# wuwushrek/sde4mbrl_px4

Hardware: AMD Instinct MI355X
Metric: MPC solves/sec, Iris H=50 P=128, arithmetic f32x3/fast (p50 solve latency in p50_solve_latency_ms: arithmetic f32/fast; same-arithmetic pairs in by_arithmetic; every arithmetic against float64 in vs_float64) (higher is better)
Workload: dtype f32 (state, accumulation and every operand f32; the two 32x32 MLP contractions per step evaluated as three-limb bf16 splits of both f32 operands on v_mfma_f32_32x32x16_bf16: error against float64 not larger than the f32 fma chain's (tests/test_mfma16_model_cpu.py), bit-identical to the CPU oracle)

## Files before the change

include/sdempc.h:

```cpp
#ifndef SDEMPC_H
#define SDEMPC_H

#include <stddef.h>
#include <stdint.h>

#ifdef __cplusplus
extern "C" {
#endif

#define SDEMPC_ABI_VERSION 3

#define SDEMPC_NX 13
#define SDEMPC_NNOISE 6
#define SDEMPC_MAX_MOTORS 8
#define SDEMPC_HID 32
#define SDEMPC_BLOB_MAGIC 0x31454453
#define SDEMPC_BLOB_HEADER_INTS 16
#define SDEMPC_BLOB_FLOATS 2120

#define SDEMPC_OK 0
#define SDEMPC_EINVAL (-1)
#define SDEMPC_EBLOB (-2)
#define SDEMPC_EDEVICE (-3)
#define SDEMPC_ENOMEM (-4)
#define SDEMPC_ECAPACITY (-5)

typedef struct sdempc_cfg {
    int32_t struct_size;
    int32_t horizon;
    int32_t num_particles;
    int32_t num_motors;
    const float* time_steps;
    float discount;
    float uref[SDEMPC_MAX_MOTORS];
    float uerr;
    float perr[3], verr[3], qerr[3], werr[3];
    float res_mult;
    float u_slew_coeff;
    int32_t has_slew_constr;
    float u_slew_lo[SDEMPC_MAX_MOTORS], u_slew_hi[SDEMPC_MAX_MOTORS];
    float u_slew_constr_coeff;
    float u_lo[SDEMPC_MAX_MOTORS], u_hi[SDEMPC_MAX_MOTORS];
    int32_t max_iter;
    int32_t max_no_improvement_iter;
    int32_t use_moment_scale;
    float moment_scale;
    float beta_init;
    float atol, rtol;
    float stepsize;
    float ls_init_stepsize, ls_max_stepsize, ls_coef, ls_decrease_factor, ls_increase_factor;
    int32_t ls_reset_option;
    int32_t ls_maxls;
    int32_t mlp_dtype;
    int32_t math_mode;
    int32_t num_state_constr;
    int32_t state_id[SDEMPC_NX];
    float state_w[SDEMPC_NX], state_lo[SDEMPC_NX], state_hi[SDEMPC_NX];
} sdempc_cfg;

typedef struct sdempc_info {
    float avg_linesearch;
    float stepsize;
    float num_steps;
    float grad_sqr;
    float avg_stepsize;
    float init_cost;
    float opt_cost;
    float num_ls_trials;
} sdempc_info;

typedef struct sdempc_handle sdempc_handle;

int sdempc_create(const sdempc_cfg* cfg, const void* model_blob, size_t blob_bytes,
                  int32_t max_batch, sdempc_handle** out);
void sdempc_destroy(sdempc_handle* h);
const char* sdempc_last_error(const sdempc_handle* h);
int sdempc_abi_version(void);
#define SDEMPC_BUILD_ALL_VARIANTS 1
int sdempc_build_flags(void);

int sdempc_set_device(sdempc_handle* h, int32_t device);

int sdempc_device_ready(const sdempc_handle* h);

#define SDEMPC_OPT_LANE 1
#define SDEMPC_OPT_COOP 2
#define SDEMPC_OPT_SPEC 3
#define SDEMPC_OPT_PK 4
#define SDEMPC_OPT_USTG 5
#define SDEMPC_OPT_COOP_LAUNCH 6
#define SDEMPC_OPT_COOP_FENCE 7
#define SDEMPC_OPT_COOP_SPIN_US 8
#define SDEMPC_OPT_DEVICE_CUS 9
#define SDEMPC_OPT_DUO 10
#define SDEMPC_OPT_HEX 11
#define SDEMPC_OPT_TEST_ABSENT_WG 12
#define SDEMPC_OPT_TEST_WS_FILL 13
#define SDEMPC_OPT_TEST_LOOP_CHUNK_BYTES 14
int sdempc_set_option(sdempc_handle* h, int32_t key, int32_t value);
int sdempc_get_option(const sdempc_handle* h, int32_t key, int32_t* value);

int sdempc_reset(sdempc_handle* h, const float* x, const float* xdes, float* yk, sdempc_info* info);

int sdempc_rollout_batch(sdempc_handle* h, int32_t B, const float* x0, const float* u,
                         const float* xref, const float* noise,
                         float* cost , float* traj ,
                         float* xmean );
int sdempc_grad_batch(sdempc_handle* h, int32_t B, const float* x0, const float* u,
                      const float* xref, const float* noise,
                      float* cost , float* grad );
int sdempc_solve_batch(sdempc_handle* h, int32_t B, const float* x0, const float* xref,
                       const float* noise, const float* u_init ,
                       const float* stepsize_in ,
                       float* uopt , float* xevol ,
                       sdempc_info* info );

size_t sdempc_noise_dev_floats(const sdempc_handle* h, int32_t B);
size_t sdempc_traj_dev_floats(const sdempc_handle* h, int32_t B);
int sdempc_noise_to_device_layout(const sdempc_handle* h, int32_t B, const float* noise_host, float* out_host);
int sdempc_noise_to_device_layout_dev(sdempc_handle* h, int32_t B, const void* noise_canonical_dev,
                                      void* noise_out_dev, void* stream);
int sdempc_traj_to_canonical_dev(sdempc_handle* h, int32_t B, void* traj_out_dev, void* stream);
int sdempc_solve_batch_dev(sdempc_handle* h, int32_t B, const void* x0_dev, const void* xref_dev,
                           const void* noise_dev, const void* u_init_dev, const void* stepsize_dev,
                           void* uopt_dev, void* xevol_dev, void* info_dev ,
                           void* stream);
int sdempc_rollout_batch_dev(sdempc_handle* h, int32_t B, const void* x0_dev, const void* u_dev,
                             const void* xref_dev, const void* noise_dev, void* cost_dev,
                             void* xmean_dev , int32_t store_traj, void* stream);
int sdempc_grad_batch_dev(sdempc_handle* h, int32_t B, const void* x0_dev, const void* u_dev,
                          const void* xref_dev, const void* noise_dev, void* cost_dev,
                          void* grad_dev, void* stream);

int sdempc_noise_from_keys_dev(sdempc_handle* h, int32_t B, const uint32_t* keys, void* noise_out_dev , void* stream);
int sdempc_noise_from_keys(sdempc_handle* h, int32_t B, const uint32_t* keys, float* noise );
int sdempc_solve_batch_keys(sdempc_handle* h, int32_t B, const float* x0, const float* xref, const uint32_t* keys,
                            const float* u_init , const float* stepsize_in ,
                            float* uopt , float* xevol , sdempc_info* info );

int sdempc_closed_loop_batch(sdempc_handle* h, int32_t B, int32_t T, const float* x0,
                             const float* xref, int32_t xref_ticks, int32_t xref_batch,
                             const uint32_t* keys, const float* u_init , const float* stepsize_in ,
                             float* xs , float* us , sdempc_info* info ,
                             float* u_next , float* stepsize_next ,
                             uint32_t* keys_next );

#define SDEMPC_PLANT_MAX_SUBSTEPS 64
typedef struct sdempc_plant_cfg {
    int32_t struct_size;
    int32_t num_plants;
    int32_t substeps;
    float dt;
    int32_t mlp_dtype;
    int32_t math_mode;
} sdempc_plant_cfg;
int sdempc_closed_loop_batch_plant(sdempc_handle* h, const sdempc_plant_cfg* pc,
                                   const void* const* plant_blobs , const size_t* plant_blob_bytes ,
                                   const int32_t* plant_of ,
                                   int32_t B, int32_t T, const float* x0,
                                   const float* xref, int32_t xref_ticks, int32_t xref_batch,
                                   const uint32_t* keys, const float* u_init , const float* stepsize_in ,
                                   float* xs , float* us , sdempc_info* info ,
                                   float* u_next , float* stepsize_next ,
                                   uint32_t* keys_next );

typedef struct sdempc_timing_cfg {
    int32_t struct_size;
    int32_t solve_period;
    int32_t solve_delay;
    float lag_alpha;
} sdempc_timing_cfg;
int sdempc_closed_loop_batch_timed(sdempc_handle* h, const sdempc_timing_cfg* timing, const sdempc_plant_cfg* pc,
                                   const void* const* plant_blobs , const size_t* plant_blob_bytes ,
                                   const int32_t* plant_of , int32_t B, int32_t T, const float* x0,
                                   const float* xref, int32_t xref_solves, int32_t xref_batch,
                                   const uint32_t* keys, const float* u_init , const float* stepsize_in ,
                                   const float* u_act_in ,
                                   float* xs , float* us , sdempc_info* info ,
                                   float* u_next , float* stepsize_next ,
                                   uint32_t* keys_next , float* u_act_next );

typedef struct sdempc_scenario_cfg {
    int32_t struct_size;
    const float* dist;
    int32_t dist_ticks;
    int32_t dist_batch;
    int32_t plant_ticks;
} sdempc_scenario_cfg;
int sdempc_closed_loop_batch_scenario(sdempc_handle* h, const sdempc_scenario_cfg* scenario, const sdempc_timing_cfg* timing, const sdempc_plant_cfg* pc,
                                      const void* const* plant_blobs , const size_t* plant_blob_bytes ,
                                      const int32_t* plant_of , int32_t B, int32_t T, const float* x0,
                                      const float* xref, int32_t xref_solves, int32_t xref_batch,
                                      const uint32_t* keys, const float* u_init , const float* stepsize_in ,
                                      const float* u_act_in ,
                                      float* xs , float* us , sdempc_info* info ,
                                      float* u_next , float* stepsize_next ,
                                      uint32_t* keys_next , float* u_act_next );

typedef struct sdempc_rate_cfg {
    int32_t struct_size;
    float kp[3];
    float ki_dt[3];
    float integ_limit[3];
    float mixer[SDEMPC_MAX_MOTORS][3];
    float motor_weight;
    float inv_m;
} sdempc_rate_cfg;
int sdempc_closed_loop_batch_rate(sdempc_handle* h, const sdempc_rate_cfg* rate, const sdempc_scenario_cfg* scenario ,
                                  const sdempc_timing_cfg* timing, const sdempc_plant_cfg* pc,
                                  const void* const* plant_blobs , const size_t* plant_blob_bytes ,
                                  const int32_t* plant_of , int32_t B, int32_t T, const float* x0,
                                  const float* xref, int32_t xref_solves, int32_t xref_batch,
                                  const uint32_t* keys, const float* u_init , const float* stepsize_in ,
                                  const float* u_act_in ,
                                  float* xs , float* us , sdempc_info* info ,
                                  float* u_next , float* stepsize_next ,
                                  uint32_t* keys_next , float* u_act_next ,
                                  const float* rate_integ_in , const float* rate_tail_in ,
                                  float* ws , float* rate_integ_next , float* rate_tail_next );

int sdempc_solve_status(sdempc_handle* h);
int32_t sdempc_layout_fallbacks(const sdempc_handle* h);

int sdempc_work_counters(sdempc_handle* h, uint64_t out[4], int32_t reset);

int sdempc_last_kernel_name(const sdempc_handle* h, char* buf, size_t n);

float sdempc_last_kernel_ms(const sdempc_handle* h);

#ifdef __cplusplus
}
#endif
#endif
```

sde4mbrl_px4_amd/_abi.py:

```python
import ctypes as C
import os

NX = 13
NNOISE = 6
MAX_MOTORS = 8
HID = 32
BLOB_MAGIC = 0x31454453
BLOB_HEADER_INTS = 16
BLOB_FLOATS = 2120

_F8 = C.c_float * MAX_MOTORS
_F3 = C.c_float * 3


class SdempcCfg(C.Structure):
    _fields_ = [
        ("struct_size", C.c_int32),
        ("horizon", C.c_int32),
        ("num_particles", C.c_int32),
        ("num_motors", C.c_int32),
        ("time_steps", C.POINTER(C.c_float)),
        ("discount", C.c_float),
        ("uref", _F8),
        ("uerr", C.c_float),
        ("perr", _F3), ("verr", _F3), ("qerr", _F3), ("werr", _F3),
        ("res_mult", C.c_float),
        ("u_slew_coeff", C.c_float),
        ("has_slew_constr", C.c_int32),
        ("u_slew_lo", _F8), ("u_slew_hi", _F8),
        ("u_slew_constr_coeff", C.c_float),
        ("u_lo", _F8), ("u_hi", _F8),
        ("max_iter", C.c_int32),
        ("max_no_improvement_iter", C.c_int32),
        ("use_moment_scale", C.c_int32),
        ("moment_scale", C.c_float),
        ("beta_init", C.c_float),
        ("atol", C.c_float), ("rtol", C.c_float),
        ("stepsize", C.c_float),
        ("ls_init_stepsize", C.c_float), ("ls_max_stepsize", C.c_float), ("ls_coef", C.c_float),
        ("ls_decrease_factor", C.c_float), ("ls_increase_factor", C.c_float),
        ("ls_reset_option", C.c_int32),
        ("ls_maxls", C.c_int32),
        ("mlp_dtype", C.c_int32),
        ("math_mode", C.c_int32),
        ("num_state_constr", C.c_int32),
        ("state_id", C.c_int32 * NX),
        ("state_w", C.c_float * NX), ("state_lo", C.c_float * NX), ("state_hi", C.c_float * NX),
    ]


class SdempcInfo(C.Structure):
    _fields_ = [(n, C.c_float) for n in (
        "avg_linesearch", "stepsize", "num_steps", "grad_sqr", "avg_stepsize", "init_cost", "opt_cost",
        "num_ls_trials")]


class SdempcPlantCfg(C.Structure):
    _fields_ = [("struct_size", C.c_int32), ("num_plants", C.c_int32), ("substeps", C.c_int32), ("dt", C.c_float),
                ("mlp_dtype", C.c_int32), ("math_mode", C.c_int32)]


class SdempcTimingCfg(C.Structure):
    _fields_ = [("struct_size", C.c_int32), ("solve_period", C.c_int32), ("solve_delay", C.c_int32), ("lag_alpha", C.c_float)]


class SdempcScenarioCfg(C.Structure):
    _fields_ = [("struct_size", C.c_int32), ("dist", C.POINTER(C.c_float)), ("dist_ticks", C.c_int32), ("dist_batch", C.c_int32),
                ("plant_ticks", C.c_int32)]


class SdempcRateCfg(C.Structure):
    _fields_ = [("struct_size", C.c_int32), ("kp", _F3), ("ki_dt", _F3), ("integ_limit", _F3), ("mixer", (C.c_float * 3) * MAX_MOTORS),
                ("motor_weight", C.c_float), ("inv_m", C.c_float)]


PLANT_MAX_SUBSTEPS = 64

INFO_FIELDS = [f[0] for f in SdempcInfo._fields_]

OPTIONS = {"lane": 1, "coop": 2, "spec": 3, "pk": 4, "ustg": 5, "coop_launch": 6, "coop_fence": 7, "coop_spin_us": 8, "device_cus": 9, "duo": 10, "hex": 11, "test_absent_wg": 12, "test_ws_fill": 13,
           "test_loop_chunk_bytes": 14}

ABI_VERSION = 3

_LIB = None


def lib_path():
    override = os.environ.get("SDEMPC_LIB")
    if override:
        return os.path.abspath(override)
    return os.path.join(os.path.dirname(os.path.abspath(__file__)), "csrc", "libsdempc.so")


def load_library():
    global _LIB
    if _LIB is not None:
        return _LIB
    path = lib_path()
    if not os.path.exists(path):
        raise RuntimeError(
            f"{path} is missing: build the HIP extension first (python -c 'import __graft_entry__ as g; g.build()' "
            "or make -C sde4mbrl_px4_amd/csrc). sde4mbrl_px4_amd has no CPU fallback.")
    lib = C.CDLL(path)
    vp, i32, fp = C.c_void_p, C.c_int32, C.POINTER(C.c_float)
    lib.sdempc_create.argtypes = [C.POINTER(SdempcCfg), vp, C.c_size_t, i32, C.POINTER(vp)]
    lib.sdempc_create.restype = C.c_int
    lib.sdempc_destroy.argtypes = [vp]
    lib.sdempc_destroy.restype = None
    lib.sdempc_last_error.argtypes = [vp]
    lib.sdempc_last_error.restype = C.c_char_p
    lib.sdempc_abi_version.restype = C.c_int
    got = lib.sdempc_abi_version()
    if got != ABI_VERSION:
        raise RuntimeError(f"{path} reports ABI version {got}, this package's struct layouts are version {ABI_VERSION} "
                           "(include/sdempc.h: SDEMPC_ABI_VERSION): rebuild the library (make -C sde4mbrl_px4_amd/csrc)")
    lib.sdempc_build_flags.restype = C.c_int
    lib.sdempc_set_device.argtypes = [vp, i32]
    lib.sdempc_device_ready.argtypes = [vp]
    lib.sdempc_device_ready.restype = C.c_int
    lib.sdempc_set_option.argtypes = [vp, i32, i32]
    lib.sdempc_set_option.restype = C.c_int
    lib.sdempc_get_option.argtypes = [vp, i32, C.POINTER(i32)]
    lib.sdempc_get_option.restype = C.c_int
    lib.sdempc_reset.argtypes = [vp, fp, fp, fp, C.POINTER(SdempcInfo)]
    lib.sdempc_rollout_batch.argtypes = [vp, i32, fp, fp, fp, fp, fp, fp, fp]
    lib.sdempc_grad_batch.argtypes = [vp, i32, fp, fp, fp, fp, fp, fp]
    lib.sdempc_solve_batch.argtypes = [vp, i32, fp, fp, fp, fp, fp, fp, fp, C.POINTER(SdempcInfo)]
    lib.sdempc_noise_dev_floats.argtypes = [vp, i32]
    lib.sdempc_noise_dev_floats.restype = C.c_size_t
    lib.sdempc_traj_dev_floats.argtypes = [vp, i32]
    lib.sdempc_traj_dev_floats.restype = C.c_size_t
    lib.sdempc_noise_to_device_layout.argtypes = [vp, i32, fp, fp]
    lib.sdempc_noise_to_device_layout_dev.argtypes = [vp, i32, vp, vp, vp]
    lib.sdempc_traj_to_canonical_dev.argtypes = [vp, i32, vp, vp]
    lib.sdempc_solve_batch_dev.argtypes = [vp, i32] + [vp] * 9
    lib.sdempc_rollout_batch_dev.argtypes = [vp, i32, vp, vp, vp, vp, vp, vp, i32, vp]
    lib.sdempc_grad_batch_dev.argtypes = [vp, i32, vp, vp, vp, vp, vp, vp, vp]
    u32p = C.POINTER(C.c_uint32)
    lib.sdempc_noise_from_keys_dev.argtypes = [vp, i32, u32p, vp, vp]
    lib.sdempc_noise_from_keys.argtypes = [vp, i32, u32p, fp]
    lib.sdempc_solve_batch_keys.argtypes = [vp, i32, fp, fp, u32p, fp, fp, fp, fp, C.POINTER(SdempcInfo)]
    lib.sdempc_closed_loop_batch.argtypes = [vp, i32, i32, fp, fp, i32, i32, u32p, fp, fp, fp, fp, C.POINTER(SdempcInfo), fp, fp, u32p]
    lib.sdempc_closed_loop_batch_plant.argtypes = [vp, C.POINTER(SdempcPlantCfg), C.POINTER(vp), C.POINTER(C.c_size_t), C.POINTER(i32)] + \
        lib.sdempc_closed_loop_batch.argtypes[1:]
    lib.sdempc_solve_status.argtypes = [vp]
    lib.sdempc_solve_status.restype = C.c_int
    lib.sdempc_layout_fallbacks.argtypes = [vp]
    lib.sdempc_layout_fallbacks.restype = C.c_int32
    lib.sdempc_work_counters.argtypes = [vp, C.POINTER(C.c_uint64), i32]
    lib.sdempc_work_counters.restype = C.c_int
    lib.sdempc_last_kernel_name.argtypes = [vp, C.c_char_p, C.c_size_t]
    lib.sdempc_last_kernel_name.restype = C.c_int
    lib.sdempc_last_kernel_ms.argtypes = [vp]
    lib.sdempc_last_kernel_ms.restype = C.c_float
    for name in ("sdempc_set_device", "sdempc_reset", "sdempc_rollout_batch", "sdempc_grad_batch", "sdempc_solve_batch",
                 "sdempc_noise_to_device_layout", "sdempc_solve_batch_dev", "sdempc_rollout_batch_dev",
                 "sdempc_grad_batch_dev", "sdempc_noise_to_device_layout_dev", "sdempc_traj_to_canonical_dev",
                 "sdempc_noise_from_keys_dev", "sdempc_noise_from_keys", "sdempc_solve_batch_keys", "sdempc_closed_loop_batch",
                 "sdempc_closed_loop_batch_plant"):
        getattr(lib, name).restype = C.c_int
    _LIB = lib
    return lib


def timed_entry(lib):
    try:
        fn = lib.sdempc_closed_loop_batch_timed
    except AttributeError:
        raise RuntimeError(f"{lib_path()} has no sdempc_closed_loop_batch_timed (SPEC.md §11b): rebuild the library (make -C sde4mbrl_px4_amd/csrc)") from None
    if fn.argtypes is None:
        a = list(lib.sdempc_closed_loop_batch_plant.argtypes)
        fp = C.POINTER(C.c_float)
        fn.argtypes = [a[0], C.POINTER(SdempcTimingCfg)] + a[1:14] + [fp] + a[14:] + [fp]
        fn.restype = C.c_int
    return fn


def scenario_entry(lib):
    try:
        fn = lib.sdempc_closed_loop_batch_scenario
    except AttributeError:
        raise RuntimeError(f"{lib_path()} has no sdempc_closed_loop_batch_scenario (SPEC.md §11c): rebuild the library (make -C sde4mbrl_px4_amd/csrc)") from None
    if fn.argtypes is None:
        a = list(timed_entry(lib).argtypes)
        fn.argtypes = [a[0], C.POINTER(SdempcScenarioCfg)] + a[1:]
        fn.restype = C.c_int
    return fn


def rate_entry(lib):
    try:
        fn = lib.sdempc_closed_loop_batch_rate
    except AttributeError:
        raise RuntimeError(f"{lib_path()} has no sdempc_closed_loop_batch_rate (SPEC.md §11d): rebuild the library (make -C sde4mbrl_px4_amd/csrc)") from None
    if fn.argtypes is None:
        a = list(scenario_entry(lib).argtypes)
        fp = C.POINTER(C.c_float)
        fn.argtypes = [a[0], C.POINTER(SdempcRateCfg)] + a[1:] + [fp] * 5
        fn.restype = C.c_int
    return fn


EXPORTED_SYMBOLS = [
    "sdempc_create", "sdempc_destroy", "sdempc_last_error", "sdempc_abi_version", "sdempc_build_flags", "sdempc_set_device", "sdempc_device_ready", "sdempc_set_option", "sdempc_get_option", "sdempc_reset",
    "sdempc_rollout_batch", "sdempc_grad_batch", "sdempc_solve_batch", "sdempc_noise_dev_floats",
    "sdempc_traj_dev_floats", "sdempc_noise_to_device_layout", "sdempc_solve_batch_dev", "sdempc_rollout_batch_dev",
    "sdempc_grad_batch_dev", "sdempc_last_kernel_ms", "sdempc_last_kernel_name", "sdempc_work_counters", "sdempc_solve_status", "sdempc_layout_fallbacks", "sdempc_noise_to_device_layout_dev", "sdempc_traj_to_canonical_dev",
    "sdempc_noise_from_keys_dev", "sdempc_noise_from_keys", "sdempc_solve_batch_keys", "sdempc_closed_loop_batch",
    "sdempc_closed_loop_batch_plant", "sdempc_closed_loop_batch_timed", "sdempc_closed_loop_batch_scenario",
    "sdempc_closed_loop_batch_rate",
]
```

sde4mbrl_px4_amd/csrc/sdempc_api.cpp:

```cpp
#include <hip/hip_runtime.h>
#include <math.h>
#include <stdint.h>
#include <stdio.h>
#include <stdlib.h>
#include <string.h>

#include <cxxabi.h>

#include <memory>
#include <new>
#include <stdexcept>
#include <string>
#include <vector>

#include "../../include/sdempc.h"
#include "sdempc_kernels.h"

using namespace sdempc;
static_assert(blob::FLOATS == SDEMPC_BLOB_FLOATS, "blob layout: sdempc_kernels.h and include/sdempc.h");

namespace {
std::string g_create_error;

float f16_rtz_host(float x) {
// ... 174 lines not shown
            (h)->err = b__;                                                             \
            return SDEMPC_EDEVICE;                                                      \
        }                                                                               \
    } while (0)

int env_int(const char* name, int dflt, int lo, int hi) {
    const char* e = getenv(name);
    if (!e || !*e) return dflt;
    char* end = nullptr;
    const long v = strtol(e, &end, 10);
    if (end == e || v < lo || v > hi) return dflt;
    return (int)v;
}
void default_options(sdempc_handle* h) {
    LaunchOpts& o = h->base.opt;
    o.cus = 256;
    o.lane = env_int("SDEMPC_LANE", 1, 0, 1);
    o.coop = env_int("SDEMPC_COOP", 1, 0, 1);
    o.spec = env_int("SDEMPC_SPEC", 1, 0, 1);
    o.pk = env_int("SDEMPC_PK", -1, -1, 1);
    o.ustg = env_int("SDEMPC_USTG", -1, -1, 1);
    o.duo = env_int("SDEMPC_DUO", -1, -1, 1);
    o.coop_launch = env_int("SDEMPC_COOP_LAUNCH", 0, 0, 1);
    o.coop_fence = env_int("SDEMPC_COOP_FENCE", 0, 0, 1);
    o.hex = env_int("SDEMPC_HEX", 1, 0, 1);
    o.absent_wg = -1;
    h->spin_us = env_int("SDEMPC_COOP_SPIN_US", -1, -1, 10 * 1000 * 1000);
}
unsigned coop_spin_ticks(const sdempc_handle* h) {
    if (h->spin_us >= 0) return (unsigned)((uint64_t)h->spin_us * 100u > 0xFFFFFFFFull ? 0xFFFFFFFFu : (unsigned)h->spin_us * 100u);
    float ms = h->coop_ms_last > 0.0f ? 5.0f * h->coop_ms_last : 100.0f;
    if (ms < 2.0f) ms = 2.0f;
    if (ms > 100.0f) ms = 100.0f;
    return (unsigned)(ms * 1e5f);
}

int null_stream_done(sdempc_handle* h) {
    HIPCHK(h, hipStreamSynchronize(nullptr));
    return 0;
}
int dev_alloc(sdempc_handle* h, DevBuf& b, size_t bytes, bool fill = false) {
    if (bytes == 0) bytes = 16;
    HIPCHK(h, hipMalloc(&b.p, bytes));
    b.bytes = bytes;
    if (fill && h->ws_fill >= 0) {
        HIPCHK(h, hipMemset(b.p, h->ws_fill, bytes));
        return null_stream_done(h);
    }
    return 0;
}
void dev_free(DevBuf& b) {
    if (b.p) (void)hipFree(b.p);
    b.p = nullptr;
    b.bytes = 0;
}

size_t noise_floats(const sdempc_handle* h, int B) { return (size_t)B * h->G * h->H * SDEMPC_NNOISE * 32; }
size_t traj_floats(const sdempc_handle* h, int B) { return (size_t)B * h->G * (h->H + 1) * SDEMPC_NX * 32; }

int ensure_device_impl(sdempc_handle* h) {
    if (h->dev_ready) {
        HIPCHK(h, hipSetDevice(h->device));
        return 0;
    }
    int n = 0;
    hipError_t e = hipGetDeviceCount(&n);
    if (e != hipSuccess || n <= 0) return fail(h, SDEMPC_EDEVICE, "no HIP device available (%s); sdempc has no CPU fallback", hipGetErrorString(e));
    if (h->device >= n) return fail(h, SDEMPC_EDEVICE, "device ordinal out of range%s");
    HIPCHK(h, hipSetDevice(h->device));
    {
        int cus = 0;
        HIPCHK(h, hipDeviceGetAttribute(&cus, hipDeviceAttributeMultiprocessorCount, h->device));
        if (cus > 0) h->base.opt.cus = cus;
    }
    HIPCHK(h, hipStreamCreateWithFlags(&h->stream, hipStreamNonBlocking));
    HIPCHK(h, hipEventCreate(&h->ev0));
    HIPCHK(h, hipEventCreate(&h->ev1));
    const int H = h->H, m = h->m, B = h->max_batch;
    int rc;
    if ((rc = dev_alloc(h, h->d_dt, sizeof(float) * H))) return rc;
    if ((rc = dev_alloc(h, h->d_sdt, sizeof(float) * H * SDEMPC_NNOISE))) return rc;
    if ((rc = dev_alloc(h, h->d_disc, sizeof(float) * (H + 1)))) return rc;
    if ((rc = dev_alloc(h, h->d_beta, sizeof(float) * h->h_beta.size()))) return rc;
    if ((rc = dev_alloc(h, h->d_wts, sizeof(float) * h->blob_f.size()))) return rc;
    HIPCHK(h, hipMemcpy(h->d_dt.p, h->time_steps.data(), sizeof(float) * H, hipMemcpyHostToDevice));
    HIPCHK(h, hipMemcpy(h->d_sdt.p, h->h_sdt.data(), sizeof(float) * H * SDEMPC_NNOISE, hipMemcpyHostToDevice));
    HIPCHK(h, hipMemcpy(h->d_disc.p, h->h_disc.data(), sizeof(float) * (H + 1), hipMemcpyHostToDevice));
    HIPCHK(h, hipMemcpy(h->d_beta.p, h->h_beta.data(), sizeof(float) * h->h_beta.size(), hipMemcpyHostToDevice));
    HIPCHK(h, hipMemcpy(h->d_wts.p, h->blob_f.data(), sizeof(float) * h->blob_f.size(), hipMemcpyHostToDevice));
    if (h->cfg.num_state_constr > 0) {
        CostK::StateBound tab[SDEMPC_NX];
        for (int k = 0; k < h->cfg.num_state_constr; ++k)
            tab[k] = CostK::StateBound{h->cfg.state_id[k], h->cfg.state_w[k], h->cfg.state_lo[k], h->cfg.state_hi[k]};
        if ((rc = dev_alloc(h, h->d_sctab, sizeof(CostK::StateBound) * h->cfg.num_state_constr))) return rc;
        HIPCHK(h, hipMemcpy(h->d_sctab.p, tab, sizeof(CostK::StateBound) * h->cfg.num_state_constr, hipMemcpyHostToDevice));
        h->base.C.sc_n = h->cfg.num_state_constr;
        h->base.C.sc_tab = (const CostK::StateBound*)h->d_sctab.p;
    }
    if ((rc = dev_alloc(h, h->d_x0, sizeof(float) * B * SDEMPC_NX, true))) return rc;
    if ((rc = dev_alloc(h, h->d_u, sizeof(float) * B * H * m, true))) return rc;
    if ((rc = dev_alloc(h, h->d_xref, sizeof(float) * B * (H + 1) * SDEMPC_NX, true))) return rc;
    if ((rc = dev_alloc(h, h->d_noise, sizeof(float) * noise_floats(h, B), true))) return rc;
    if ((rc = dev_alloc(h, h->d_step, sizeof(float) * B, true))) return rc;
    if ((rc = dev_alloc(h, h->d_cost, sizeof(float) * B, true))) return rc;
    if ((rc = dev_alloc(h, h->d_grad, sizeof(float) * B * H * m, true))) return rc;
    if ((rc = dev_alloc(h, h->d_xmean, sizeof(float) * B * (H + 1) * SDEMPC_NX, true))) return rc;
    if ((rc = dev_alloc(h, h->d_uopt, sizeof(float) * B * H * m, true))) return rc;
    if ((rc = dev_alloc(h, h->d_info, sizeof(float) * B * 8, true))) return rc;
    if ((rc = dev_alloc(h, h->d_work, sizeof(unsigned long long) * 5))) return rc;
    HIPCHK(h, hipMemset(h->d_work.p, 0, h->d_work.bytes));
    if ((rc = null_stream_done(h))) return rc;
    h->base.work = (unsigned long long*)h->d_work.p;
    h->base.ticket_host = &h->ticket_total;
    h->ticket_total = 0;
    h->base.dt = (const float*)h->d_dt.p;
    h->base.sdt = (const float*)h->d_sdt.p;
    h->base.disc = (const float*)h->d_disc.p;
    h->base.beta = (const float*)h->d_beta.p;
    h->base.wts = (const float*)h->d_wts.p;
    h->dev_ready = true;
    return 0;
}

int ensure_workspace(sdempc_handle* h, int rows) {
    if (rows <= h->ws_rows) return 0;
    HIPCHK(h, hipStreamSynchronize(h->stream));
    for (DevBuf* b : {&h->d_traj, &h->d_act, &h->d_part, &h->d_ustg}) dev_free(*b);
    h->ws_rows = 0; h->base.ws_rows = 0; h->traj_batch = 0;
    h->base.traj = h->base.act = h->base.part = h->base.ustg = nullptr;
    const int H = h->H;
    int rc;
    if ((rc = dev_alloc(h, h->d_traj, sizeof(float) * traj_floats(h, rows), true))) return rc;
    if (h->ws_fill < 0) {
        HIPCHK(h, hipMemset(h->d_traj.p, 0, h->d_traj.bytes));
        if ((rc = null_stream_done(h))) return rc;
    }
    if ((rc = dev_alloc(h, h->d_act, sizeof(float) * (size_t)rows * h->G * H * ACT_STRIDE, true))) return rc;
    if ((rc = dev_alloc(h, h->d_part, sizeof(float) * (size_t)rows * h->G * part_stride(H), true))) return rc;
    if ((rc = dev_alloc(h, h->d_ustg, sizeof(float) * (size_t)rows * H * 36, true))) return rc;
    h->base.traj = (float*)h->d_traj.p;
    h->base.act = (float*)h->d_act.p;
    h->base.part = (float*)h->d_part.p;
    h->base.ustg = (float*)h->d_ustg.p;
    h->ws_rows = rows;
    h->base.ws_rows = rows;
    return 0;
}

void release_device(sdempc_handle* h);

int ensure_device(sdempc_handle* h) {
    const bool was_ready = h->dev_ready;
    const int rc = ensure_device_impl(h);
    if (rc != 0 && !was_ready) { const std::string keep = h->err; release_device(h); h->err = keep; }
    return rc;
}

int check_batch(sdempc_handle* h, int B) {
    if (!h) return SDEMPC_EINVAL;
    if (B < 1) return fail(h, SDEMPC_EINVAL, "batch must be >= 1%s");
    if (B > h->max_batch) return fail(h, SDEMPC_ECAPACITY, "batch exceeds max_batch given to sdempc_create%s");
    return 0;
}

void noise_to_dev_layout(const sdempc_handle* h, int B, const float* in, float* out) {
    const int P = h->P, H = h->H, G = h->G;
    memset(out, 0, sizeof(float) * noise_floats(h, B));
    for (int b = 0; b < B; ++b)
        for (int p = 0; p < P; ++p) {
            const int g = p / 32, l = p % 32;
            for (int t = 0; t < H; ++t)
                for (int i = 0; i < SDEMPC_NNOISE; ++i)
                    out[((((size_t)b * G + g) * H + t) * SDEMPC_NNOISE + i) * 32 + l] = in[(((size_t)b * P + p) * H + t) * SDEMPC_NNOISE + i];
        }
}

int stage_common(sdempc_handle* h, int B, const float* x0, const float* u, const float* xref, const float* noise) {
    const int H = h->H, m = h->m;
    int rc;
    if (!h->d_noise_canon.p && (rc = dev_alloc(h, h->d_noise_canon, sizeof(float) * (size_t)h->max_batch * h->P * H * SDEMPC_NNOISE, true))) return rc;
    HIPCHK(h, hipMemcpyAsync(h->d_x0.p, x0, sizeof(float) * B * SDEMPC_NX, hipMemcpyHostToDevice, h->stream));
    HIPCHK(h, hipMemcpyAsync(h->d_u.p, u, sizeof(float) * B * H * m, hipMemcpyHostToDevice, h->stream));
    HIPCHK(h, hipMemcpyAsync(h->d_xref.p, xref, sizeof(float) * B * (H + 1) * SDEMPC_NX, hipMemcpyHostToDevice, h->stream));
    HIPCHK(h, hipMemcpyAsync(h->d_noise_canon.p, noise, sizeof(float) * (size_t)B * h->P * H * SDEMPC_NNOISE, hipMemcpyHostToDevice, h->stream));
    HIPCHK(h, launch_relayout(true, (const float*)h->d_noise_canon.p, (float*)h->d_noise.p, B, h->P, h->G, H * SDEMPC_NNOISE, h->stream));
    return 0;
}

int noise_from_keys(sdempc_handle* h, int B, const uint32_t* keys, float* out_dev, hipStream_t st) {
    int rc;
    if (!h->d_keys.p && (rc = dev_alloc(h, h->d_keys, sizeof(uint32_t) * 2 * (size_t)h->max_batch))) return rc;
    HIPCHK(h, hipMemcpyAsync(h->d_keys.p, keys, sizeof(uint32_t) * 2 * (size_t)B, hipMemcpyHostToDevice, st));
    HIPCHK(h, launch_noise_from_keys((const uint32_t*)h->d_keys.p, out_dev, B, h->P, h->G, h->H, st));
    return 0;
}

int coop_timed_out(sdempc_handle* h, bool* timed_out) {
    *timed_out = false;
    if (h->last_coop_B <= 0) return 0;
    std::vector<unsigned> f(COOP_BAR_WORDS * (size_t)h->last_coop_B);
    HIPCHK(h, hipMemcpy(f.data(), h->d_coop_bar.p, sizeof(unsigned) * f.size(), hipMemcpyDeviceToHost));
    for (int b = 0; b < h->last_coop_B; ++b)
        if (f[COOP_BAR_WORDS * b + 1] != 0u) *timed_out = true;
    if (*timed_out) {
        h->coop_off = true;
        h->layout_fallbacks += 1;
        h->last_coop_B = 0;
    } else if (h->timed) {
        float ms = 0.0f;
        if (hipEventElapsedTime(&ms, h->ev0, h->ev1) == hipSuccess && ms > 0.0f) h->coop_ms_last = ms;
    }
    return 0;
}

int tickets_consistent(sdempc_handle* h) {
    if (!h->last_ticketed || !h->dev_ready) return 0;
    h->last_ticketed = false;
    unsigned word = 0;
    HIPCHK(h, hipMemcpy(&word, (const char*)h->d_work.p + 4 * sizeof(unsigned long long), sizeof word, hipMemcpyDeviceToHost));
    if (word == h->ticket_total) return 0;
    char msg[256];
    snprintf(msg, sizeof msg, "ticketed launch: the device's ticket word reads %u where the host expects %u (aborted kernel, overlapping launches of one "
                              "handle, or a replayed graph); instances of that launch may be unsolved", word, h->ticket_total);
    h->ticket_total = word;
    return fail(h, SDEMPC_EDEVICE, "%s", msg);
}

template <class F>
int timed_launch(sdempc_handle* h, hipStream_t st, F&& f) {
    HIPCHK(h, hipEventRecord(h->ev0, st));
    hipError_t e = f();
    if (e != hipSuccess) return fail(h, SDEMPC_EDEVICE, "kernel launch failed: %s", hipGetErrorString(e));
    HIPCHK(h, hipEventRecord(h->ev1, st));
    h->timed = true;
    h->last_fn = last_launched_kernel();
    return 0;
}


int solve_staged(sdempc_handle* h, int32_t B, float* uopt, float* xevol, sdempc_info* info);
struct LoopIo {
    int B, T, xref_ticks, xref_batch;
    const float *x0, *xref;
    const uint32_t* keys;
    const float *u_init, *stepsize_in;
    float *xs, *us;
    sdempc_info* info;
    float *u_next, *stepsize_next;
    uint32_t* keys_next;
};
struct PlantRun {
    KArgs k;
    LoopPlant Q;
    float* xi;
    float dt;
};
struct TimedRun {
    int S, D;
    float alpha;
    const float* u_act_in;
    float* u_act_next;
};
struct ScenarioRun {
    const float* dist;
    int Td, Bd;
    const int32_t* plant_of;
    int Tp;
};
struct RateRun {
    const sdempc_rate_cfg* cfg;
    float inv_m;
    const float *integ_in, *tail_in;
    float *ws, *integ_next, *tail_next;
};
inline int loop_solves(int T, int S) { return (int)(((long long)T + S - 1) / S); }
enum LoopLayer { LOOP_PLAIN, LOOP_PLANT, LOOP_TIMED, LOOP_SCENARIO, LOOP_RATE };
struct LoopCall {
    LoopLayer layer;
    LoopIo io;
    const sdempc_plant_cfg* pc;
    const void* const* plant_blobs;
    const size_t* plant_blob_bytes;
    const int32_t* plant_of;
    const sdempc_timing_cfg* tc;
    const float* u_act_in;
    float* u_act_next;
    const sdempc_scenario_cfg* sc;
    const sdempc_rate_cfg* rc;
    const float *rate_integ_in, *rate_tail_in;
    float *ws, *rate_integ_next, *rate_tail_next;
};
int closed_loop_call(sdempc_handle* h, const LoopCall& c);
int check_loop_args(sdempc_handle* h, const LoopIo& io, int solves);
int check_plant_args(sdempc_handle* h, const sdempc_plant_cfg* pc, const void* const* plant_blobs, const size_t* plant_blob_bytes, const int32_t* plant_of, int B, int sched_rows);
int closed_loop_attempts(sdempc_handle* h, const LoopIo& io, const PlantRun* plant, const TimedRun* timed, const ScenarioRun* scen, const RateRun* rate);
int closed_loop_run(sdempc_handle* h, const LoopIo& io, const PlantRun* plant, const TimedRun* timed, const ScenarioRun* scen, const RateRun* rate, bool* again);
int stage_plants(sdempc_handle* h, const sdempc_plant_cfg& pc, const void* const* blobs, const int32_t* plant_of, int B, PlantRun* out, int xi_ticks = 1);
}

extern "C" {

int sdempc_abi_version(void) { return SDEMPC_ABI_VERSION; }
int sdempc_build_flags(void) { return SDEMPC_ALL_VARIANTS ? SDEMPC_BUILD_ALL_VARIANTS : 0; }

const char* sdempc_last_error(const sdempc_handle* h) { return h ? h->err.c_str() : g_create_error.c_str(); }

int sdempc_create(const sdempc_cfg* cfg, const void* model_blob, size_t blob_bytes, int32_t max_batch, sdempc_handle** out) {
    return guarded(nullptr, [&]() -> int {
    if (!out) return fail(nullptr, SDEMPC_EINVAL, "out is NULL%s");
    *out = nullptr;
    if (!cfg || cfg->struct_size != (int32_t)sizeof(sdempc_cfg)) return fail(nullptr, SDEMPC_EINVAL, "cfg NULL or struct_size mismatch%s");
    if (int rc = check_blob(nullptr, model_blob, blob_bytes)) return rc;
    const int32_t* hd = (const int32_t*)model_blob;
    const int m = hd[2];
    if (m < 1 || m > SDEMPC_MAX_MOTORS || m != cfg->num_motors) return fail(nullptr, SDEMPC_EINVAL, "num_motors of cfg and model blob differ or out of range%s");
    if (cfg->horizon < 1 || cfg->horizon > 4096 || cfg->num_particles < 1 || !cfg->time_steps || max_batch < 1)
        return fail(nullptr, SDEMPC_EINVAL, "horizon/num_particles/time_steps/max_batch invalid%s");
    if (cfg->max_iter < 0 || cfg->ls_maxls < 0 || cfg->max_no_improvement_iter < 1) return fail(nullptr, SDEMPC_EINVAL, "apg parameters invalid%s");
    if (cfg->num_state_constr < 0 || cfg->num_state_constr > SDEMPC_NX) return fail(nullptr, SDEMPC_EINVAL, "num_state_constr out of range%s");
    for (int k = 0; k < cfg->num_state_constr; ++k)
        if (cfg->state_id[k] < 0 || cfg->state_id[k] >= SDEMPC_NX || (k > 0 && cfg->state_id[k] <= cfg->state_id[k - 1]))
            return fail(nullptr, SDEMPC_EINVAL, "state_id must be strictly ascending indices into the 13-state%s");
    for (int t = 0; t < cfg->horizon; ++t)
        if (!(cfg->time_steps[t] > 0.0f)) return fail(nullptr, SDEMPC_EINVAL, "time_steps must be positive%s");
    if (smem_bytes(cfg->horizon, m, team_ipb((cfg->num_particles + 31) / 32, cfg->horizon, m)) > 160 * 1024) return fail(nullptr, SDEMPC_EINVAL, "horizon too large for one workgroup's LDS (160 KiB)%s");
    if (cfg->max_iter > 10 * 1000 * 1000) return fail(nullptr, SDEMPC_EINVAL, "max_iter beyond 10^7%s");
    std::unique_ptr<sdempc_handle> hp(new (std::nothrow) sdempc_handle());
    sdempc_handle* h = hp.get();
    if (!h) return fail(nullptr, SDEMPC_ENOMEM, "out of memory%s");
    h->cfg = *cfg;
    h->H = cfg->horizon; h->P = cfg->num_particles; h->m = m; h->G = (h->P + 31) / 32; h->max_batch = max_batch;
    h->time_steps.assign(cfg->time_steps, cfg->time_steps + h->H);
    h->cfg.time_steps = h->time_steps.data();
    const float* f = (const float*)(hd + SDEMPC_BLOB_HEADER_INTS);
    if (cfg->mlp_dtype < 0 || cfg->mlp_dtype > 2) return fail(nullptr, SDEMPC_EINVAL, "mlp_dtype must be 0 (f32), 1 (f16) or 2 (f32x3)%s");
    if (cfg->math_mode != 0 && cfg->math_mode != 1) return fail(nullptr, SDEMPC_EINVAL, "math_mode must be 0 (exact) or 1 (fast)%s");
    PreparedModel pm;
    prepare_model(f, cfg->mlp_dtype, cfg->math_mode, h->time_steps.data(), h->H, pm);
    h->blob_f = std::move(pm.blob_f);
    h->h_sdt = std::move(pm.sdt);
    h->h_disc.resize(h->H + 1);
    float d = 1.0f / (float)h->H;
    for (int t = 0; t <= h->H; ++t) { h->h_disc[t] = d; d = d * cfg->discount; }
    h->h_beta.resize(cfg->max_iter + 2);
    for (int i = 0; i < cfg->max_iter + 2; ++i) {
        float b = (i == 0) ? cfg->beta_init : (float)(i + 1) / (float)(i + 4);
        if (i > 0 && cfg->use_moment_scale) b = cfg->moment_scale * b;
        h->h_beta[i] = b;
    }
    KArgs& a = h->base;
    memset(&a, 0, sizeof a);
    a.H = h->H; a.P = h->P; a.m = m; a.G = h->G;
    a.invP = 1.0f / (float)h->P;
    a.f16 = cfg->mlp_dtype;
    a.fast = cfg->math_mode == 1;
    a.M = pm.M;
    for (int i = 0; i < 3; ++i) { a.C.perr[i] = cfg->perr[i]; a.C.verr[i] = cfg->verr[i]; a.C.qerr[i] = cfg->qerr[i]; a.C.werr[i] = cfg->werr[i]; }
    a.C.res_mult = cfg->res_mult; a.C.uerr = cfg->uerr; a.C.slew = cfg->u_slew_coeff; a.C.slew_cc = cfg->u_slew_constr_coeff;
    a.C.has_sc = cfg->has_slew_constr;
    for (int j = 0; j < 8; ++j) {
        a.C.slew_lo[j] = cfg->u_slew_lo[j]; a.C.slew_hi[j] = cfg->u_slew_hi[j]; a.C.uref[j] = cfg->uref[j];
        a.C.ulo[j] = cfg->u_lo[j]; a.C.uhi[j] = cfg->u_hi[j];
    }
    a.C.sc_n = 0; a.C.sc_tab = nullptr;
    a.A.max_iter = cfg->max_iter; a.A.max_noimp = cfg->max_no_improvement_iter; a.A.maxls = cfg->ls_maxls;
    a.A.reset_inc = cfg->ls_reset_option == 1;
    a.A.atol = cfg->atol; a.A.rtol = cfg->rtol; a.A.stepsize = cfg->stepsize; a.A.smax = cfg->ls_max_stepsize;
    a.A.coef = cfg->ls_coef; a.A.dec = cfg->ls_decrease_factor; a.A.inc = cfg->ls_increase_factor;
    default_options(h);
    *out = hp.release();
    return SDEMPC_OK;
    });
}

void sdempc_destroy(sdempc_handle* h) {
    if (!h) return;
    release_device(h);
    delete h;
}

}

namespace {
void release_device(sdempc_handle* h) {
    if (h->dev_ready || h->stream || h->d_dt.p) {
        (void)hipSetDevice(h->device);
        for (DevBuf* b : {&h->d_sctab, &h->d_ustg, &h->d_part, &h->d_act, &h->d_dt, &h->d_sdt, &h->d_disc, &h->d_beta, &h->d_wts, &h->d_traj, &h->d_x0, &h->d_u, &h->d_xref, &h->d_noise, &h->d_noise_canon, &h->d_traj_canon, &h->d_keys, &h->d_loop, &h->d_loop_chunk, &h->d_plant, &h->d_rate, &h->d_work, &h->d_coop_bar, &h->d_coop_pp, &h->d_coop_ck,
                          &h->d_step, &h->d_cost, &h->d_grad, &h->d_xmean, &h->d_uopt, &h->d_info})
            dev_free(*b);
        if (h->ev0) (void)hipEventDestroy(h->ev0);
        if (h->ev1) (void)hipEventDestroy(h->ev1);
        if (h->stream) (void)hipStreamDestroy(h->stream);
        h->ev0 = h->ev1 = nullptr; h->stream = nullptr; h->coop_cap = 0; h->ws_rows = 0;
    }
    h->dev_ready = false; h->timed = false;
}
}

extern "C" {

int sdempc_set_device(sdempc_handle* h, int32_t device) {
    return guarded(h, [&]() -> int {
    if (!h) return SDEMPC_EINVAL;
    if (h->dev_ready) return fail(h, SDEMPC_EINVAL, "sdempc_set_device must precede the first device call%s");
    if (device < 0) return fail(h, SDEMPC_EINVAL, "negative device ordinal%s");
    h->device = device;
    return SDEMPC_OK;
    });
}

int sdempc_device_ready(const sdempc_handle* h) { return h && h->dev_ready ? 1 : 0; }

int sdempc_set_option(sdempc_handle* h, int32_t key, int32_t value) {
    return guarded(h, [&]() -> int {
    if (!h) return SDEMPC_EINVAL;
    LaunchOpts& o = h->base.opt;
    auto flag = [&](int& dst) { if (value != 0 && value != 1) return fail(h, SDEMPC_EINVAL, "option value must be 0 or 1%s"); dst = value; return (int)SDEMPC_OK; };
    auto tri = [&](int& dst) { if (value < -1 || value > 1) return fail(h, SDEMPC_EINVAL, "option value must be -1 (auto), 0 or 1%s"); dst = value; return (int)SDEMPC_OK; };
    switch (key) {
        case SDEMPC_OPT_LANE: return flag(o.lane);
        case SDEMPC_OPT_COOP: { int rc = flag(o.coop); if (rc == SDEMPC_OK && value == 1) h->coop_off = false; return rc; }
        case SDEMPC_OPT_SPEC: return flag(o.spec);
        case SDEMPC_OPT_PK:
            if (value == 1 && !SDEMPC_ALL_VARIANTS) return fail(h, SDEMPC_EINVAL, "this build carries no packed-tanh instantiations (make EXTRA=-DSDEMPC_ALL_VARIANTS=1)%s");
            return tri(o.pk);
        case SDEMPC_OPT_USTG: return tri(o.ustg);
        case SDEMPC_OPT_DUO: return tri(o.duo);
        case SDEMPC_OPT_COOP_LAUNCH: return flag(o.coop_launch);
        case SDEMPC_OPT_COOP_FENCE: return flag(o.coop_fence);
        case SDEMPC_OPT_HEX: return flag(o.hex);
        case SDEMPC_OPT_TEST_ABSENT_WG:
            if (value < -1) return fail(h, SDEMPC_EINVAL, "absent workgroup must be -1 (none) or a workgroup index%s");
            o.absent_wg = value;
            return SDEMPC_OK;
        case SDEMPC_OPT_TEST_WS_FILL:
            if (value < -1 || value > 255) return fail(h, SDEMPC_EINVAL, "workspace fill must be -1 (none) or a byte value 0..255%s");
            h->ws_fill = value;
            return SDEMPC_OK;
        case SDEMPC_OPT_COOP_SPIN_US:
            if (value < -1) return fail(h, SDEMPC_EINVAL, "spin budget must be -1 (derived) or >= 0 microseconds%s");
            h->spin_us = value;
            return SDEMPC_OK;
        case SDEMPC_OPT_TEST_LOOP_CHUNK_BYTES:
            if (value < -1) return fail(h, SDEMPC_EINVAL, "loop chunk bytes must be -1 (built-in) or >= 0%s");
            h->loop_chunk_bytes = value;
            return SDEMPC_OK;
        default: return fail(h, SDEMPC_EINVAL, "unknown option key%s");
    }
    });
}

int sdempc_get_option(const sdempc_handle* h, int32_t key, int32_t* value) {
    return guarded(h, [&]() -> int {
    if (!h || !value) return SDEMPC_EINVAL;
    const LaunchOpts& o = h->base.opt;
    switch (key) {
        case SDEMPC_OPT_LANE: *value = o.lane; break;
        case SDEMPC_OPT_COOP: *value = o.coop && !h->coop_off; break;
        case SDEMPC_OPT_SPEC: *value = o.spec; break;
        case SDEMPC_OPT_PK: *value = o.pk; break;
        case SDEMPC_OPT_USTG: *value = o.ustg; break;
        case SDEMPC_OPT_DUO: *value = o.duo; break;
        case SDEMPC_OPT_COOP_LAUNCH: *value = o.coop_launch; break;
        case SDEMPC_OPT_COOP_FENCE: *value = o.coop_fence; break;
        case SDEMPC_OPT_HEX: *value = o.hex; break;
        case SDEMPC_OPT_TEST_ABSENT_WG: *value = o.absent_wg; break;
        case SDEMPC_OPT_TEST_WS_FILL: *value = h->ws_fill; break;
        case SDEMPC_OPT_TEST_LOOP_CHUNK_BYTES: *value = h->loop_chunk_bytes; break;
        case SDEMPC_OPT_COOP_SPIN_US: *value = h->spin_us >= 0 ? h->spin_us : (int32_t)(coop_spin_ticks(h) / 100u); break;
        case SDEMPC_OPT_DEVICE_CUS: *value = o.cus; break;
        default: return SDEMPC_EINVAL;
    }
    return SDEMPC_OK;
    });
}

int sdempc_reset(sdempc_handle* h, const float* x, const float* xdes, float* yk, sdempc_info* info) {
    return guarded(h, [&]() -> int {
    if (!h || !yk || !info) return SDEMPC_EINVAL;
    (void)x; (void)xdes;
    for (int t = 0; t < h->H; ++t)
        for (int j = 0; j < h->m; ++j) yk[t * h->m + j] = h->cfg.uref[j];
    memset(info, 0, sizeof *info);
    info->stepsize = h->cfg.ls_maxls > 0 ? h->cfg.ls_init_stepsize : h->cfg.stepsize;
    return SDEMPC_OK;
    });
}

size_t sdempc_noise_dev_floats(const sdempc_handle* h, int32_t B) { return h ? noise_floats(h, B) : 0; }
size_t sdempc_traj_dev_floats(const sdempc_handle* h, int32_t B) { return h ? traj_floats(h, B) : 0; }

int sdempc_noise_to_device_layout(const sdempc_handle* h, int32_t B, const float* noise_host, float* out_host) {
    return guarded(h, [&]() -> int {
    if (!h || !noise_host || !out_host || B < 1) return SDEMPC_EINVAL;
    noise_to_dev_layout(h, B, noise_host, out_host);
    return SDEMPC_OK;
    });
}

int sdempc_noise_to_device_layout_dev(sdempc_handle* h, int32_t B, const void* noise_canonical_dev, void* noise_out_dev, void* stream) {
    return guarded(h, [&]() -> int {
    int rc = check_batch(h, B);
    if (rc) return rc;
    if (!noise_canonical_dev || !noise_out_dev) return fail(h, SDEMPC_EINVAL, "NULL device pointer%s");
    if ((rc = ensure_device(h))) return rc;
    hipStream_t st = stream ? (hipStream_t)stream : h->stream;
    HIPCHK(h, launch_relayout(true, (const float*)noise_canonical_dev, (float*)noise_out_dev, B, h->P, h->G, h->H * SDEMPC_NNOISE, st));
    return SDEMPC_OK;
    });
}

int sdempc_traj_to_canonical_dev(sdempc_handle* h, int32_t B, void* traj_out_dev, void* stream) {
    return guarded(h, [&]() -> int {
    int rc = check_batch(h, B);
    if (rc) return rc;
    if (!traj_out_dev) return fail(h, SDEMPC_EINVAL, "NULL device pointer%s");
    if ((rc = ensure_device(h))) return rc;
    if (B > h->traj_batch)
        return fail(h, SDEMPC_EINVAL, h->traj_batch ? "the trajectory workspace holds fewer instances than asked for (last rollout with store_traj was smaller)%s"
                                                     : "the trajectory workspace holds no rollout: run a rollout with store_traj first (a gradient evaluation, a solve or a "
                                                       "workspace reallocation since then has overwritten it)%s");
    hipStream_t st = stream ? (hipStream_t)stream : h->stream;
    HIPCHK(h, launch_relayout(false, (const float*)h->d_traj.p, (float*)traj_out_dev, B, h->P, h->G, (h->H + 1) * SDEMPC_NX, st));
    return SDEMPC_OK;
    });
}

int sdempc_rollout_batch_dev(sdempc_handle* h, int32_t B, const void* x0_dev, const void* u_dev, const void* xref_dev, const void* noise_dev,
                             void* cost_dev, void* xmean_dev, int32_t store_traj, void* stream) {
    return guarded(h, [&]() -> int {
    int rc = check_batch(h, B);
    if (rc) return rc;
    if (!x0_dev || !u_dev || !xref_dev || !noise_dev || !cost_dev) return fail(h, SDEMPC_EINVAL, "NULL device pointer%s");
    if ((rc = ensure_device(h))) return rc;
    if ((rc = ensure_workspace(h, B))) return rc;
    KArgs a = h->base;
    a.x0 = (const float*)x0_dev; a.u = (const float*)u_dev; a.xref = (const float*)xref_dev; a.noise = (const float*)noise_dev;
    a.cost = (float*)cost_dev; a.xmean = (float*)xmean_dev; a.store_traj = store_traj;
    hipStream_t st = stream ? (hipStream_t)stream : h->stream;
    h->traj_batch = 0;
    rc = timed_launch(h, st, [&] { return launch_rollout(a, B, st); });
    if (rc == SDEMPC_OK && store_traj) h->traj_batch = B;
    return rc;
    });
}

int sdempc_grad_batch_dev(sdempc_handle* h, int32_t B, const void* x0_dev, const void* u_dev, const void* xref_dev, const void* noise_dev,
                          void* cost_dev, void* grad_dev, void* stream) {
    return guarded(h, [&]() -> int {
    int rc = check_batch(h, B);
    if (rc) return rc;
    if (!x0_dev || !u_dev || !xref_dev || !noise_dev || !cost_dev || !grad_dev) return fail(h, SDEMPC_EINVAL, "NULL device pointer%s");
    if ((rc = ensure_device(h))) return rc;
    if ((rc = ensure_workspace(h, B))) return rc;
    KArgs a = h->base;
    a.x0 = (const float*)x0_dev; a.u = (const float*)u_dev; a.xref = (const float*)xref_dev; a.noise = (const float*)noise_dev;
    a.cost = (float*)cost_dev; a.grad = (float*)grad_dev;
    hipStream_t st = stream ? (hipStream_t)stream : h->stream;
    h->traj_batch = 0;
    return timed_launch(h, st, [&] { return launch_grad(a, B, st); });
    });
}

int sdempc_solve_batch_dev(sdempc_handle* h, int32_t B, const void* x0_dev, const void* xref_dev, const void* noise_dev, const void* u_init_dev,
                           const void* stepsize_dev, void* uopt_dev, void* xevol_dev, void* info_dev, void* stream) {
    return guarded(h, [&]() -> int {
    int rc = check_batch(h, B);
    if (rc) return rc;
    if (!x0_dev || !xref_dev || !noise_dev || !u_init_dev || !stepsize_dev || !uopt_dev || !xevol_dev || !info_dev)
        return fail(h, SDEMPC_EINVAL, "NULL device pointer%s");
    if ((rc = ensure_device(h))) return rc;
    {
        KArgs probe = h->base; probe.B = B;
        if ((rc = ensure_workspace(h, solve_workspace_rows(probe, B)))) return rc;
    }
    h->traj_batch = 0;
    KArgs a = h->base;
    a.x0 = (const float*)x0_dev; a.u = (const float*)u_init_dev; a.xref = (const float*)xref_dev; a.noise = (const float*)noise_dev;
    a.stepsize_in = (const float*)stepsize_dev; a.uopt = (float*)uopt_dev; a.xmean = (float*)xevol_dev; a.info = (float*)info_dev;
    hipStream_t st = stream ? (hipStream_t)stream : h->stream;
    const bool coop_ok = !a.f16 && !h->coop_off && a.C.sc_n == 0;
    const int smax = coop_ok ? spec_max_instances(h->P, h->H, h->m, a.opt) : 0;
    int cmax = coop_ok ? coop_max_instances(h->P, h->H, h->m, a.opt) : 0;
    if (smax > cmax) cmax = smax;
    if (B <= cmax) {
        if (!h->d_coop_bar.p) {
            const int cap = cmax < h->max_batch ? cmax : h->max_batch;
            if ((rc = dev_alloc(h, h->d_coop_bar, sizeof(unsigned) * COOP_BAR_WORDS * (size_t)cap))) return rc;
            if ((rc = dev_alloc(h, h->d_coop_pp, sizeof(float) * coop_pp_floats(h->H, h->G) * cap, true))) return rc;
            if ((rc = dev_alloc(h, h->d_coop_ck, sizeof(float) * coop_ck_floats(h->H, h->P) * cap, true))) return rc;
            h->coop_cap = cap;
        }
        if (B <= h->coop_cap) {
            HIPCHK(h, hipMemsetAsync(h->d_coop_bar.p, 0, sizeof(unsigned) * COOP_BAR_WORDS * (size_t)B, st));
            a.coop_bar = (unsigned*)h->d_coop_bar.p; a.coop_pp = (float*)h->d_coop_pp.p; a.coop_ck = (float*)h->d_coop_ck.p;
            a.coop_spin = coop_spin_ticks(h);
            h->last_coop_B = B; h->last_ticketed = false;
            if (B <= smax) {
                HIPCHK(h, hipMemsetAsync(h->d_coop_pp.p, 0, sizeof(float) * coop_pp_floats(h->H, h->G) * (size_t)B, st));
                return timed_launch(h, st, [&] { return launch_solve_spec(a, B, st); });
            }
            if (B <= coop_max_instances(h->P, h->H, h->m, a.opt)) return timed_launch(h, st, [&] { return launch_solve_coop(a, B, st); });
            h->last_coop_B = 0;
        }
    }
    h->last_coop_B = 0;
// ... 585 lines not shown
```

sde4mbrl_px4_amd/csrc/sdempc_duo.inc.h:

```cpp

DI void half_split(float v, float& a_both, float& b_both) {
    unsigned a = __builtin_bit_cast(unsigned, v), b;
    asm("v_mov_b32 %0, %1" : "=v"(b) : "v"(a));
    auto r = __builtin_amdgcn_permlane32_swap(a, b, false, false);
    const unsigned r0 = r[0], r1 = r[1];
    a_both = __builtin_bit_cast(float, r0); b_both = __builtin_bit_cast(float, r1);
}
DI float half_join_sum(float pa, float pb) {
    auto r = __builtin_amdgcn_permlane32_swap(__builtin_bit_cast(unsigned, pa), __builtin_bit_cast(unsigned, pb), false, false);
    const unsigned r0 = r[0], r1 = r[1];
    return __builtin_bit_cast(float, r0) + __builtin_bit_cast(float, r1);
}

template <class Team>
DI int duo_workspace_slot() { return __builtin_amdgcn_readfirstlane((int)(blockIdx.x * Team::IPB) + Team::team()); }

struct DuoPair {
    int g;
    bool hasB;
    bool own;
};
DI DuoPair duo_pair(int gp, int G, int h) {
    DuoPair p;
    p.hasB = (2 * gp + 1) < G;
    p.own = (h == 0) || p.hasB;
    p.g = 2 * gp + ((h && p.hasB) ? 1 : 0);
    return p;
}

DI void duo_reform_rotation(const float* x, float* Rm) {
    float xq[NX];
#pragma unroll
    for (int i = 0; i < NX; ++i) xq[i] = x[i];
#pragma unroll
    for (int i = 6; i < 10; ++i) asm volatile("" : "+v"(xq[i]));
    rot_from_q(xq, Rm);
}

constexpr int PRIO_SLICE_LOG2 = 16;
DI void duo_rotate_priority() {
    const unsigned slot = __builtin_amdgcn_s_getreg(63492) & 15u;
    const unsigned r = ((unsigned)(__builtin_amdgcn_s_memrealtime() >> PRIO_SLICE_LOG2) + slot) % 3u;
    if (r == 0) __builtin_amdgcn_s_setprio(0);
    else if (r == 1) __builtin_amdgcn_s_setprio(1);
    else __builtin_amdgcn_s_setprio(2);
}

DI void duo_noise_request(const float* nzb, unsigned nzo, int t, const float* stage) {
    const float* rows = nzb + (size_t)t * (NN * 32);
    const unsigned m0 = (unsigned)__builtin_amdgcn_readfirstlane((int)(unsigned)(size_t)(const __attribute__((address_space(3))) float*)stage);
    unsigned m0_keep;
    asm volatile(
        "s_mov_b32 %0, m0\n\t"
        "s_mov_b32 m0, %3\n\ts_nop 0\n\tglobal_load_lds_dword %1, %2\n\t"
        "s_add_u32 m0, m0, 0x80\n\ts_nop 0\n\tglobal_load_lds_dword %1, %2 offset:128\n\t"
        "s_add_u32 m0, m0, 0x80\n\ts_nop 0\n\tglobal_load_lds_dword %1, %2 offset:256\n\t"
        "s_add_u32 m0, m0, 0x80\n\ts_nop 0\n\tglobal_load_lds_dword %1, %2 offset:384\n\t"
        "s_add_u32 m0, m0, 0x80\n\ts_nop 0\n\tglobal_load_lds_dword %1, %2 offset:512\n\t"
        "s_add_u32 m0, m0, 0x80\n\ts_nop 0\n\tglobal_load_lds_dword %1, %2 offset:640\n\t"
        "s_mov_b32 m0, %0"
        : "=&s"(m0_keep) : "v"(nzo * 4u), "s"(rows), "s"(m0) : "memory", "scc");
}
template <int PENDING>
DI void duo_noise_take(const float* stage, int lane, float* xi) {
    asm volatile("s_waitcnt vmcnt(%0)" ::"n"(PENDING) : "memory");
#pragma unroll
    for (int i = 0; i < NN; ++i) xi[i] = stage[i * 64 + lane];
}

template <int F16, bool CKPT, bool NZS>
DI void duo_step_fwd(const KArgs& a, const Smem& sm, const WaveW& ww, int t, int h, int lane, bool hasB, const float* x, const float* xi_reg, float* xn,
                     StepAux& A, float* acA, float* acB) {
    const float* ust = sm.ust + t * UST;
    float z[NN], zA[NN], zB[NN];
    fwd_head(x, A.Rm, z);
#pragma unroll
    for (int k = 0; k < NN; ++k) half_split(z[k], zA[k], zB[k]);
    SCHED_PHASE();
    float PA[7], PB[7];
    fwd_mlp_partials<F16, false, CKPT ? 4 : 7>(a, sm, ww, ust, h, lane, zA, A, PA);
    if constexpr (CKPT) {
#pragma unroll
        for (int q = 0; q < 4; ++q)
            *reinterpret_cast<float4*>(acA + (q * 64 + lane) * 4) = make_float4(A.h2[4 * q], A.h2[4 * q + 1], A.h2[4 * q + 2], A.h2[4 * q + 3]);
    }
    SCHED_PHASE();
    if (hasB) {
        fwd_mlp_partials<F16, false, CKPT ? 4 : 7>(a, sm, ww, ust, h, lane, zB, A, PB);
        if constexpr (CKPT) {
#pragma unroll
            for (int q = 0; q < 4; ++q)
                *reinterpret_cast<float4*>(acB + (q * 64 + lane) * 4) = make_float4(A.h2[4 * q], A.h2[4 * q + 1], A.h2[4 * q + 2], A.h2[4 * q + 3]);
        }
    } else {
#pragma unroll
        for (int i = 0; i < 7; ++i) PB[i] = PA[i];
    }
    SCHED_PHASE();
    float o[6];
#pragma unroll
    for (int i = 0; i < 6; ++i) o[i] = half_join_sum(PA[i], PB[i]) + a.M.b3[i];
    const float eta = sigmoid_spec(half_join_sum(PA[6], PB[6]) + a.M.b3n);
    SCHED_PHASE();
    if constexpr (CKPT) duo_reform_rotation(x, A.Rm);
    float xi[NN];
    if constexpr (NZS) duo_noise_take<CKPT ? 4 : 0>(sm.nzs, lane, xi);
    else {
#pragma unroll
        for (int i = 0; i < NN; ++i) xi[i] = xi_reg[i];
    }
    fwd_tail(a, sm, ust, t, x, xi, A.Rm, o, eta, xn, A);
}

template <class Team, int F16, bool NZS>
DI float duo_rollout(const KArgs& a, const Smem& sm, const WaveW& ww, const float* u, int b, int tid, bool store_traj, float* xmean_out) {
    b = opaque_s(b); tid = opaque_v(tid);
    const int H = a.H, G = a.G, P = a.P;
    const int lane = tid & 63, j = lane & 31, h = lane >> 5;
    const int wave = __builtin_amdgcn_readfirstlane(tid >> 6);
    const bool want_mean = xmean_out != nullptr;
    CLK_BEGIN(t_roll);
    Team::sync();
    block_prepass<Team>(a, sm, u, tid);
    const int PS = part_stride(H);
    const int ws = duo_workspace_slot<Team>();
    float* prows = a.part + (size_t)ws * G * PS;
    float cu = block_ucost<Team>(a, sm, u, tid);
    Team::sync();
    const int NPAIR = (G + 1) >> 1;
    for (int gp = wave; gp < NPAIR; gp += Team::NWAVES) {
        const DuoPair pr = duo_pair(gp, G, h);
        const bool valid = pr.own && (pr.g * 32 + j) < P;
        const unsigned gofs = (unsigned)(pr.g - 2 * gp);
        const float* nzb = a.noise + ((size_t)(b * G + 2 * gp) * H) * NN * 32;
        float* tjb = a.traj + ((size_t)(ws * G + 2 * gp) * (H + 1)) * NX * 32;
        const unsigned nzo = gofs * (unsigned)(H * NN * 32) + (unsigned)j;
        const unsigned tjo = gofs * (unsigned)((H + 1) * NX * 32) + (unsigned)j;
        float* xm = prows + (size_t)pr.g * PS;
        float x[NX], xn[NX], xi[NN];
#pragma unroll
        for (int i = 0; i < NX; ++i) x[i] = a.x0[b * NX + i];
        if constexpr (NZS) {
            duo_noise_request(nzb, nzo, 0, sm.nzs);
#pragma unroll
            for (int i = 0; i < NX; ++i) asm volatile("" : "+v"(x[i]));
        } else {
#pragma unroll
            for (int i = 0; i < NN; ++i) xi[i] = nzb[nzo + (unsigned)(i * 32)];
        }
        if (store_traj && pr.own) {
#pragma unroll
            for (int i = 0; i < NX; ++i) tjb[tjo + (unsigned)(i * 32)] = x[i];
        }
        if (want_mean) {
#pragma unroll
            for (int i = 0; i < NX; ++i) { float s = group_bfly32(valid ? x[i] : 0.0f); if (j == 0 && pr.own) xm[i] = s; }
        }
        float J = 0.0f;
        StepAux A;
        CLK_BEGIN(t_loop);
        for (int t = 0; t < H; ++t) {
            duo_rotate_priority();
            float xin[NN];
            if constexpr (!NZS) {
                if (t + 1 < H) {
#pragma unroll
                    for (int i = 0; i < NN; ++i) xin[i] = nzb[nzo + (unsigned)(((t + 1) * NN + i) * 32)];
                }
            }
            duo_step_fwd<F16, false, NZS>(a, sm, ww, t, h, lane, pr.hasB, x, xi, xn, A, nullptr, nullptr);
            if constexpr (NZS) { if (t + 1 < H) duo_noise_request(nzb, nzo, t + 1, sm.nzs); }
            float l = stage_cost<false>(a, xn, sm.xref + (t + 1) * NX, nullptr);
            l = FMA(a.C.res_mult * A.eta, A.eta, l);
            J = FMA(sm.disc[t], l, J);
#pragma unroll
            for (int i = 0; i < NX; ++i) x[i] = xn[i];
            if constexpr (!NZS) {
                if (t + 1 < H) {
#pragma unroll
                    for (int i = 0; i < NN; ++i) xi[i] = xin[i];
                }
            }
            if (store_traj && pr.own) {
#pragma unroll
                for (int i = 0; i < NX; ++i) tjb[tjo + (unsigned)(((t + 1) * NX + i) * 32)] = x[i];
            }
            if (want_mean) {
#pragma unroll
                for (int i = 0; i < NX; ++i) { float s = group_bfly32(valid ? x[i] : 0.0f); if (j == 0 && pr.own) xm[(t + 1) * NX + i] = s; }
            }
        }
        CLK_END(2, t_loop);
        const float T = group_bfly32(valid ? J : 0.0f);
        if (j == 0 && pr.own) xm[PS - 1] = T;
    }
    Team::sync();
    const float tot = group_ordered_sum(prows, G, PS, PS - 1);
    if (want_mean) {
        for (int i = tid; i < (H + 1) * NX; i += Team::NT) xmean_out[i] = group_ordered_sum(prows, G, PS, i) * a.invP;
    }
    CLK_END(1, t_roll);
    return FMA(tot, a.invP, cu);
}

template <class Team, int M, int F16, bool NZS>
DI float duo_cost_grad(const KArgs& a, const Smem& sm, const WaveW& ww, const float* y, float* gout, int b, int tid) {
    b = opaque_s(b); tid = opaque_v(tid);
    const int H = a.H, G = a.G, P = a.P;
    constexpr int nq = M + 4;
    const int lane = tid & 63, j = lane & 31, h = lane >> 5;
    const int wave = __builtin_amdgcn_readfirstlane(tid >> 6);
    CLK_BEGIN(t_grad);
    Team::sync();
    block_prepass<Team>(a, sm, y, tid);
    const int PS = part_stride(H);
    const int ws = duo_workspace_slot<Team>();
    float* prows = a.part + (size_t)ws * G * PS;
    float cu = block_ucost<Team>(a, sm, y, tid);
    Team::sync();
    const int NPAIR = (G + 1) >> 1;
    for (int gp = wave; gp < NPAIR; gp += Team::NWAVES) {
        const DuoPair pr = duo_pair(gp, G, h);
        const bool valid = pr.own && (pr.g * 32 + j) < P;
        const int gA = 2 * gp, gB = pr.hasB ? 2 * gp + 1 : gA;
        const unsigned gofs = (unsigned)(pr.g - gA);
        const float* nzb = a.noise + ((size_t)(b * G + gA) * H) * NN * 32;
        float* tjb = a.traj + ((size_t)(ws * G + gA) * (H + 1)) * NX * 32;
        const unsigned nzo = gofs * (unsigned)(H * NN * 32) + (unsigned)j;
        const unsigned tjo = gofs * (unsigned)((H + 1) * NX * 32) + (unsigned)j;
        float* acA = a.act + ((size_t)(ws * G + gA) * H) * ACT_STRIDE;
        float* acB = a.act + ((size_t)(ws * G + gB) * H) * ACT_STRIDE;
        const unsigned aso = gofs * (unsigned)(H * ACT_STRIDE) + 1024u + (unsigned)j * 8u;
        float* Sq = prows + (size_t)pr.g * PS;
        float x[NX], xn[NX], xi[NN];
        StepAux A;
        CLK_BEGIN(t_fwd);
#pragma unroll
        for (int i = 0; i < NX; ++i) x[i] = a.x0[b * NX + i];
        if (pr.own) {
#pragma unroll
            for (int i = 0; i < NX; ++i) tjb[tjo + (unsigned)(i * 32)] = x[i];
        }
        if constexpr (NZS) {
            duo_noise_request(nzb, nzo, 0, sm.nzs);
#pragma unroll
            for (int i = 0; i < NX; ++i) asm volatile("" : "+v"(x[i]));
        } else {
#pragma unroll
            for (int i = 0; i < NN; ++i) xi[i] = nzb[nzo + (unsigned)(i * 32)];
        }
        float J = 0.0f;
        for (int t = 0; t < H; ++t) {
            duo_rotate_priority();
            float xin[NN];
            if constexpr (!NZS) {
                if (t + 1 < H) {
#pragma unroll
                    for (int i = 0; i < NN; ++i) xin[i] = nzb[nzo + (unsigned)(((t + 1) * NN + i) * 32)];
                }
            }
            duo_step_fwd<F16, true, NZS>(a, sm, ww, t, h, lane, pr.hasB, x, xi, xn, A, acA + (size_t)t * ACT_STRIDE, acB + (size_t)t * ACT_STRIDE);
            if constexpr (NZS) { if (t + 1 < H) duo_noise_request(nzb, nzo, t + 1, sm.nzs); }
            if (pr.own) {
                const unsigned so = aso + (unsigned)(t * ACT_STRIDE);
                *reinterpret_cast<float4*>(acA + so) = make_float4(A.eta, A.Fb[0], A.Fb[1], A.Fb[2]);
                acA[so + 4] = A.rn;
            }
            float l = stage_cost<false>(a, xn, sm.xref + (t + 1) * NX, nullptr);
            l = FMA(a.C.res_mult * A.eta, A.eta, l);
            J = FMA(sm.disc[t], l, J);
#pragma unroll
            for (int i = 0; i < NX; ++i) x[i] = xn[i];
            if constexpr (!NZS) {
                if (t + 1 < H) {
#pragma unroll
                    for (int i = 0; i < NN; ++i) xi[i] = xin[i];
                }
            }
            if (pr.own) {
#pragma unroll
                for (int i = 0; i < NX; ++i) tjb[tjo + (unsigned)(((t + 1) * NX + i) * 32)] = x[i];
            }
        }
        { const float T = group_bfly32(valid ? J : 0.0f); if (j == 0 && pr.own) Sq[PS - 1] = T; }
        CLK_END(4, t_fwd);
        CLK_BEGIN(t_adj);
        float lam[NX], xt[NX];
#pragma unroll
        for (int i = 0; i < NX; ++i) lam[i] = 0.0f;
        __builtin_amdgcn_fence(__ATOMIC_SEQ_CST, "workgroup");
        for (int t = H - 1; t >= 0; --t) {
            duo_rotate_priority();
            const float* apA = acA + (size_t)t * ACT_STRIDE;
            const float* apB = acB + (size_t)t * ACT_STRIDE;
            float4 hA[4], hB[4];
#pragma unroll
            for (int q = 0; q < 4; ++q) hA[q] = *reinterpret_cast<const float4*>(apA + (q * 64 + lane) * 4);
            float touched = 0.0f;
            {
                if (pr.hasB) {
                    const float* tp = apB + (lane & 31) * 32;
                    asm volatile("global_load_dword %0, %1, off" : "=v"(touched) : "v"(tp) : "memory");
                }
            }
            const unsigned so = aso + (unsigned)(t * ACT_STRIDE);
            const float4 ns4 = *reinterpret_cast<const float4*>(acA + so);
            const float nrn = acA[so + 4];
            {
#pragma unroll
                for (int i = 0; i < NX; ++i) xt[i] = tjb[tjo + (unsigned)((t * NX + i) * 32)];
#pragma unroll
                for (int i = 0; i < NN; ++i) xi[i] = nzb[nzo + (unsigned)((t * NN + i) * 32)];
            }
            const float dsc = sm.disc[t];
            {
                float gx[NX];
                stage_cost<true>(a, x, sm.xref + (t + 1) * NX, gx);
#pragma unroll
                for (int i = 0; i < NX; ++i) lam[i] = FMA(dsc, gx[i], lam[i]);
            }
            SCHED_PHASE();
            const float* ust = sm.ust + t * UST;
            float z[NN], zA[NN], zB[NN];
            fwd_head(xt, A.Rm, z);
#pragma unroll
            for (int k = 0; k < NN; ++k) half_split(z[k], zA[k], zB[k]);
            A.eta = ns4.x; A.Fb[0] = ns4.y; A.Fb[1] = ns4.z; A.Fb[2] = ns4.w; A.rn = nrn;
#pragma unroll
            for (int i = 0; i < 3; ++i) A.Jom[i] = a.M.J[i] * xt[10 + i];
#pragma unroll
            for (int i = 0; i < 4; ++i) A.qn[i] = x[6 + i];
            const float ebc = dsc * ((2.0f * a.C.res_mult) * A.eta);
            VjpTmp T;
            float gq[12], lamn[NX];
            vjp_head<M>(a, sm, t, xt, xi, A, lam, ebc, T, gq);
            float eA, eB, obA[6], obB[6];
            float adj_inv = 1.0f;
            ObLimbs OA, OB;
            if constexpr (FAST && F16 != 0) {
                const AdjScale S = adj_scale(a, T.ebraw, T.ob);
                adj_inv = S.inv;
                half_split(T.ebraw * S.s2, eA, eB);
                float obs[6];
#pragma unroll
                for (int i = 0; i < 6; ++i) obs[i] = T.ob[i] * S.s2;
                const ObLimbs O = ob_limbs(obs);
#pragma unroll
                for (int i = 0; i < 3; ++i) {
                    float la, lb;
                    half_split(__builtin_bit_cast(float, O.r1[i]), la, lb); OA.r1[i] = __builtin_bit_cast(unsigned, la); OB.r1[i] = __builtin_bit_cast(unsigned, lb);
                    half_split(__builtin_bit_cast(float, O.r2[i]), la, lb); OA.r2[i] = __builtin_bit_cast(unsigned, la); OB.r2[i] = __builtin_bit_cast(unsigned, lb);
                }
            } else {
            half_split(T.ebraw, eA, eB);
#pragma unroll
            for (int i = 0; i < 6; ++i) half_split(T.ob[i], obA[i], obB[i]);
            }
            SCHED_PHASE();
            float zb[NN];
            if constexpr (FAST && F16 != 0) {
                constexpr int NR = AdjRegs<M>::N;
                float rA[NR], rB[NR];
                if constexpr (NZS) {
#pragma unroll
                    for (int k = 0; k < NN; ++k) sm.nzs[k * 64 + lane] = zB[k];
                }
                adj_mlp_pass_mp<NR, false, F16>(sm, ww, ust, h, lane, zA, hA, eA, OA, rA, []() {});
                SCHED_PHASE();
                if constexpr (NZS) {
#pragma unroll
                    for (int k = 0; k < NN; ++k) zB[k] = sm.nzs[k * 64 + lane];
                }
                if (pr.hasB) adj_mlp_pass_mp<NR, true, F16>(sm, ww, ust, h, lane, zB, hB, eB, OB, rB, [&]() {
#pragma unroll
                    for (int q = 0; q < 4; ++q) hB[q] = *reinterpret_cast<const float4*>(apB + (q * 64 + lane) * 4);
                });
                else {
#pragma unroll
                    for (int r = 0; r < NR; ++r) asm volatile("v_mov_b32 %0, %1" : "=v"(rB[r]) : "v"(rA[r]));
                }
                SCHED_PHASE();
                float lo[8], hi[8];
#pragma unroll
                for (int r = 0; r < NR; ++r) {
                    auto sw = __builtin_amdgcn_permlane32_swap(__builtin_bit_cast(unsigned, rA[r]), __builtin_bit_cast(unsigned, rB[r]), false, false);
                    const unsigned s0 = sw[0], s1 = sw[1];
                    lo[r] = __builtin_bit_cast(float, s0); hi[r] = __builtin_bit_cast(float, s1);
                }
#pragma unroll
                for (int k = 0; k < NN; ++k) zb[k] = (adj_row_upper(k) ? hi[adj_row_reg(k)] : lo[adj_row_reg(k)]) * adj_inv;
#pragma unroll
                for (int jj = 0; jj < M; ++jj) gq[jj] = (adj_row_upper(NN + jj) ? hi[adj_row_reg(NN + jj)] : lo[adj_row_reg(NN + jj)]) * adj_inv;
            } else {
            float PzA[NN], PuA[M], PzB[NN], PuB[M];
            adj_mlp_pass<M, F16>(sm, ww, ust, h, lane, zA, hA, eA, obA, PzA, PuA);
            SCHED_PHASE();
            if (pr.hasB) {
#pragma unroll
                for (int q = 0; q < 4; ++q) hB[q] = *reinterpret_cast<const float4*>(apB + (q * 64 + lane) * 4);
                SCHED_PHASE();
                adj_mlp_pass<M, F16>(sm, ww, ust, h, lane, zB, hB, eB, obB, PzB, PuB);
            } else {
#pragma unroll
                for (int k = 0; k < NN; ++k) PzB[k] = PzA[k];
#pragma unroll
                for (int jj = 0; jj < M; ++jj) PuB[jj] = PuA[jj];
            }
            SCHED_PHASE();
#pragma unroll
            for (int k = 0; k < NN; ++k) zb[k] = half_join_sum(PzA[k], PzB[k]);
#pragma unroll
            for (int jj = 0; jj < M; ++jj) gq[jj] = half_join_sum(PuA[jj], PuB[jj]);
            }
            asm volatile("" :: "v"(touched));
            duo_reform_rotation(xt, A.Rm);
            vjp_tail(sm, t, xt, A, lam, T, zb, lamn);
#pragma unroll
            for (int i = 0; i < NX; ++i) { lam[i] = lamn[i]; x[i] = xt[i]; }
#pragma unroll
            for (int k = 0; k < nq; ++k) {
                const float s = group_bfly32(valid ? gq[k] : 0.0f);
                if (j == 0 && pr.own) Sq[t * 12 + k] = s;
            }
        }
        CLK_END(5, t_adj);
    }
    Team::sync();
    const float tot = group_ordered_sum(prows, G, PS, PS - 1);
    assemble_gradient<Team, M>(a, sm, y, gout, tid, [&](int q) { return group_ordered_sum(prows, G, PS, q); });
    Team::sync();
    CLK_END(3, t_grad);
    return FMA(tot, a.invP, cu);
}
```

sde4mbrl_px4_amd/csrc/sdempc_kernels.h:

```cpp
#pragma once
#include <hip/hip_runtime.h>
#include <stddef.h>
#include <stdint.h>

#ifndef SDEMPC_ALL_VARIANTS
#define SDEMPC_ALL_VARIANTS 0
#endif

namespace sdempc {

namespace blob {
constexpr int SF = 40;
constexpr int SIGMA = 48;
constexpr int W1Z = 56, B1 = W1Z + 64 * 6, W1U = B1 + 64, W2 = W1U + 32 * 8, B2 = W2 + 32 * 32, W3 = B2 + 32, B3 = W3 + 8 * 32, W3N = B3 + 8, B3N = W3N + 32;
constexpr int FLOATS = B3N + 8;
static_assert(FLOATS == 2120, "include/sdempc.h: SDEMPC_BLOB_FLOATS");
}

struct ModelK {
    float inv_mass, grav, J[3], iJ[3], ct2, ct1, ct0, cm2, cm1;
    float rx[8], ry[8], dir[8];
    float sF[3], sT[3];
    float b3[6], b3n;
    float adj_s0, adj_i0;
};
struct CostK {
    float perr[3], verr[3], qerr[3], werr[3];
    float res_mult, uerr, slew, slew_cc;
    int has_sc;
    float slew_lo[8], slew_hi[8], uref[8], ulo[8], uhi[8];
    int sc_n;
    struct StateBound { int id; float w, lo, hi; };
    const StateBound* sc_tab;
};
struct ApgK {
    int max_iter, max_noimp, maxls, reset_inc;
    float atol, rtol, stepsize, smax, coef, dec, inc;
};
struct LaunchOpts {
    int cus;
    int lane;
    int coop;
    int spec;
    int pk;
    int ustg;
    int coop_launch;
    int duo;
    int coop_fence;
    int absent_wg;
    int hex;
};
constexpr int COOP_BAR_WORDS = 4;
struct KArgs {
    int H, P, m, G;
    int B;
    float invP;
    ModelK M;
    CostK C;
    ApgK A;
    const float* dt;
    const float* sdt;
    const float* disc;
    const float* beta;
    const float* wts;
    const float* x0;
    const float* u;
    const float* xref;
    const float* noise;
    const float* stepsize_in;
    float* traj;
    float* act;
    float* part;
    float* cost;
    float* grad;
    float* xmean;
    float* uopt;
    float* info;
    int store_traj;
    int ws_rows;
    int f16;
    int coop_nwg;
    int coop_ngrp;
    unsigned* coop_bar;
    float* ustg;
    unsigned coop_spin;
    float* coop_pp;
    float* coop_ck;
    unsigned long long* work;
    int tickets;
    unsigned ticket_base;
    unsigned* ticket_host;
    int fast;
    LaunchOpts opt;
};

__host__ __device__ inline int part_stride(int H) { const int a = H * 12, b = (H + 1) * 13; return ((a > b ? a : b) + 1 + 3) & ~3; }
constexpr int ACT_STRIDE = 1280;
size_t smem_bytes(int H, int m, int ipb);
void note_kernel(const void* host_fn);
const void* last_launched_kernel();
int coop_nwg(int P);
int coop_max_instances(int P, int H, int m, const LaunchOpts& o);
size_t coop_pp_floats(int H, int G);
size_t coop_ck_floats(int H, int P);
hipError_t launch_solve_coop(const KArgs& a, int B, hipStream_t st);
int spec_max_instances(int P, int H, int m, const LaunchOpts& o);
hipError_t launch_solve_spec(const KArgs& a, int B, hipStream_t st);
int team_ipb(int G, int H, int m);
hipError_t launch_rollout(const KArgs& a, int B, hipStream_t st);
hipError_t launch_grad(const KArgs& a, int B, hipStream_t st);
hipError_t launch_solve(const KArgs& a, int B, hipStream_t st);
int solve_workspace_rows(const KArgs& a, int B);
struct LoopAdvance {
    const float* uopt;
    const float* info;
    const float* xi;
    const unsigned* coop_bar;
    float* x;
    float* u;
    float* step;
    float* xs;
    float* us;
    unsigned* gave_up;
    int B, H;
};
struct LoopPlant {
    const ModelK* models;
    const float* wts;
    const float* sdt;
    const int* plant_of;
    int wts_stride;
    int substeps;
};
struct LoopPeriod {
    float* act;
    float alpha;
    int ticks;
    int xi_ticks;
    int shift;
    int arrive;
};
struct LoopScenario {
    const float* dist;
    int dist_tick_stride;
    int dist_ep_stride;
    const int* plant;
    int plant_tick_stride;
    float dtp;
};
struct LoopRate {
    float kp[3], ki_dt[3], glim[3];
    float M[8][3];
    float lo[8], hi[8];
    float inv_m;
    float w;
    const float* xevol;
    float* wt;
    float* g;
    float* ws;
};
hipError_t launch_loop(const KArgs& a, const LoopAdvance& L, const LoopPlant* Q, const LoopPeriod* R, const LoopScenario* C, const LoopRate* W, hipStream_t st);
hipError_t launch_loop_keys(uint32_t* keys_dev, uint32_t* sub_dev, float* xi_dev, int B, hipStream_t st, int substeps = 1);
hipError_t launch_loop_keys_period(uint32_t* keys_dev, uint32_t* sub_dev, float* xi_dev, int B, int ticks, int xi_ticks, int substeps, hipStream_t st);
hipError_t launch_broadcast_rows(const float* row_dev, float* rows_dev, int n, int B, hipStream_t st);
hipError_t launch_relayout(bool to_dev, const float* in, float* out, int B, int P, int G, int C, hipStream_t st);
hipError_t launch_noise_from_keys(const uint32_t* keys_dev, float* out, int B, int P, int G, int H, hipStream_t st);

}
```

sde4mbrl_px4_amd/csrc/sdempc_kernels.hip:

```cpp
#include <hip/hip_runtime.h>
#include <stdint.h>
#include <stdlib.h>
#include <type_traits>
#include "sdempc_kernels.h"

#ifndef SDEMPC_FAST
#define SDEMPC_FAST 0
#endif
#ifndef SDEMPC_TU
#define SDEMPC_TU 0
#endif
#ifndef SDEMPC_VAR_PHASE_CLK
#define SDEMPC_VAR_PHASE_CLK 0
#endif

namespace sdempc {
#if SDEMPC_FAST
namespace fastm {
#else
namespace exact {
#endif
constexpr bool FAST = SDEMPC_FAST != 0;

typedef float f32x16 __attribute__((ext_vector_type(16)));
typedef _Float16 half8 __attribute__((ext_vector_type(8)));
typedef __bf16 bf16x8 __attribute__((ext_vector_type(8)));
typedef unsigned u32x4 __attribute__((ext_vector_type(4)));
#define FMA(a, b, c) __builtin_fmaf((a), (b), (c))
#define DI __device__ __forceinline__
#define SCHED_PHASE() __builtin_amdgcn_sched_barrier(0)

constexpr int NX = 13, NN = 6, HID = 32;

struct TeamBlock {
    static constexpr int NT = 256, NWAVES = 4, IPB = 1, BNT = 256;
    DI static int tid() { return threadIdx.x; }
    DI static int team() { return 0; }
    DI static void sync() { __syncthreads(); }
};
struct TeamBlock8 {
    static constexpr int NT = 512, NWAVES = 8, IPB = 1, BNT = 512;
    DI static int tid() { return threadIdx.x; }
    DI static int team() { return 0; }
    DI static void sync() { __syncthreads(); }
};
struct TeamBlock2 {
    static constexpr int NT = 128, NWAVES = 2, IPB = 1, BNT = 128;
    DI static int tid() { return threadIdx.x; }
    DI static int team() { return 0; }
    DI static void sync() { __syncthreads(); }
};
__shared__ unsigned sdempc_pair_bar[8];
#if SDEMPC_VAR_PHASE_CLK
__shared__ unsigned long long sdempc_clk[8][8];
DI unsigned long long clk_now() { return __builtin_amdgcn_s_memrealtime(); }
DI void clk_add(int slot, unsigned long long t0) { if ((threadIdx.x & 63) == 0) sdempc_clk[threadIdx.x >> 6][slot] += clk_now() - t0; }
#define CLK_BEGIN(v) const unsigned long long v = clk_now()
#define CLK_END(slot, v) clk_add(slot, v)
#else
#define CLK_BEGIN(v) ((void)0)
#define CLK_END(slot, v) ((void)0)
#endif
template <int IPB_>
struct TeamPairT {
    static constexpr int NT = 128, NWAVES = 2, IPB = IPB_, BNT = 128 * IPB_;
    DI static int tid() { return threadIdx.x & 127; }
    DI static int team() { return __builtin_amdgcn_readfirstlane(threadIdx.x >> 7); }
    DI static void sync() {
        CLK_BEGIN(tb);
        __builtin_amdgcn_fence(__ATOMIC_RELEASE, "workgroup");
        unsigned* c = sdempc_pair_bar + team();
        unsigned v = 0;
        if ((threadIdx.x & 63) == 0) v = __hip_atomic_fetch_add(c, 1u, __ATOMIC_RELAXED, __HIP_MEMORY_SCOPE_WORKGROUP);
        v = (unsigned)__builtin_amdgcn_readfirstlane((int)v);
        const unsigned target = (v | 1u) + 1u;
        while ((int)(__hip_atomic_load(c, __ATOMIC_RELAXED, __HIP_MEMORY_SCOPE_WORKGROUP) - target) < 0) __builtin_amdgcn_s_sleep(1);
        __builtin_amdgcn_fence(__ATOMIC_ACQUIRE, "workgroup");
        CLK_END(6, tb);
    }
};
using TeamPair = TeamPairT<2>;
using TeamHex = TeamPairT<6>;
struct TeamWave {
    static constexpr int NT = 64, NWAVES = 1, IPB = 4, BNT = 256;
    DI static int tid() { return threadIdx.x & 63; }
    DI static int team() { return __builtin_amdgcn_readfirstlane(threadIdx.x >> 6); }
    DI static void sync() { __builtin_amdgcn_fence(__ATOMIC_SEQ_CST, "workgroup"); __builtin_amdgcn_wave_barrier(); }
};

#include "sdempc_math.inc.h"

struct Smem {
    float *W3, *w3n, *b1n, *b2, *b1d, *W1zT, *W1uT;
    float *A2, *A2T;
    float *A2h;
    float *A2x, *A2xT;
    float *ust;
    float *xref;
    float *dt, *sdt, *disc;
    float *red;
    float *tot;
    float *rec, *nzl, *cend;
    float *v[6];
    float *nzs;
};
constexpr int NZ_STAGE = 6 * 64;
constexpr int ZROWS_D = 15, ZROWS_N = 7;
constexpr int A3T_ROWS = 33;
struct AdjOff { int xt, azd, azn, a3t; };
__host__ __device__ constexpr AdjOff adj_off(int f16) { return f16 == 2 ? AdjOff{1536, 1024, 2560, 2784} : AdjOff{0, 1024, 1536, 1760}; }
static_assert(adj_off(2).azd + 2 * 2 * 2 * ZROWS_D * 4 <= 1536 && adj_off(2).azn + 2 * 2 * 2 * ZROWS_N * 4 <= adj_off(2).a3t && adj_off(2).a3t + 2 * A3T_ROWS * 4 <= 3072, "f32x3: adjoint images must fit the slack of the limb region");
static_assert(adj_off(1).azd + 2 * 2 * 2 * ZROWS_D * 4 <= adj_off(1).azn && adj_off(1).azn + 2 * 2 * 2 * ZROWS_N * 4 <= adj_off(1).a3t && adj_off(1).a3t + 2 * A3T_ROWS * 4 <= 2048, "f16: adjoint images must stay below the fp16 forward image");
constexpr int UST = 36;
constexpr int REC = 64, NZL = 8;
constexpr int COOP_ROW = 172;
constexpr int SPEC_SLOTS = 9;
__host__ __device__ inline size_t coop_gtot_offset(int H, int Ppad) { return (size_t)2 * 2 * SPEC_SLOTS * part_stride(H) * Ppad; }
__host__ __device__ inline size_t coop_pp_stride(int H, int Ppad) { return coop_gtot_offset(H, Ppad) + 4 * (size_t)part_stride(H); }

DI Smem carve(float* base, int H, int m, int team, bool coop = false, bool ust_lds = true) {
    Smem s;
    float* p = base;
    s.W3 = p; p += 6 * HID;
    s.w3n = p; p += HID;
    s.b1n = p; p += HID;
    s.b2 = p; p += HID;
    s.b1d = p; p += HID;
    s.W1zT = p; p += NN * 2 * HID;
    s.W1uT = p; p += m * HID;
    s.A2 = p; p += HID * HID;
    s.A2T = p; p += HID * HID;
    s.A2h = p; p += 512 + 512;
    s.A2x = s.A2; s.A2xT = s.A2 + 3 * 2 * 64 * 4;
    s.dt = p; p += (H + 3) & ~3;
    s.sdt = p; p += (H * NN + 3) & ~3;
    s.disc = p; p += (H + 1 + 3) & ~3;
    const int nv = (H * m + 3) & ~3;
    const int per_team = (ust_lds ? H * UST : 0) + (((H + 1) * NX + 3) & ~3) + 16 + 6 * nv;
    p += team * per_team;
    s.ust = p; if (ust_lds) p += H * UST;
    s.xref = p; p += ((H + 1) * NX + 3) & ~3;
    s.red = p; p += 16;
    for (int i = 0; i < 6; ++i) { s.v[i] = p; p += nv; }
    s.tot = p;
    s.rec = s.tot + ((H * 12 + 3) & ~3); s.nzl = s.rec + H * REC; s.cend = s.nzl + 4 * H * NZL;
    s.nzs = nullptr;
    (void)coop;
    return s;
}
__host__ __device__ inline size_t smem_floats(int H, int m, int ipb, bool coop = false, bool ust_lds = true) {
    size_t shared = 6 * HID + 4 * HID + NN * 2 * HID + (size_t)m * HID + 2 * HID * HID + 1024 + ((H + 3) & ~3) + ((H * NN + 3) & ~3) + ((H + 1 + 3) & ~3);
    size_t per_team = (ust_lds ? (size_t)H * UST : 0) + (((H + 1) * NX + 3) & ~3) + 16 + 6 * (size_t)((H * m + 3) & ~3);
    return shared + ipb * per_team + (coop ? (size_t)((H * 12 + 3) & ~3) + (size_t)H * REC + (size_t)4 * H * NZL : 0);
}
inline size_t smem_bytes(int H, int m, int ipb, bool coop = false, bool ust_lds = true, int nz_waves = 0) {
    return (smem_floats(H, m, ipb, coop, ust_lds) + (size_t)nz_waves * NZ_STAGE) * sizeof(float);
}

constexpr int OFF_SF = blob::SF;
constexpr int OFF_W1Z = blob::W1Z, OFF_B1 = blob::B1, OFF_W1U = blob::W1U, OFF_W2 = blob::W2, OFF_B2 = blob::B2,
              OFF_W3 = blob::W3, OFF_B3 = blob::B3, OFF_W3N = blob::W3N, OFF_B3N = blob::B3N;

constexpr int BLOB_FLOATS = OFF_B3N + 8;
static_assert(BLOB_FLOATS == 2120, "blob layout (include/sdempc.h: SDEMPC_BLOB_FLOATS)");
constexpr int VJP_BASE = FAST ? BLOB_FLOATS : 0;
DI float fwd_w1(float w) { return FAST ? TANH_PRESCALE * w : w; }
DI float vjp_w3(float w) { return FAST ? -2.0f * w : w; }

struct WaveW {
    float w1d[3], w1n[3];
    half8 h1d, h1n;
};

DI int opaque_s(int v) { asm volatile("" : "+s"(v)); return v; }
DI int opaque_v(int v) { asm volatile("" : "+v"(v)); return v; }
DI int rowmap(int r, int h) { return (r & 3) + 8 * (r >> 2) + 4 * h; }

DI void load_adj_images(const KArgs& a, const Smem& sm, const float* w, int tid, int BNT, const AdjOff O, bool with_xt) {
    if (with_xt) {
        unsigned short* axt = reinterpret_cast<unsigned short*>(sm.A2 + O.xt);
        for (int i = tid; i < 2 * 64 * 8; i += BNT) {
            const int e = i & 7, l = (i >> 3) & 63, hf = i >> 9, jj = l & 31, hh = l >> 5, un = rowmap(8 * hf + e, hh);
            const float wv = w[VJP_BASE + OFF_W2 + un * HID + jj];
            const _Float16 h1 = (_Float16)wv;
            const _Float16 h2 = (_Float16)(wv - (float)h1);
            axt[(0 * 2 + hf) * 512 + l * 8 + e] = __builtin_bit_cast(unsigned short, h1);
            axt[(1 * 2 + hf) * 512 + l * 8 + e] = __builtin_bit_cast(unsigned short, h2);
        }
    }
    unsigned short* zd = reinterpret_cast<unsigned short*>(sm.A2 + O.azd);
    unsigned short* zn = reinterpret_cast<unsigned short*>(sm.A2 + O.azn);
    for (int i = tid; i < 2 * 2 * (ZROWS_D + ZROWS_N) * 8; i += BNT) {
        const int e = i & 7, rw = (i >> 3) % (ZROWS_D + ZROWS_N), hh = ((i >> 3) / (ZROWS_D + ZROWS_N)) & 1, hf = ((i >> 3) / (ZROWS_D + ZROWS_N)) >> 1;
        const int un = rowmap(8 * hf + e, hh);
        const bool dr = rw < ZROWS_D;
        const int row = dr ? rw : rw - ZROWS_D;
        float wz = 0.0f;
        if (dr) wz = row < NN ? w[VJP_BASE + OFF_W1Z + un * NN + row] : (row < NN + a.m ? w[VJP_BASE + OFF_W1U + un * 8 + (row - NN)] : 0.0f);
        else if (row < NN) wz = w[VJP_BASE + OFF_W1Z + (HID + un) * NN + row];
        const _Float16 h1 = (_Float16)wz;
        const _Float16 h2 = (_Float16)(wz - (float)h1);
        unsigned short* dst = dr ? zd : zn;
        const int R = dr ? ZROWS_D : ZROWS_N;
        dst[(((0 * 2 + hf) * 2 + hh) * R + row) * 8 + e] = __builtin_bit_cast(unsigned short, h1);
        dst[(((1 * 2 + hf) * 2 + hh) * R + row) * 8 + e] = __builtin_bit_cast(unsigned short, h2);
    }
    unsigned short* a3 = reinterpret_cast<unsigned short*>(sm.A2 + O.a3t);
    for (int i = tid; i < A3T_ROWS * 8; i += BNT) {
        const int e = i & 7, row = i >> 3;
        const float w3v = (row < HID && e < 6) ? w[OFF_W3 + e * HID + row] : 0.0f;
        const _Float16 h1 = (_Float16)w3v;
        const _Float16 h2 = (_Float16)(w3v - (float)h1);
        a3[(0 * A3T_ROWS + row) * 8 + e] = __builtin_bit_cast(unsigned short, h1);
        a3[(1 * A3T_ROWS + row) * 8 + e] = __builtin_bit_cast(unsigned short, h2);
    }
}

DI void load_weights(const KArgs& a, const Smem& sm, WaveW& ww, int tid, int BNT) {
    const float* w = a.wts;
    const int lane = tid & 63, j = lane & 31, h = lane >> 5;
    for (int i = tid; i < 6 * HID; i += BNT) sm.W3[i] = w[OFF_W3 + i];
    for (int i = tid; i < HID; i += BNT) {
        sm.w3n[i] = w[OFF_W3N + i];
        sm.b1d[i] = w[OFF_B1 + i];
        sm.b1n[i] = w[OFF_B1 + HID + i];
        sm.b2[i] = w[OFF_B2 + i];
    }
    for (int i = tid; i < NN * 2 * HID; i += BNT) { int k = i / (2 * HID), r = i % (2 * HID); sm.W1zT[i] = w[VJP_BASE + OFF_W1Z + r * NN + k]; }
    for (int i = tid; i < a.m * HID; i += BNT) { int j = i / HID, r = i % HID; sm.W1uT[i] = w[VJP_BASE + OFF_W1U + r * 8 + j]; }
    for (int i = tid; i < a.H; i += BNT) sm.dt[i] = a.dt[i];
    for (int i = tid; i < a.H * NN; i += BNT) sm.sdt[i] = a.sdt[i];
    for (int i = tid; i <= a.H; i += BNT) sm.disc[i] = a.disc[i];
#pragma unroll
    for (int s = 0; s < 3; ++s) { ww.w1d[s] = w[OFF_W1Z + j * NN + 2 * s + h]; ww.w1n[s] = w[OFF_W1Z + (HID + j) * NN + 2 * s + h]; }
    if (a.f16 == 2) {
        unsigned short* ax = reinterpret_cast<unsigned short*>(sm.A2x);
        unsigned short* axt = reinterpret_cast<unsigned short*>(sm.A2xT);
        for (int i = tid; i < 2 * 64 * 8; i += BNT) {
            const int e = i & 7, l = (i >> 3) & 63, hf = i >> 9, jj = l & 31, hh = l >> 5, un = rowmap(8 * hf + e, hh);
            float wv[2] = {w[OFF_W2 + jj * HID + un], w[VJP_BASE + OFF_W2 + un * HID + jj]};
            if constexpr (FAST) {
#pragma unroll
                for (int tr = 0; tr < 2; ++tr) {
                    unsigned short* dst = tr ? axt : ax;
                    const _Float16 h1 = (_Float16)wv[tr];
                    const _Float16 h2 = (_Float16)(wv[tr] - (float)h1);
                    dst[(0 * 2 + hf) * 512 + l * 8 + e] = __builtin_bit_cast(unsigned short, h1);
                    dst[(1 * 2 + hf) * 512 + l * 8 + e] = __builtin_bit_cast(unsigned short, h2);
                }
            }
#pragma unroll
            for (int tr = FAST ? 2 : 0; tr < 2; ++tr) {
                unsigned short* dst = tr ? axt : ax;
                float rem = wv[tr];
#pragma unroll
                for (int lb = 0; lb < 3; ++lb) {
                    const unsigned hi = __float_as_uint(rem) & 0xFFFF0000u;
                    dst[(lb * 2 + hf) * 512 + l * 8 + e] = (unsigned short)(hi >> 16);
                    rem = rem - __uint_as_float(hi);
                }
            }
        }
        if constexpr (FAST) load_adj_images(a, sm, w, tid, BNT, adj_off(2), false);
    } else if (FAST && a.f16 == 1) {
        load_adj_images(a, sm, w, tid, BNT, adj_off(1), true);
    } else
    for (int i = tid; i < HID * HID; i += BNT) {
        int c = i & 3, l = (i >> 2) & 63, q = i >> 8, jj = l & 31, hh = l >> 5, r = 4 * q + c;
        sm.A2[i] = w[OFF_W2 + jj * HID + rowmap(r, hh)];
        sm.A2T[i] = w[VJP_BASE + OFF_W2 + rowmap(r, hh) * HID + jj];
    }
    if (a.f16 == 1) {
        _Float16* ah = reinterpret_cast<_Float16*>(sm.A2h);
        for (int i = tid; i < 2 * 64 * 8; i += BNT) {
            int e = i & 7, l = (i >> 3) & 63, hf = i >> 9, jj = l & 31, hh = l >> 5;
            ah[i] = (_Float16)w[OFF_W2 + jj * HID + rowmap(8 * hf + e, hh)];
        }
#pragma unroll
        for (int e = 0; e < 8; ++e) {
            ww.h1d[e] = (e < NN && h == 0) ? (_Float16)w[OFF_W1Z + j * NN + e] : (_Float16)0.0f;
            ww.h1n[e] = (e < NN && h == 0) ? (_Float16)w[OFF_W1Z + (HID + j) * NN + e] : (_Float16)0.0f;
        }
    }
}

template <int CTRL>
DI float dpp_f(float v) {
    return __builtin_bit_cast(float, __builtin_amdgcn_update_dpp(0, __builtin_bit_cast(int, v), CTRL, 0xF, 0xF, false));
}
DI float xor32_sum(float v) {
    unsigned a = __builtin_bit_cast(unsigned, v), b;
    asm("v_mov_b32 %0, %1" : "=v"(b) : "v"(a));
    auto r = __builtin_amdgcn_permlane32_swap(a, b, false, false);
    const unsigned r0 = r[0], r1 = r[1];
    return __builtin_bit_cast(float, r0) + __builtin_bit_cast(float, r1);
}
DI float xor16_sum(float v) {
    unsigned a = __builtin_bit_cast(unsigned, v), b;
    asm("v_mov_b32 %0, %1" : "=v"(b) : "v"(a));
    auto r = __builtin_amdgcn_permlane16_swap(a, b, false, false);
    const unsigned r0 = r[0], r1 = r[1];
    return __builtin_bit_cast(float, r0) + __builtin_bit_cast(float, r1);
}
DI float group_bfly32(float v) {
    v = xor16_sum(v);
    v = v + dpp_f<0x128>(v);
    v = v + dpp_f<0x124>(v);
    v = v + dpp_f<0x4E>(v);
    v = v + dpp_f<0xB1>(v);
    return v;
}
DI float wave_bfly64(float v) { return group_bfly32(xor32_sum(v)); }
template <class Team, class F>
DI float team_reduce256(const Smem& sm, int N, int tid, F&& elem) {
    if constexpr (Team::NT != 256 && Team::NT != 64) Team::sync();
    if constexpr (Team::NT >= 256) {
        float acc = 0.0f;
        if (tid < 256)
            for (int e = tid; e < N; e += 256) acc = elem(e, acc);
        acc = wave_bfly64(acc);
        Team::sync();
        if ((tid & 63) == 0 && tid < 256) sm.red[tid >> 6] = acc;
        Team::sync();
        return ((sm.red[0] + sm.red[1]) + sm.red[2]) + sm.red[3];
    } else {
        const int ln = tid & 63;
        float w[4];
#pragma unroll
        for (int vw = 0; vw < 4; ++vw) {
            float acc = 0.0f;
            for (int e = vw * 64 + ln; e < N; e += 256) acc = elem(e, acc);
            w[vw] = wave_bfly64(acc);
        }
        return ((w[0] + w[1]) + w[2]) + w[3];
    }
}
template <class Team>
DI float block_dot(const Smem& sm, const float* x, const float* y, int N, int tid) {
    return team_reduce256<Team>(sm, N, tid, [&](int e, float acc) { return FMA(x[e], y ? y[e] : 1.0f, acc); });
}

DI float slew_dw(const KArgs& a, const float* u, int t, int j, int m, float& cterm) {
    float ds = u[t * m + j] - u[(t - 1) * m + j];
    float c = (a.C.slew * ds) * ds;
    float d = (2.0f * a.C.slew) * ds;
    if (a.C.has_sc) {
        float hi = ds - a.C.slew_hi[j]; hi = hi < 0.0f ? 0.0f : hi;
        float lo = a.C.slew_lo[j] - ds; lo = lo < 0.0f ? 0.0f : lo;
        c = FMA(a.C.slew_cc * hi, hi, c);
        c = FMA(a.C.slew_cc * lo, lo, c);
        d = FMA(2.0f * a.C.slew_cc, hi - lo, d);
    }
    cterm = c;
    return d;
}
DI float ucost_elem(const KArgs& a, const Smem& sm, const float* u, int e, int m) {
    int t = e / m, j = e - t * m;
    float du = u[e] - a.C.uref[j];
    float c = (a.C.uerr * du) * du;
    if (t >= 1) {
        float ds = u[e] - u[e - m];
        c = FMA(a.C.slew * ds, ds, c);
        if (a.C.has_sc) {
            float hi = ds - a.C.slew_hi[j]; hi = hi < 0.0f ? 0.0f : hi;
            float lo = a.C.slew_lo[j] - ds; lo = lo < 0.0f ? 0.0f : lo;
            c = FMA(a.C.slew_cc * hi, hi, c);
            c = FMA(a.C.slew_cc * lo, lo, c);
        }
    }
    return sm.disc[t] * c;
}
template <class Team>
DI float block_ucost(const KArgs& a, const Smem& sm, const float* u, int tid) {
    return team_reduce256<Team>(sm, a.H * a.m, tid, [&](int e, float acc) { return FMA(ucost_elem(a, sm, u, e, a.m), 1.0f, acc); });
}

template <class Team>
DI void block_prepass(const KArgs& a, const Smem& sm, const float* u, int tid) {
    const int H = a.H, m = a.m;
    for (int e = tid; e < H * HID; e += Team::NT) {
        int t = e >> 5, r = e & 31;
        float c = sm.b1d[r];
        for (int j = 0; j < m; ++j) c = FMA(fwd_w1(sm.W1uT[j * HID + r]), u[t * m + j], c);
        sm.ust[t * UST + r] = c;
    }
    for (int t = tid; t < H; t += Team::NT) {
        float Tz = 0.0f, t0 = 0.0f, t1 = 0.0f, t2 = 0.0f;
        for (int j = 0; j < m; ++j) {
            float uj = u[t * m + j];
            float T = FMA(FMA(a.M.ct2, uj, a.M.ct1), uj, a.M.ct0);
            float Mq = a.M.dir[j] * (FMA(a.M.cm2, uj, a.M.cm1) * uj);
            Tz = Tz + T;
            t0 = FMA(a.M.ry[j], T, t0);
            t1 = FMA(-a.M.rx[j], T, t1);
            t2 = t2 + Mq;
        }
        sm.ust[t * UST + 32] = Tz; sm.ust[t * UST + 33] = t0; sm.ust[t * UST + 34] = t1; sm.ust[t * UST + 35] = t2;
    }
}

#include "sdempc_step.inc.h"

DI float group_ordered_sum(const float* rows, int G, int PS, int i) {
    float S0 = 0.0f, S1 = 0.0f, S2 = 0.0f, S3 = 0.0f;
    for (int g = 0; g < G; g += 4) {
        S0 = S0 + rows[(size_t)g * PS + i];
        if (g + 1 < G) S1 = S1 + rows[(size_t)(g + 1) * PS + i];
        if (g + 2 < G) S2 = S2 + rows[(size_t)(g + 2) * PS + i];
        if (g + 3 < G) S3 = S3 + rows[(size_t)(g + 3) * PS + i];
    }
    return ((S0 + S1) + S2) + S3;
}

#include "sdempc_lane.inc.h"

#include "sdempc_lane2.inc.h"

#include "sdempc_coop.inc.h"

#include "sdempc_duo.inc.h"

template <class Team, int F16, bool PK = false>
DI float block_rollout(const KArgs& a, const Smem& sm, const WaveW& ww, const float* u, int b, int tid, bool store_traj, float* xmean_out) {
    b = opaque_s(b); tid = opaque_v(tid);
    const int H = a.H, G = a.G, P = a.P;
    const int lane = tid & 63, j = lane & 31, h = lane >> 5, wave = tid >> 6;
    const bool want_mean = xmean_out != nullptr;
    Team::sync();
    block_prepass<Team>(a, sm, u, tid);
    const int PS = part_stride(H);
    float* prows = a.part + (size_t)b * G * PS;
    float cu = block_ucost<Team>(a, sm, u, tid);
    float x0r[NX];
#pragma unroll
    for (int i = 0; i < NX; ++i) x0r[i] = a.x0[b * NX + i];
    for (int g = wave; g < G; g += Team::NWAVES) {
        const bool valid = (g * 32 + j) < P;
        const float* nz = a.noise + ((size_t)(b * G + g) * H) * NN * 32 + j;
        float* tj = a.traj + ((size_t)(b * G + g) * (H + 1)) * NX * 32 + j;
        float* xm = prows + (size_t)g * PS;
        float x[NX], xn[NX], xi[NN];
#pragma unroll
        for (int i = 0; i < NX; ++i) x[i] = x0r[i];
#pragma unroll
        for (int i = 0; i < NN; ++i) xi[i] = nz[i * 32];
        if (store_traj) {
#pragma unroll
            for (int c = 0; c < 7; ++c) { if (c + 7 * h < NX) tj[(c + 7 * h) * 32] = h ? x[(c + 7) % NX] : x[c]; }
        }
        if (want_mean) {
#pragma unroll
            for (int i = 0; i < NX; ++i) { float s = group_bfly32(valid ? x[i] : 0.0f); if (lane == 0) xm[i] = s; }
        }
        float J = 0.0f;
        StepAux A;
        for (int t = 0; t < H; ++t) {
            float xin[NN];
            if (t + 1 < H) {
#pragma unroll
                for (int i = 0; i < NN; ++i) xin[i] = nz[((t + 1) * NN + i) * 32];
            }
            step_fwd<F16, PK>(a, sm, ww, t, h, lane, x, xi, xn, A);
            float l = stage_cost<false>(a, xn, sm.xref + (t + 1) * NX, nullptr);
            l = FMA(a.C.res_mult * A.eta, A.eta, l);
            J = FMA(sm.disc[t], l, J);
#pragma unroll
            for (int i = 0; i < NX; ++i) x[i] = xn[i];
            if (t + 1 < H) {
#pragma unroll
                for (int i = 0; i < NN; ++i) xi[i] = xin[i];
            }
            if (store_traj) {
                float* tp = tj + (size_t)(t + 1) * NX * 32;
#pragma unroll
                for (int c = 0; c < 7; ++c) { if (c + 7 * h < NX) tp[(c + 7 * h) * 32] = h ? x[(c + 7) % NX] : x[c]; }
            }
            if (want_mean) {
#pragma unroll
                for (int i = 0; i < NX; ++i) { float s = group_bfly32(valid ? x[i] : 0.0f); if (lane == 0) xm[(t + 1) * NX + i] = s; }
            }
        }
        float T = group_bfly32(valid ? J : 0.0f);
        if (lane == 0) xm[PS - 1] = T;
    }
    Team::sync();
    const float tot = group_ordered_sum(prows, G, PS, PS - 1);
    if (want_mean) {
        for (int i = tid; i < (H + 1) * NX; i += Team::NT) xmean_out[i] = group_ordered_sum(prows, G, PS, i) * a.invP;
    }
    return FMA(tot, a.invP, cu);
}

template <class Team, int M, int F16, bool PK = false, bool PREF = true>
DI float block_cost_grad(const KArgs& a, const Smem& sm, const WaveW& ww, const float* y, float* gout, int b, int tid) {
    b = opaque_s(b); tid = opaque_v(tid);
    const int H = a.H, G = a.G, P = a.P, m = a.m;
    constexpr int nq = M + 4;
    const int lane = tid & 63, j = lane & 31, h = lane >> 5, wave = tid >> 6;
    Team::sync();
    block_prepass<Team>(a, sm, y, tid);
    const int PS = part_stride(H);
    float* prows = a.part + (size_t)b * G * PS;
    float cu = block_ucost<Team>(a, sm, y, tid);
    float x0r[NX];
#pragma unroll
    for (int i = 0; i < NX; ++i) x0r[i] = a.x0[b * NX + i];
    for (int g = wave; g < G; g += Team::NWAVES) {
        const bool valid = (g * 32 + j) < P;
        const float* nz = a.noise + ((size_t)(b * G + g) * H) * NN * 32 + j;
        float* tj = a.traj + ((size_t)(b * G + g) * (H + 1)) * NX * 32 + j;
        float* ac = a.act + ((size_t)(b * G + g) * H) * ACT_STRIDE;
        float* Sq = prows + (size_t)g * PS;
        float x[NX], xn[NX], xi[NN];
        StepAux A;
#pragma unroll
        for (int i = 0; i < NX; ++i) x[i] = x0r[i];
#pragma unroll
        for (int i = 0; i < NN; ++i) xi[i] = nz[i * 32];
#pragma unroll
        for (int c = 0; c < 7; ++c) { if (c + 7 * h < NX) tj[(c + 7 * h) * 32] = h ? x[(c + 7) % NX] : x[c]; }
        float J = 0.0f;
        for (int t = 0; t < H; ++t) {
            float xin[NN];
            if (t + 1 < H) {
#pragma unroll
                for (int i = 0; i < NN; ++i) xin[i] = nz[((t + 1) * NN + i) * 32];
            }
            step_fwd<F16, PK>(a, sm, ww, t, h, lane, x, xi, xn, A);
            {
                float* ap = ac + (size_t)t * ACT_STRIDE;
#pragma unroll
                for (int q = 0; q < 4; ++q)
                    *reinterpret_cast<float4*>(ap + (q * 64 + lane) * 4) = make_float4(A.h2[4 * q], A.h2[4 * q + 1], A.h2[4 * q + 2], A.h2[4 * q + 3]);
                if (h == 0) {
                    *reinterpret_cast<float4*>(ap + 1024 + j * 8) = make_float4(A.eta, A.Fb[0], A.Fb[1], A.Fb[2]);
                    ap[1024 + j * 8 + 4] = A.rn;
                }
            }
            float l = stage_cost<false>(a, xn, sm.xref + (t + 1) * NX, nullptr);
            l = FMA(a.C.res_mult * A.eta, A.eta, l);
            J = FMA(sm.disc[t], l, J);
#pragma unroll
            for (int i = 0; i < NX; ++i) x[i] = xn[i];
            if (t + 1 < H) {
#pragma unroll
                for (int i = 0; i < NN; ++i) xi[i] = xin[i];
            }
            float* tp = tj + (size_t)(t + 1) * NX * 32;
#pragma unroll
            for (int c = 0; c < 7; ++c) { if (c + 7 * h < NX) tp[(c + 7 * h) * 32] = h ? x[(c + 7) % NX] : x[c]; }
        }
        { const float T = group_bfly32(valid ? J : 0.0f); if (lane == 0) Sq[PS - 1] = T; }
        float lam[NX], xt[NX];
#pragma unroll
        for (int i = 0; i < NX; ++i) lam[i] = 0.0f;
        __builtin_amdgcn_fence(__ATOMIC_SEQ_CST, "workgroup");
        float4 nh[4], ns4;
        float nrn, nxt[NX], nxi[NN];
        auto issue_loads = [&](int t) {
            const float* ap = ac + (size_t)t * ACT_STRIDE;
#pragma unroll
            for (int q = 0; q < 4; ++q) nh[q] = *reinterpret_cast<const float4*>(ap + (q * 64 + lane) * 4);
            ns4 = *reinterpret_cast<const float4*>(ap + 1024 + j * 8);
            nrn = ap[1024 + j * 8 + 4];
            const float* tp = tj + (size_t)t * NX * 32;
#pragma unroll
            for (int i = 0; i < NX; ++i) nxt[i] = tp[i * 32];
#pragma unroll
            for (int i = 0; i < NN; ++i) nxi[i] = nz[(t * NN + i) * 32];
        };
        if constexpr (PREF) issue_loads(H - 1);
        for (int t = H - 1; t >= 0; --t) {
            if constexpr (!PREF) issue_loads(t);
            f32x16 h2l;
#pragma unroll
            for (int q = 0; q < 4; ++q) { h2l[4 * q] = nh[q].x; h2l[4 * q + 1] = nh[q].y; h2l[4 * q + 2] = nh[q].z; h2l[4 * q + 3] = nh[q].w; }
            const float eta_l = ns4.x, fb0 = ns4.y, fb1 = ns4.z, fb2 = ns4.w, rn_l = nrn;
#pragma unroll
            for (int i = 0; i < NX; ++i) xt[i] = nxt[i];
#pragma unroll
            for (int i = 0; i < NN; ++i) xi[i] = nxi[i];
            if constexpr (PREF) { if (t > 0) issue_loads(t - 1); }
            const float dsc = sm.disc[t];
            {
                float gx[NX];
                stage_cost<true>(a, x, sm.xref + (t + 1) * NX, gx);
#pragma unroll
                for (int i = 0; i < NX; ++i) lam[i] = FMA(dsc, gx[i], lam[i]);
            }
            SCHED_PHASE();
            float lamn[NX], gq[12];
            step_fwd<F16, PK>(a, sm, ww, t, h, lane, xt, xi, xn, A);
            A.h2 = h2l; A.eta = eta_l; A.Fb[0] = fb0; A.Fb[1] = fb1; A.Fb[2] = fb2; A.rn = rn_l;
#pragma unroll
            for (int i = 0; i < 3; ++i) A.Jom[i] = a.M.J[i] * xt[10 + i];
#pragma unroll
            for (int i = 0; i < 4; ++i) A.qn[i] = x[6 + i];
            float ebc = dsc * ((2.0f * a.C.res_mult) * A.eta);
            step_vjp<M, (F16 == 2 || (FAST && F16 == 1)) ? F16 : 0>(a, sm, ww, t, h, lane, xt, xi, A, lam, ebc, lamn, gq);
#pragma unroll
            for (int i = 0; i < NX; ++i) { lam[i] = lamn[i]; x[i] = xt[i]; }
            {
                constexpr int half = (nq + 1) / 2;
#pragma unroll
                for (int k = 0; k < half; ++k) {
                    const float lo = gq[k], hi = (k + half < nq) ? gq[k + half] : 0.0f;
                    float s = group_bfly32(valid ? (h ? hi : lo) : 0.0f);
                    if (j == 0 && (h == 0 || k + half < nq)) {
                        Sq[t * 12 + k + h * half] = s;
                    }
                }
            }
        }
    }
    Team::sync();
    const float tot = group_ordered_sum(prows, G, PS, PS - 1);
    const int N = H * m;
    for (int e = tid; e < N; e += Team::NT) {
        int t = e / m, jj = e - t * m;
        float S[5];
        int idx[5] = {jj, M, M + 1, M + 2, M + 3};
#pragma unroll
        for (int k = 0; k < 5; ++k) {
            S[k] = group_ordered_sum(prows, G, PS, t * 12 + idx[k]);
        }
        float uj = y[e];
        float dT = FMA(2.0f * a.M.ct2, uj, a.M.ct1);
        float dM = a.M.dir[jj] * FMA(2.0f * a.M.cm2, uj, a.M.cm1);
        float acc = S[0];
        acc = FMA(S[1], dT, acc);
        acc = FMA(S[2], a.M.ry[jj] * dT, acc);
        acc = FMA(S[3], -(a.M.rx[jj] * dT), acc);
        acc = FMA(S[4], dM, acc);
        float du = uj - a.C.uref[jj];
        float dw = 0.0f, ctmp;
        if (t >= 1) dw = slew_dw(a, y, t, jj, m, ctmp);
        float gcu = sm.disc[t] * FMA(2.0f * a.C.uerr, du, dw);
        if (t + 1 < H) { float dwn = slew_dw(a, y, t + 1, jj, m, ctmp); gcu = FMA(-sm.disc[t + 1], dwn, gcu); }
        gout[e] = FMA(acc, a.invP, gcu);
    }
    Team::sync();
    return FMA(tot, a.invP, cu);
}

template <class Team, int F16, bool PK, int MODE>
DI float team_rollout(const KArgs& a, const Smem& sm, const WaveW& ww, const LaneW& LW, CoopCtx& CC, const float* u, int b, int tid, bool store_traj, float* xmean_out) {
    if constexpr (MODE >= 3) return duo_rollout<Team, F16, MODE == 3>(a, sm, ww, u, b, tid, store_traj, xmean_out);
    else if constexpr (MODE == 2) return coop_rollout<Team>(a, sm, LW, CC, u, b, tid, xmean_out);
    else if constexpr (MODE == 1) return lane_rollout<Team>(a, sm, LW, u, b, tid, store_traj, xmean_out);
    else return block_rollout<Team, F16, PK>(a, sm, ww, u, b, tid, store_traj, xmean_out);
}
template <class Team, int M, int F16, bool PK, bool PREF, int MODE>
DI float team_cost_grad(const KArgs& a, const Smem& sm, const WaveW& ww, const LaneW& LW, CoopCtx& CC, const float* y, float* gout, int b, int tid) {
    if constexpr (MODE >= 3) return duo_cost_grad<Team, M, F16, MODE == 3>(a, sm, ww, y, gout, b, tid);
    else if constexpr (MODE == 2) return coop_cost_grad<Team, M>(a, sm, LW, CC, y, gout, b, tid);
    else if constexpr (MODE == 1) return lane_cost_grad<Team, M>(a, sm, LW, y, gout, b, tid);
    else return block_cost_grad<Team, M, F16, PK, PREF>(a, sm, ww, y, gout, b, tid);
}

template <class Team>
DI void load_common(const KArgs& a, const Smem& sm, int b, int tid) {
    for (int i = tid; i < (a.H + 1) * NX; i += Team::NT) sm.xref[i] = a.xref[(size_t)b * (a.H + 1) * NX + i];
}

#define SDEMPC_KERNEL_PROLOGUE(USTG_)                                                \
    extern __shared__ __attribute__((aligned(16))) float smem[];                     \
    LaneW LW;                                                                        \
    CoopCtx CC;                                                                      \
    const int tid = Team::tid();                                                     \
    int b_;                                                                          \
    if constexpr (MODE == 2) {                                                       \
        b_ = blockIdx.x / a.coop_nwg;                                                \
        CC.nwg = a.coop_nwg; CC.wgi = blockIdx.x - b_ * a.coop_nwg; CC.Ppad = a.G * 32; CC.epoch = 0u; CC.spin_limit = a.coop_spin; CC.fence = a.opt.coop_fence; \
        CC.bar = a.coop_bar + COOP_BAR_WORDS * b_;                                              \
        CC.pp = a.coop_pp + (size_t)b_ * coop_pp_stride(a.H, CC.Ppad);               \
        CC.gtot = reinterpret_cast<unsigned long long*>(CC.pp + coop_gtot_offset(a.H, CC.Ppad)); \
        CC.ck = a.coop_ck + (size_t)b_ * a.P * (a.H + 1) * COOP_ROW;                 \
    } else {                                                                         \
        b_ = blockIdx.x * Team::IPB + Team::team();                                  \
    }                                                                                \
    const int b = __builtin_amdgcn_readfirstlane(b_);                                \
    Smem sm = carve(smem, a.H, a.m, Team::team(), MODE == 2, !(USTG_));              \
    if constexpr (USTG_) sm.ust = a.ustg + (size_t)b * a.H * UST;                    \
    WaveW ww;                                                                        \
    load_weights(a, sm, ww, threadIdx.x, Team::BNT);                                 \
    __syncthreads();                                                                 \
    if (b >= a.B) return;  \
    if constexpr (MODE == 2) { if ((int)blockIdx.x == a.opt.absent_wg) return; }  \
    if constexpr (MODE == 1) load_lane_weights(a, LW, threadIdx.x & 63);              \
    load_common<Team>(a, sm, b, tid);                                                \
    if constexpr (MODE == 2) {                                                       \
        __syncthreads(); lane2_stage<Team>(a, sm, b, CC.wgi, tid);                   \
        if (CC.wgi == 0)    \
            for (int i = tid; i < 2 * part_stride(a.H); i += Team::NT) __hip_atomic_store(CC.gtot + i, 0ull, __ATOMIC_RELAXED, __HIP_MEMORY_SCOPE_AGENT); \
    }

template <class Team, int F16, int MODE = 0>
__global__ void __launch_bounds__(Team::BNT, (MODE ? 2 : 3)) sdempc_rollout_kernel(KArgs a) {
    SDEMPC_KERNEL_PROLOGUE(false);
    const int N = a.H * a.m;
    for (int e = tid; e < N; e += Team::NT) sm.v[5][e] = a.u[(size_t)b * N + e];
    float c = team_rollout<Team, F16, false, MODE>(a, sm, ww, LW, CC, sm.v[5], b, tid, a.store_traj != 0, a.xmean ? a.xmean + (size_t)b * (a.H + 1) * NX : nullptr);
    if (tid == 0) a.cost[b] = c;
}

template <class Team, int M, int F16, int MODE = 0>
__global__ void __launch_bounds__(Team::BNT, (MODE ? 2 : 3)) sdempc_grad_kernel(KArgs a) {
    SDEMPC_KERNEL_PROLOGUE(false);
    const int N = a.H * a.m;
    for (int e = tid; e < N; e += Team::NT) sm.v[5][e] = a.u[(size_t)b * N + e];
    float c = team_cost_grad<Team, M, F16, false, false, MODE>(a, sm, ww, LW, CC, sm.v[5], sm.v[3], b, tid);
    if (tid == 0) a.cost[b] = c;
    for (int e = tid; e < N; e += Team::NT) a.grad[(size_t)b * N + e] = sm.v[3][e];
}

template <class Team, bool PK> constexpr int solve_waves_per_simd() { return PK ? 2 : 3; }
template <class Team, int M, int F16, bool PK, int MODE>
DI void solve_instance(const KArgs& a, const Smem& sm, const WaveW& ww, const LaneW& LW, CoopCtx& CC, const int b, const int tid) {
    const int m = a.m, N = a.H * m;
    float *xk = sm.v[0], *yk = sm.v[1], *xn = sm.v[2], *g = sm.v[3], *d1 = sm.v[4], *d2 = sm.v[5];
    for (int e = tid; e < N; e += Team::NT) {
        int jj = e % m;
        float v = clampf(a.u[(size_t)b * N + e], a.C.ulo[jj], a.C.uhi[jj]);
        xk[e] = v; yk[e] = v;
    }
#if SDEMPC_VAR_PHASE_CLK
    if ((threadIdx.x & 63) == 0) for (int i = 0; i < 8; ++i) sdempc_clk[threadIdx.x >> 6][i] = 0ull;
#endif
    CLK_BEGIN(t_solve);
    const float c_init = uni_f(team_rollout<Team, F16, PK, MODE>(a, sm, ww, LW, CC, xk, b, tid, false, nullptr));
    float c_x = c_init, s = a.stepsize_in[b], gsq = 0.0f, sum_ls = 0.0f, sum_s = 0.0f;
    int kr = 0, noimp = 0, nit = 0, nls_tot = 0, plain = 1;
    int yk_unchanged = 0, ngrad = 0;
    float c_y = 0.0f;
    for (int k = 0; k < a.A.max_iter; ++k) {
        c_x = uni_f(c_x); s = uni_f(s); sum_ls = uni_f(sum_ls); sum_s = uni_f(sum_s); c_y = uni_f(c_y); gsq = uni_f(gsq);
        if (!yk_unchanged) {
            c_y = uni_f(team_cost_grad<Team, M, F16, PK, solve_waves_per_simd<Team, PK>() == 2, MODE>(a, sm, ww, LW, CC, yk, g, b, tid));
            gsq = uni_f(block_dot<Team>(sm, g, g, N, tid));
            ngrad += 1;
        }
        if (!(gsq < __builtin_inff())) break;
        float c_n = 0.0f;
        int nls = 0;
        if (a.A.maxls > 0) {
            if (k > 0 && a.A.reset_inc) s = s * a.A.inc;
            if (s > a.A.smax) s = a.A.smax;
            for (int jl = 0; jl < a.A.maxls; ++jl) {
                Team::sync();
                for (int e = tid; e < N; e += Team::NT) {
                    int jj = e % m;
                    float v = clampf(FMA(-s, g[e], yk[e]), a.C.ulo[jj], a.C.uhi[jj]);
                    xn[e] = v; d1[e] = v - yk[e];
                }
                c_n = uni_f(team_rollout<Team, F16, PK, MODE>(a, sm, ww, LW, CC, xn, b, tid, false, nullptr));
                float gd = uni_f(block_dot<Team>(sm, g, d1, N, tid));
                nls = jl + 1;
                if (c_n <= FMA(a.A.coef, gd, c_y)) break;
                if (jl < a.A.maxls - 1) s = s * a.A.dec;
            }
        } else {
            s = a.A.stepsize;
            Team::sync();
            for (int e = tid; e < N; e += Team::NT) { int jj = e % m; xn[e] = clampf(FMA(-s, g[e], yk[e]), a.C.ulo[jj], a.C.uhi[jj]); }
            c_n = uni_f(team_rollout<Team, F16, PK, MODE>(a, sm, ww, LW, CC, xn, b, tid, false, nullptr));
            nls = 1;
        }
        sum_ls = sum_ls + (float)nls; sum_s = sum_s + s; nit = k + 1; nls_tot += nls;
        int stop = (__builtin_fabsf(c_n - c_x) <= FMA(a.A.rtol, __builtin_fabsf(c_x), a.A.atol));
        Team::sync();
        yk_unchanged = plain && !(c_n < c_x);
        if (c_n < c_x) {
            for (int e = tid; e < N; e += Team::NT) { d1[e] = yk[e] - xn[e]; d2[e] = xn[e] - xk[e]; }
            float rs = uni_f(block_dot<Team>(sm, d1, d2, N, tid));
            if (rs > 0.0f) {
                kr = 0; plain = 1;
                for (int e = tid; e < N; e += Team::NT) { yk[e] = xn[e]; xk[e] = xn[e]; }
            } else {
                float bt = a.beta[kr];
                for (int e = tid; e < N; e += Team::NT) { int jj = e % m; yk[e] = clampf(FMA(bt, d2[e], xn[e]), a.C.ulo[jj], a.C.uhi[jj]); xk[e] = xn[e]; }
                kr = kr + 1; plain = 0;
            }
            c_x = c_n; noimp = 0;
        } else {
            if (!plain) stop = 0;
            kr = 0; plain = 1;
            for (int e = tid; e < N; e += Team::NT) yk[e] = xk[e];
            noimp = noimp + 1;
        }
        if (noimp >= a.A.max_noimp) stop = 1;
        if (stop) break;
    }
    Team::sync();
    if (MODE != 2 || CC.wgi == 0)
        for (int e = tid; e < N; e += Team::NT) a.uopt[(size_t)b * N + e] = xk[e];
    team_rollout<Team, F16, PK, MODE>(a, sm, ww, LW, CC, xk, b, tid, false, a.xmean + (size_t)b * (a.H + 1) * NX);
#if SDEMPC_VAR_PHASE_CLK
    CLK_END(0, t_solve);
    if (a.work && (threadIdx.x & 63) == 0) {
        const unsigned long long* c = sdempc_clk[threadIdx.x >> 6];
        __hip_atomic_fetch_add(a.work + 0, ((c[0] >> 10) << 32) | (c[1] >> 10), __ATOMIC_RELAXED, __HIP_MEMORY_SCOPE_AGENT);
        if (tid == 0) __hip_atomic_fetch_add(a.work + 1, (unsigned long long)ngrad, __ATOMIC_RELAXED, __HIP_MEMORY_SCOPE_AGENT);
        __hip_atomic_fetch_add(a.work + 2, ((c[4] >> 10) << 32) | (c[5] >> 10), __ATOMIC_RELAXED, __HIP_MEMORY_SCOPE_AGENT);
        __hip_atomic_fetch_add(a.work + 3, ((c[6] >> 10) << 32) | 1ull, __ATOMIC_RELAXED, __HIP_MEMORY_SCOPE_AGENT);
    }
#endif
    if (tid == 0 && (MODE != 2 || CC.wgi == 0)) {
        float* inf = a.info + (size_t)b * 8;
        const float fn = (float)nit;
        inf[0] = nit ? sum_ls / fn : 0.0f; inf[1] = s; inf[2] = fn; inf[3] = gsq; inf[4] = nit ? sum_s / fn : 0.0f;
        inf[5] = c_init; inf[6] = c_x; inf[7] = (float)nls_tot;
        if (a.work && !SDEMPC_VAR_PHASE_CLK) {
            __hip_atomic_fetch_add(a.work + 0, 1ull, __ATOMIC_RELAXED, __HIP_MEMORY_SCOPE_AGENT);
            __hip_atomic_fetch_add(a.work + 1, (unsigned long long)ngrad, __ATOMIC_RELAXED, __HIP_MEMORY_SCOPE_AGENT);
            __hip_atomic_fetch_add(a.work + 2, (unsigned long long)(nls_tot + 2), __ATOMIC_RELAXED, __HIP_MEMORY_SCOPE_AGENT);
        }
#if SDEMPC_VAR_PHASE_CLK
        inf[0] = __uint_as_float(__builtin_amdgcn_s_getreg(63492));
        inf[1] = __uint_as_float(__builtin_amdgcn_s_getreg(63508));
        inf[3] = (float)(unsigned)(t_solve & 0x3FFFFFFFull) * 1e-5f;
        inf[4] = (float)(clk_now() - t_solve) * 1e-5f;
#endif
        if constexpr (MODE == 2) {
            if (__hip_atomic_load(CC.bar + 1, __ATOMIC_RELAXED, __HIP_MEMORY_SCOPE_AGENT) != 0u)
                for (int i = 0; i < 8; ++i) inf[i] = __builtin_nanf("");
        }
    }
}

template <class Team, int M, int F16, bool PK = false, int MODE = 0, bool USTG = false>
__global__ void __launch_bounds__(Team::BNT, (MODE == 2 && PK ? 1 : (MODE == 1 || MODE == 2) ? 2 : solve_waves_per_simd<Team, PK>())) sdempc_solve_kernel(KArgs a) {
    if constexpr (MODE >= 3) {
        extern __shared__ __attribute__((aligned(16))) float smem[];
        LaneW LW;
        CoopCtx CC;
        const int tid = Team::tid();
        Smem sm = carve(smem, a.H, a.m, Team::team(), false, !USTG);
        if constexpr (MODE == 3) sm.nzs = smem + smem_floats(a.H, a.m, Team::IPB, false, !USTG) + __builtin_amdgcn_readfirstlane(threadIdx.x >> 6) * NZ_STAGE;
        WaveW ww;
        if constexpr (Team::IPB > 1) { if (threadIdx.x < Team::IPB) sdempc_pair_bar[threadIdx.x] = 0u; }
        load_weights(a, sm, ww, threadIdx.x, Team::BNT);
        __syncthreads();
        unsigned* ticket = a.tickets ? reinterpret_cast<unsigned*>(a.work + 4) : nullptr;
        const unsigned nteams = gridDim.x * Team::IPB, ndraw = (unsigned)a.B - nteams;
        int bb = blockIdx.x * Team::IPB + Team::team();
        while (bb < a.B) {
            const int b = __builtin_amdgcn_readfirstlane(bb);
            if constexpr (USTG) sm.ust = a.ustg + (size_t)duo_workspace_slot<Team>() * a.H * UST;
            Team::sync();
            load_common<Team>(a, sm, b, tid);
            solve_instance<Team, M, F16, PK, MODE>(a, sm, ww, LW, CC, b, tid);
            if (ticket) {
                Team::sync();
                if (tid == 0) reinterpret_cast<unsigned*>(sm.red)[0] = __hip_atomic_fetch_add(ticket, 1u, __ATOMIC_RELAXED, __HIP_MEMORY_SCOPE_AGENT) - a.ticket_base;
                Team::sync();
                const unsigned t = (unsigned)__builtin_amdgcn_readfirstlane((int)reinterpret_cast<const unsigned*>(sm.red)[0]);
                bb = t < ndraw ? (int)(nteams + t) : a.B;
            } else {
                bb += gridDim.x * Team::IPB;
            }
        }
        return;
    }
    SDEMPC_KERNEL_PROLOGUE(USTG);
    solve_instance<Team, M, F16, PK, MODE>(a, sm, ww, LW, CC, b, tid);
}

template <bool LIMITED = false, class F>
static hipError_t with_m(int m, F&& f) {
    if (m == 4) return f(std::integral_constant<int, 4>{});
    if (m == 6) return f(std::integral_constant<int, 6>{});
    if constexpr (!LIMITED || SDEMPC_ALL_VARIANTS) return f(std::integral_constant<int, 8>{});
    else return hipErrorInvalidValue;
}
static constexpr bool every_layout_built(int m) { return m == 4 || m == 6 || SDEMPC_ALL_VARIANTS != 0; }
template <class F>
static hipError_t with_f16(int f16, F&& f) {
    if (f16 == 2) return f(std::integral_constant<int, 2>{});
    return f16 ? f(std::integral_constant<int, 1>{}) : f(std::integral_constant<int, 0>{});
}

#define SDEMPC_DUO_M(X, TEAM, M)                                                                                   \
    X(TEAM, M, 0, 3, false) X(TEAM, M, 1, 3, false) X(TEAM, M, 2, 3, false) X(TEAM, M, 0, 3, true) X(TEAM, M, 1, 3, true) X(TEAM, M, 2, 3, true)  \
    X(TEAM, M, 0, 4, true) X(TEAM, M, 1, 4, true) X(TEAM, M, 2, 4, true)
#if SDEMPC_ALL_VARIANTS
#define SDEMPC_DUO_M8(X, TEAM) SDEMPC_DUO_M(X, TEAM, 8)
#define SDEMPC_DUO_T8(X, TEAM) X(TEAM, 8, 0, 3, false) X(TEAM, 8, 1, 3, false) X(TEAM, 8, 2, 3, false)
#else
#define SDEMPC_DUO_M8(X, TEAM)
#define SDEMPC_DUO_T8(X, TEAM)
#endif
#define SDEMPC_DUO_TEAM(X, TEAM) SDEMPC_DUO_M(X, TEAM, 4) SDEMPC_DUO_M(X, TEAM, 6) SDEMPC_DUO_M8(X, TEAM)
#define SDEMPC_DUO_PAIR(X)                                                                                          \
    X(TeamPair, 4, 0, 3, false) X(TeamPair, 4, 1, 3, false) X(TeamPair, 4, 2, 3, false) X(TeamPair, 6, 0, 3, false) X(TeamPair, 6, 1, 3, false) X(TeamPair, 6, 2, 3, false) \
    SDEMPC_DUO_T8(X, TeamPair)
#define SDEMPC_DUO_HEX(X)                                                                                           \
    X(TeamHex, 4, 0, 3, false) X(TeamHex, 4, 1, 3, false) X(TeamHex, 4, 2, 3, false) X(TeamHex, 6, 0, 3, false) X(TeamHex, 6, 1, 3, false) X(TeamHex, 6, 2, 3, false) \
    SDEMPC_DUO_T8(X, TeamHex)
#define SDEMPC_DUO_DECL(TEAM, M, F16, MODE, USTG) extern template __global__ void sdempc_solve_kernel<TEAM, M, F16, false, MODE, USTG>(KArgs);
#define SDEMPC_DUO_DEF(TEAM, M, F16, MODE, USTG) template __global__ void sdempc_solve_kernel<TEAM, M, F16, false, MODE, USTG>(KArgs);

#if SDEMPC_TU == 1
SDEMPC_DUO_PAIR(SDEMPC_DUO_DEF)
SDEMPC_DUO_TEAM(SDEMPC_DUO_DEF, TeamBlock2)
}
#elif SDEMPC_TU == 2
SDEMPC_DUO_TEAM(SDEMPC_DUO_DEF, TeamBlock)
}
#elif SDEMPC_TU == 3
SDEMPC_DUO_HEX(SDEMPC_DUO_DEF)
}
#elif SDEMPC_TU == 4
#include "sdempc_loop.inc.h"
}
#if !SDEMPC_FAST
namespace fastm {
hipError_t launch_loop(const KArgs& a, const LoopAdvance& L, const LoopPlant* Q, const LoopPeriod* R, const LoopScenario* C, const LoopRate* W, hipStream_t st);
}
hipError_t launch_loop(const KArgs& a, const LoopAdvance& L, const LoopPlant* Q, const LoopPeriod* R, const LoopScenario* C, const LoopRate* W, hipStream_t st) {
    return a.fast ? fastm::launch_loop(a, L, Q, R, C, W, st) : exact::launch_loop(a, L, Q, R, C, W, st);
}
#endif
#else
SDEMPC_DUO_PAIR(SDEMPC_DUO_DECL)
SDEMPC_DUO_HEX(SDEMPC_DUO_DECL)
SDEMPC_DUO_TEAM(SDEMPC_DUO_DECL, TeamBlock2)
SDEMPC_DUO_TEAM(SDEMPC_DUO_DECL, TeamBlock)

#include "sdempc_spec.inc.h"

#if SDEMPC_DEV_KERNEL
#if SDEMPC_DEV_KERNEL == 1
template __global__ void sdempc_solve_spec_kernel<4, false>(KArgs);
#elif SDEMPC_DEV_KERNEL == 2
template __global__ void sdempc_solve_spec_kernel<4, true>(KArgs);
#elif SDEMPC_DEV_KERNEL == 3
template __global__ void sdempc_solve_kernel<TeamBlock, 4, false, true, 2>(KArgs);
#elif SDEMPC_DEV_KERNEL == 4
template __global__ void sdempc_solve_kernel<TeamWave, 4, false, false, 1>(KArgs);
#endif
}
#else
static hipError_t set_smem_attr(const void* fn, size_t bytes) {
    if (bytes > 64 * 1024) return hipFuncSetAttribute(fn, hipFuncAttributeMaxDynamicSharedMemorySize, (int)bytes);
    return hipSuccess;
}
static bool use_wave_team(int G, int H, int m) { return G == 1 && smem_bytes(H, m, TeamWave::IPB) <= 80 * 1024; }
int team_ipb(int G, int H, int m) { return use_wave_team(G, H, m) ? TeamWave::IPB : TeamBlock::IPB; }

template <class Kern>
static hipError_t launch_k(Kern k, const KArgs& a, hipStream_t st, int ipb, int bnt = 256, bool ust_lds = true) {
    const size_t sb = smem_bytes(a.H, a.m, ipb, false, ust_lds);
    hipError_t e = set_smem_attr((const void*)k, sb);
    if (e != hipSuccess) return e;
    note_kernel((const void*)k);
    hipLaunchKernelGGL(k, dim3((a.B + ipb - 1) / ipb), dim3(bnt), sb, st, a);
    return hipGetLastError();
}
template <class Team>
static hipError_t launch_rollout_team(const KArgs& a, hipStream_t st) {
    return with_f16(a.f16, [&](auto F16) { return launch_k(sdempc_rollout_kernel<Team, F16>, a, st, Team::IPB); });
}
template <class Team, int F16>
static hipError_t launch_grad_team(const KArgs& a, hipStream_t st) {
    return with_m(a.m, [&](auto M) { return launch_k(sdempc_grad_kernel<Team, M, F16>, a, st, Team::IPB); });
}
bool use_global_ust(int H, int m, const LaunchOpts& o, int nwaves = 4) {
    if (o.ustg >= 0) return o.ustg == 1;
    const size_t cap = 156 * 1024, by_regs = 12 / (size_t)nwaves;
    auto per_cu = [&](size_t bytes) { const size_t n = bytes ? cap / bytes : by_regs; return n > by_regs ? by_regs : n; };
    return per_cu(smem_bytes(H, m, 1, false, false)) > per_cu(smem_bytes(H, m, 1));
}
template <class Kern>
static hipError_t launch_persistent(Kern k, const KArgs& a, hipStream_t st, int wg_waves, int bnt, bool ust_lds, int ipb = 1, bool stage = true) {
    const size_t sb = smem_bytes(a.H, a.m, ipb, false, ust_lds, stage ? wg_waves : 0);
    hipError_t e = set_smem_attr((const void*)k, sb);
    if (e != hipSuccess) return e;
    size_t per_cu = 12 / (size_t)wg_waves;
    const size_t by_lds = (156 * 1024) / (sb ? sb : 1);
    if (by_lds < per_cu) per_cu = by_lds;
    if (per_cu < 1) per_cu = 1;
    size_t grid = per_cu * (size_t)(a.opt.cus > 0 ? a.opt.cus : 256);
    const size_t need = ((size_t)a.B + ipb - 1) / ipb;
    if (grid > need) grid = need;
    if (a.ws_rows > 0 && grid * (size_t)ipb > (size_t)a.ws_rows) return hipErrorInvalidValue;
    KArgs ka = a;
    ka.tickets = a.work != nullptr && a.ticket_host != nullptr && (size_t)a.B >= 3 * grid * (size_t)ipb;
    if (ka.tickets) ka.ticket_base = *a.ticket_host;
    note_kernel((const void*)k);
    hipLaunchKernelGGL(k, dim3((unsigned)grid), dim3(bnt), sb, st, ka);
    e = hipGetLastError();
    if (e == hipSuccess && ka.tickets) *a.ticket_host = ka.ticket_base + (unsigned)a.B;
    return e;
}
template <class TeamD, int M, int F16>
static hipError_t launch_duo_m(const KArgs& a, hipStream_t st) {
    constexpr int W = TeamD::NWAVES;
    const size_t cap = 156 * 1024, by_regs = 12 / (size_t)W;
    auto per_cu = [&](bool ust_lds, bool stage) { const size_t n = cap / smem_bytes(a.H, a.m, 1, false, ust_lds, stage ? W : 0); return n > by_regs ? by_regs : n; };
    const bool can_g = a.ustg != nullptr && a.opt.ustg != 0, must_g = can_g && a.opt.ustg == 1;
    int pick = 0;
    size_t best = must_g ? 0 : per_cu(true, true);
    if (must_g) pick = 1, best = per_cu(false, true);
    else if (can_g && per_cu(false, true) > best) pick = 1, best = per_cu(false, true);
    if (can_g && per_cu(false, false) > best) pick = 2;
    if (pick == 2) return launch_persistent(sdempc_solve_kernel<TeamD, M, F16, false, 4, true>, a, st, W, TeamD::BNT, false, 1, false);
    if (pick == 1) return launch_persistent(sdempc_solve_kernel<TeamD, M, F16, false, 3, true>, a, st, W, TeamD::BNT, false);
    return launch_persistent(sdempc_solve_kernel<TeamD, M, F16, false, 3, false>, a, st, W, TeamD::BNT, true);
}
template <int M, int F16>
static hipError_t launch_duo_small(const KArgs& a, hipStream_t st) {
    const int cus = a.opt.cus > 0 ? a.opt.cus : 256;
    if (a.opt.ustg != 1 && a.opt.hex != 0 && a.B >= 6 * cus && smem_bytes(a.H, a.m, TeamHex::IPB, false, true, 2 * TeamHex::IPB) <= 156 * 1024)
        return launch_persistent(sdempc_solve_kernel<TeamHex, M, F16, false, 3, false>, a, st, 2 * TeamHex::IPB, TeamHex::BNT, true, TeamHex::IPB);
    if (a.opt.ustg != 1 && smem_bytes(a.H, a.m, 2, false, true, 4) * 3 <= 156 * 1024)
        return launch_persistent(sdempc_solve_kernel<TeamPair, M, F16, false, 3, false>, a, st, 4, TeamPair::BNT, true, 2);
    return launch_duo_m<TeamBlock2, M, F16>(a, st);
}
template <int F16>
static hipError_t launch_duo(const KArgs& a, hipStream_t st) {
    return with_m<true>(a.m, [&](auto M) { return a.G <= 4 ? launch_duo_small<M, F16>(a, st) : launch_duo_m<TeamBlock, M, F16>(a, st); });
}
static bool one_group_per_wave_batch(const KArgs& a, int B) {
    if (a.opt.duo >= 0 || a.G > 4) return false;
    if (!every_layout_built(a.m)) return false;
    const bool gtab = use_global_ust(a.H, a.m, a.opt) && a.ustg;
    size_t per_cu = (156 * 1024) / smem_bytes(a.H, a.m, 1, false, !gtab);
    if (per_cu > 3) per_cu = 3;
    return (size_t)B <= per_cu * (size_t)(a.opt.cus > 0 ? a.opt.cus : 256);
}
static bool takes_pk(const KArgs& a, int B) {
    if (!SDEMPC_ALL_VARIANTS || a.f16 != 0 || FAST) return false;
    const int ipb = team_ipb(a.G, a.H, a.m), wgs = (B + ipb - 1) / ipb;
    return a.opt.pk >= 0 ? a.opt.pk == 1 : wgs <= a.opt.cus;
}
static bool takes_duo(const KArgs& a, int B) {
    return a.G >= 2 && a.opt.duo != 0 && every_layout_built(a.m) && !one_group_per_wave_batch(a, B);
}
template <class Team, int F16>
static hipError_t launch_solve_team(const KArgs& a, hipStream_t st) {
#if SDEMPC_ALL_VARIANTS
    if constexpr (F16 == 0 && !FAST) {
        if (takes_pk(a, a.B)) {
            if (a.G > 4)
                return with_m(a.m, [&](auto M) { return launch_k(sdempc_solve_kernel<TeamBlock8, M, 0, true>, a, st, 1, TeamBlock8::BNT); });
            return with_m(a.m, [&](auto M) { return launch_k(sdempc_solve_kernel<Team, M, 0, true>, a, st, Team::IPB); });
        }
    }
#endif
    if constexpr (Team::IPB == 1) {
        if (takes_duo(a, a.B)) return launch_duo<F16>(a, st);
        if (use_global_ust(a.H, a.m, a.opt) && a.ustg && every_layout_built(a.m))
            return with_m<true>(a.m, [&](auto M) { return launch_k(sdempc_solve_kernel<Team, M, F16, false, 0, true>, a, st, 1, Team::BNT, false); });
    }
    return with_m(a.m, [&](auto M) { return launch_k(sdempc_solve_kernel<Team, M, F16>, a, st, Team::IPB); });
}
static bool use_lane(const KArgs& k) {
    if (k.f16 || k.P != 1 || k.C.sc_n != 0 || !use_wave_team(k.G, k.H, k.m)) return false;
    return k.opt.lane != 0;
}
template <int M>
static hipError_t launch_lane(int what, const KArgs& k, hipStream_t st) {
    if (what == 0) return launch_k(sdempc_rollout_kernel<TeamWave, false, 1>, k, st, TeamWave::IPB);
    if (what == 1) return launch_k(sdempc_grad_kernel<TeamWave, M, false, 1>, k, st, TeamWave::IPB);
    return launch_k(sdempc_solve_kernel<TeamWave, M, false, false, 1>, k, st, TeamWave::IPB);
}
static hipError_t launch_lane_m(int what, const KArgs& k, hipStream_t st) {
    return with_m(k.m, [&](auto M) { return launch_lane<M>(what, k, st); });
}
int coop_nwg(int P) { return (P + 3) / 4; }
int coop_max_instances(int P, int H, int m, const LaunchOpts& o) {
    if (!o.coop || P < 2 || o.cus < 16 || !every_layout_built(m)) return 0;
    if (smem_bytes(H, m, 1, true) > 160 * 1024) return 0;
    return (2 * o.cus - 16) / coop_nwg(P);
}
size_t coop_pp_floats(int H, int G) { return coop_pp_stride(H, G * 32); }
size_t coop_ck_floats(int H, int P) { return (size_t)SPEC_CKS * P * (H + 1) * COOP_ROW; }
int spec_max_instances(int P, int H, int m, const LaunchOpts& o) {
    if (!o.spec || !o.coop || !every_layout_built(m)) return 0;
    const size_t nv = (size_t)((H * m + 3) & ~3);
    if (smem_bytes(H, m, 1, true) + (SPEC_XV * nv + SPEC_MRED) * sizeof(float) > 160 * 1024) return 0;
    return o.cus / (2 * coop_nwg(P));
}
template <class K>
static hipError_t launch_resident(K kern, dim3 grid, dim3 block, size_t sb, hipStream_t st, const KArgs& k) {
    note_kernel((const void*)kern);
    if (k.opt.coop_launch == 1) {
        KArgs kk = k;
        void* args[] = {(void*)&kk};
        const hipError_t rc = hipLaunchCooperativeKernel((const void*)kern, grid, block, args, (unsigned)sb, st);
        if (rc == hipSuccess) return rc;
        (void)hipGetLastError();
        if (rc != hipErrorCooperativeLaunchTooLarge && rc != hipErrorNotSupported && rc != hipErrorInvalidConfiguration) return rc;
    }
    hipLaunchKernelGGL(kern, grid, block, sb, st, k);
    return hipGetLastError();
}
template <int M>
static hipError_t launch_spec_m(const KArgs& k, hipStream_t st) {
    auto kern = k.P == 1 ? sdempc_solve_spec_kernel<M, true> : sdempc_solve_spec_kernel<M, false>;
    const size_t sb = smem_bytes(k.H, k.m, 1, true) + (SPEC_XV * (size_t)((k.H * k.m + 3) & ~3) + SPEC_MRED) * sizeof(float);
    hipError_t e = set_smem_attr((const void*)kern, sb);
    if (e != hipSuccess) return e;
    return launch_resident(kern, dim3(k.B * k.coop_ngrp * k.coop_nwg), dim3(TeamBlock::BNT), sb, st, k);
}
hipError_t launch_solve_spec(const KArgs& a, int B, hipStream_t st) {
    KArgs k = a; k.B = B; k.coop_nwg = coop_nwg(k.P);
    if (B < 1 || B > (spec_max_instances)(k.P, k.H, k.m, k.opt) || !k.coop_bar || !k.coop_pp || !k.coop_ck) return hipErrorInvalidValue;
    k.coop_ngrp = k.opt.cus / (B * k.coop_nwg);
    if (k.coop_ngrp > SPEC_GROUPS) k.coop_ngrp = SPEC_GROUPS;
    return with_m<true>(k.m, [&](auto M) { return launch_spec_m<M>(k, st); });
}
template <int M>
static hipError_t launch_coop_m(const KArgs& k, hipStream_t st) {
    const size_t sb = smem_bytes(k.H, k.m, 1, true);
    if (k.B * k.coop_nwg <= k.opt.cus) {
        auto kern = sdempc_solve_kernel<TeamBlock, M, false, true, 2>;
        hipError_t e = set_smem_attr((const void*)kern, sb);
        if (e != hipSuccess) return e;
        return launch_resident(kern, dim3(k.B * k.coop_nwg), dim3(TeamBlock::BNT), sb, st, k);
    }
    auto kern = sdempc_solve_kernel<TeamBlock, M, false, false, 2>;
    hipError_t e = set_smem_attr((const void*)kern, sb);
    if (e != hipSuccess) return e;
    return launch_resident(kern, dim3(k.B * k.coop_nwg), dim3(TeamBlock::BNT), sb, st, k);
}
hipError_t launch_solve_coop(const KArgs& a, int B, hipStream_t st) {
    KArgs k = a; k.B = B; k.coop_nwg = coop_nwg(k.P);
    if (B < 1 || B > (coop_max_instances)(k.P, k.H, k.m, k.opt) || !k.coop_bar || !k.coop_pp || !k.coop_ck) return hipErrorInvalidValue;
    return with_m<true>(k.m, [&](auto M) { return launch_coop_m<M>(k, st); });
}

int solve_workspace_rows(const KArgs& k, int B) {
    if (use_wave_team(k.G, k.H, k.m) || takes_pk(k, B) || !takes_duo(k, B)) return B;
    const int slots = 6 * (k.opt.cus > 0 ? k.opt.cus : 256), even = (B + 1) & ~1;
    return even < slots ? even : slots;
}
hipError_t launch_rollout(const KArgs& a, int B, hipStream_t st) {
    KArgs k = a; k.B = B;
    if (use_lane(k)) return launch_lane_m(0, k, st);
    return use_wave_team(k.G, k.H, k.m) ? launch_rollout_team<TeamWave>(k, st) : launch_rollout_team<TeamBlock>(k, st);
}
hipError_t launch_grad(const KArgs& a, int B, hipStream_t st) {
    KArgs k = a; k.B = B;
    if (use_lane(k)) return launch_lane_m(1, k, st);
    const bool wave = use_wave_team(k.G, k.H, k.m);
    return with_f16(k.f16, [&](auto F16) { return wave ? launch_grad_team<TeamWave, F16>(k, st) : launch_grad_team<TeamBlock, F16>(k, st); });
}
hipError_t launch_solve(const KArgs& a, int B, hipStream_t st) {
    KArgs k = a; k.B = B;
    if (use_lane(k)) return launch_lane_m(2, k, st);
    const bool wave = use_wave_team(k.G, k.H, k.m);
    return with_f16(k.f16, [&](auto F16) { return wave ? launch_solve_team<TeamWave, F16>(k, st) : launch_solve_team<TeamBlock, F16>(k, st); });
}

template <bool TO_DEV>
__global__ void __launch_bounds__(256) sdempc_relayout_kernel(const float* __restrict__ in, float* __restrict__ out, int P, int G, int C) {
    __shared__ float tile[32][33];
    const int c0 = blockIdx.x * 32, g = blockIdx.y, b = blockIdx.z;
    const int tx = threadIdx.x & 31, ty = threadIdx.x >> 5;
    if (TO_DEV) {
        for (int r = ty; r < 32; r += 8) {
            const int p = g * 32 + r, c = c0 + tx;
            tile[r][tx] = (p < P && c < C) ? in[((size_t)b * P + p) * C + c] : 0.0f;
        }
        __syncthreads();
        for (int r = ty; r < 32; r += 8) {
            const int c = c0 + r;
            if (c < C) out[(((size_t)b * G + g) * C + c) * 32 + tx] = tile[tx][r];
        }
    } else {
        for (int r = ty; r < 32; r += 8) {
            const int c = c0 + r;
            tile[r][tx] = c < C ? in[(((size_t)b * G + g) * C + c) * 32 + tx] : 0.0f;
        }
        __syncthreads();
        for (int r = ty; r < 32; r += 8) {
            const int p = g * 32 + r, c = c0 + tx;
            if (p < P && c < C) out[((size_t)b * P + p) * C + c] = tile[tx][r];
        }
    }
}
hipError_t launch_relayout(bool to_dev, const float* in, float* out, int B, int P, int G, int C, hipStream_t st) {
    if (B < 1 || G < 1 || G > 65535 || C < 1 || P < 1 || P > G * 32) return hipErrorInvalidValue;
    const size_t canon = (size_t)P * C, dev = (size_t)G * C * 32;
    for (int b0 = 0; b0 < B; b0 += 65535) {
        const int nb = B - b0 < 65535 ? B - b0 : 65535;
        dim3 grid((C + 31) / 32, G, nb);
        if (to_dev) sdempc_relayout_kernel<true><<<grid, 256, 0, st>>>(in + b0 * canon, out + b0 * dev, P, G, C);
        else sdempc_relayout_kernel<false><<<grid, 256, 0, st>>>(in + b0 * dev, out + b0 * canon, P, G, C);
    }
    return hipGetLastError();
}

#if SDEMPC_FAST
}
#else
}
namespace fastm {
hipError_t launch_rollout(const KArgs& a, int B, hipStream_t st);
hipError_t launch_grad(const KArgs& a, int B, hipStream_t st);
hipError_t launch_solve(const KArgs& a, int B, hipStream_t st);
int solve_workspace_rows(const KArgs& a, int B);
hipError_t launch_solve_coop(const KArgs& a, int B, hipStream_t st);
hipError_t launch_solve_spec(const KArgs& a, int B, hipStream_t st);
}
static thread_local const void* g_last_kernel_fn = nullptr;
void note_kernel(const void* host_fn) { g_last_kernel_fn = host_fn; }
const void* last_launched_kernel() { return g_last_kernel_fn; }
size_t smem_bytes(int H, int m, int ipb) { return exact::smem_bytes(H, m, ipb); }
int team_ipb(int G, int H, int m) { return exact::team_ipb(G, H, m); }
hipError_t launch_rollout(const KArgs& a, int B, hipStream_t st) { return a.fast ? fastm::launch_rollout(a, B, st) : exact::launch_rollout(a, B, st); }
hipError_t launch_grad(const KArgs& a, int B, hipStream_t st) { return a.fast ? fastm::launch_grad(a, B, st) : exact::launch_grad(a, B, st); }
hipError_t launch_solve(const KArgs& a, int B, hipStream_t st) { return a.fast ? fastm::launch_solve(a, B, st) : exact::launch_solve(a, B, st); }
int solve_workspace_rows(const KArgs& a, int B) { return a.fast ? fastm::solve_workspace_rows(a, B) : exact::solve_workspace_rows(a, B); }
int coop_nwg(int P) { return exact::coop_nwg(P); }
int coop_max_instances(int P, int H, int m, const LaunchOpts& o) { return exact::coop_max_instances(P, H, m, o); }
size_t coop_pp_floats(int H, int G) { return exact::coop_pp_floats(H, G); }
size_t coop_ck_floats(int H, int P) { return exact::coop_ck_floats(H, P); }
hipError_t launch_solve_coop(const KArgs& a, int B, hipStream_t st) { return a.fast ? fastm::launch_solve_coop(a, B, st) : exact::launch_solve_coop(a, B, st); }
int spec_max_instances(int P, int H, int m, const LaunchOpts& o) { return exact::spec_max_instances(P, H, m, o); }
hipError_t launch_solve_spec(const KArgs& a, int B, hipStream_t st) { return a.fast ? fastm::launch_solve_spec(a, B, st) : exact::launch_solve_spec(a, B, st); }
hipError_t launch_relayout(bool to_dev, const float* in, float* out, int B, int P, int G, int C, hipStream_t st) {
    return exact::launch_relayout(to_dev, in, out, B, P, G, C, st);
}
#endif
#endif
#endif

}
```

Measured before the change: 4625.

## Prefetch adjoint trajectory and noise rows into wider LDS staging via DMA

Adds a wide per-wave LDS staging area (12 rows instead of 6) for the fast, matrix-pipe duo solve kernel. During the backward adjoint sweep, trajectory rows 3..12 and two noise rows for step t-1 are loaded with global_load_lds while step t computes, replacing direct global loads on the critical path. Writes of the per-step reduced sums are deferred by one iteration. A host-side plan picks the wide layout only when it does not reduce workgroups per CU, and the plan is exposed through a new ABI query.

```diff
diff --git a/include/sdempc.h b/include/sdempc.h
--- a/include/sdempc.h
+++ b/include/sdempc.h
@@ -78,6 +78,7 @@
 int sdempc_abi_version(void);
 #define SDEMPC_BUILD_ALL_VARIANTS 1
 int sdempc_build_flags(void);
+int sdempc_duo_stage_plan(int32_t H, int32_t m, int32_t ipb, int32_t wg_waves, int32_t ust_lds, int32_t math_fast, int32_t mlp_dtype, int64_t out[4]);
 
 int sdempc_set_device(sdempc_handle* h, int32_t device);
 
diff --git a/sde4mbrl_px4_amd/_abi.py b/sde4mbrl_px4_amd/_abi.py
--- a/sde4mbrl_px4_amd/_abi.py
+++ b/sde4mbrl_px4_amd/_abi.py
@@ -202,6 +202,18 @@
     return fn
 
 
+def duo_stage_plan(lib, H, m, ipb, wg_waves, ust_lds=True, math_mode="exact", mlp_dtype="f32"):
+    fn = lib.sdempc_duo_stage_plan
+    if fn.argtypes is None:
+        fn.argtypes = [C.c_int32] * 7 + [C.POINTER(C.c_int64)]
+        fn.restype = C.c_int
+    out = (C.c_int64 * 4)()
+    rc = fn(H, m, ipb, wg_waves, int(bool(ust_lds)), int(math_mode == "fast"), {"f32": 0, "f16": 1, "f32x3": 2}[mlp_dtype], out)
+    if rc != 0:
+        raise ValueError(f"sdempc_duo_stage_plan: {rc}")
+    return dict(rows=int(out[0]), bytes=int(out[1]), per_cu=int(out[2]), per_cu_narrow=int(out[3]))
+
+
 EXPORTED_SYMBOLS = [
     "sdempc_create", "sdempc_destroy", "sdempc_last_error", "sdempc_abi_version", "sdempc_build_flags", "sdempc_set_device", "sdempc_device_ready", "sdempc_set_option", "sdempc_get_option", "sdempc_reset",
     "sdempc_rollout_batch", "sdempc_grad_batch", "sdempc_solve_batch", "sdempc_noise_dev_floats",
@@ -209,5 +221,5 @@
     "sdempc_grad_batch_dev", "sdempc_last_kernel_ms", "sdempc_last_kernel_name", "sdempc_work_counters", "sdempc_solve_status", "sdempc_layout_fallbacks", "sdempc_noise_to_device_layout_dev", "sdempc_traj_to_canonical_dev",
     "sdempc_noise_from_keys_dev", "sdempc_noise_from_keys", "sdempc_solve_batch_keys", "sdempc_closed_loop_batch",
     "sdempc_closed_loop_batch_plant", "sdempc_closed_loop_batch_timed", "sdempc_closed_loop_batch_scenario",
-    "sdempc_closed_loop_batch_rate",
+    "sdempc_closed_loop_batch_rate", "sdempc_duo_stage_plan",
 ]
diff --git a/sde4mbrl_px4_amd/csrc/sdempc_api.cpp b/sde4mbrl_px4_amd/csrc/sdempc_api.cpp
--- a/sde4mbrl_px4_amd/csrc/sdempc_api.cpp
+++ b/sde4mbrl_px4_amd/csrc/sdempc_api.cpp
@@ -500,6 +500,14 @@
 
 int sdempc_abi_version(void) { return SDEMPC_ABI_VERSION; }
 int sdempc_build_flags(void) { return SDEMPC_ALL_VARIANTS ? SDEMPC_BUILD_ALL_VARIANTS : 0; }
+int sdempc_duo_stage_plan(int32_t H, int32_t m, int32_t ipb, int32_t wg_waves, int32_t ust_lds, int32_t math_fast, int32_t mlp_dtype, int64_t out[4]) {
+    return guarded(nullptr, [&]() -> int {
+    if (H < 1 || m < 1 || m > 8 || ipb < 1 || wg_waves < 1 || wg_waves > 12 || mlp_dtype < 0 || mlp_dtype > 2 || !out) return SDEMPC_EINVAL;
+    const DuoStagePlan p = duo_stage_plan(H, m, ipb, wg_waves, ust_lds != 0, math_fast != 0, mlp_dtype);
+    out[0] = p.rows; out[1] = (int64_t)p.bytes; out[2] = p.per_cu; out[3] = p.per_cu_narrow;
+    return SDEMPC_OK;
+    });
+}
 
 const char* sdempc_last_error(const sdempc_handle* h) { return h ? h->err.c_str() : g_create_error.c_str(); }
 
diff --git a/sde4mbrl_px4_amd/csrc/sdempc_duo.inc.h b/sde4mbrl_px4_amd/csrc/sdempc_duo.inc.h
--- a/sde4mbrl_px4_amd/csrc/sdempc_duo.inc.h
+++ b/sde4mbrl_px4_amd/csrc/sdempc_duo.inc.h
@@ -46,26 +46,56 @@
     else __builtin_amdgcn_s_setprio(2);
 }
 
-DI void duo_noise_request(const float* nzb, unsigned nzo, int t, const float* stage) {
-    const float* rows = nzb + (size_t)t * (NN * 32);
+#define DUO_DMA_ROW0(V, S) "s_mov_b32 m0, %[m]\n\ts_nop 0\n\tglobal_load_lds_dword " V ", " S "\n\t"
+#define DUO_DMA_ROW(V, S, OFS) "s_add_u32 m0, m0, 0x80\n\ts_nop 0\n\tglobal_load_lds_dword " V ", " S " offset:" #OFS "\n\t"
+template <int NA>
+DI void duo_rows_request(const float* rowsA, unsigned offA, const float* rowsB, unsigned offB, const float* stage) {
+    static_assert(NA == 6 || NA == 4, "row splits in use");
     const unsigned m0 = (unsigned)__builtin_amdgcn_readfirstlane((int)(unsigned)(size_t)(const __attribute__((address_space(3))) float*)stage);
     unsigned m0_keep;
-    asm volatile(
-        "s_mov_b32 %0, m0\n\t"
-        "s_mov_b32 m0, %3\n\ts_nop 0\n\tglobal_load_lds_dword %1, %2\n\t"
-        "s_add_u32 m0, m0, 0x80\n\ts_nop 0\n\tglobal_load_lds_dword %1, %2 offset:128\n\t"
-        "s_add_u32 m0, m0, 0x80\n\ts_nop 0\n\tglobal_load_lds_dword %1, %2 offset:256\n\t"
-        "s_add_u32 m0, m0, 0x80\n\ts_nop 0\n\tglobal_load_lds_dword %1, %2 offset:384\n\t"
-        "s_add_u32 m0, m0, 0x80\n\ts_nop 0\n\tglobal_load_lds_dword %1, %2 offset:512\n\t"
-        "s_add_u32 m0, m0, 0x80\n\ts_nop 0\n\tglobal_load_lds_dword %1, %2 offset:640\n\t"
-        "s_mov_b32 m0, %0"
-        : "=&s"(m0_keep) : "v"(nzo * 4u), "s"(rows), "s"(m0) : "memory", "scc");
+    if constexpr (NA == 6) {
+        asm volatile(
+            "s_mov_b32 %[k], m0\n\t"
+            DUO_DMA_ROW0("%[oa]", "%[ba]") DUO_DMA_ROW("%[oa]", "%[ba]", 128) DUO_DMA_ROW("%[oa]", "%[ba]", 256)
+            DUO_DMA_ROW("%[oa]", "%[ba]", 384) DUO_DMA_ROW("%[oa]", "%[ba]", 512) DUO_DMA_ROW("%[oa]", "%[ba]", 640)
+            "s_mov_b32 m0, %[k]"
+            : [k] "=&s"(m0_keep) : [oa] "v"(offA), [ba] "s"(rowsA), [m] "s"(m0) : "memory", "scc");
+    } else {
+        const float* rb = rowsB - NA * 32;
+        asm volatile(
+            "s_mov_b32 %[k], m0\n\t"
+            DUO_DMA_ROW0("%[oa]", "%[ba]") DUO_DMA_ROW("%[oa]", "%[ba]", 128) DUO_DMA_ROW("%[oa]", "%[ba]", 256)
+            DUO_DMA_ROW("%[oa]", "%[ba]", 384) DUO_DMA_ROW("%[ob]", "%[bb]", 512) DUO_DMA_ROW("%[ob]", "%[bb]", 640)
+            "s_mov_b32 m0, %[k]"
+            : [k] "=&s"(m0_keep) : [oa] "v"(offA), [ba] "s"(rowsA), [ob] "v"(offB), [bb] "s"(rb), [m] "s"(m0) : "memory", "scc");
+    }
+}
+#undef DUO_DMA_ROW0
+#undef DUO_DMA_ROW
+DI void duo_noise_request(const float* nzb, unsigned nzo, int t, const float* stage) {
+    duo_rows_request<6>(nzb + (size_t)t * (NN * 32), nzo * 4u, nullptr, 0u, stage);
 }
 template <int PENDING>
 DI void duo_noise_take(const float* stage, int lane, float* xi) {
     asm volatile("s_waitcnt vmcnt(%0)" ::"n"(PENDING) : "memory");
 #pragma unroll
     for (int i = 0; i < NN; ++i) xi[i] = stage[i * 64 + lane];
+}
+
+constexpr int ADJ_X0 = 3, ADJ_NX = NX - ADJ_X0, ADJ_NXI = 2;
+static_assert(ADJ_NX + ADJ_NXI == 12 && ADJ_NX == 10, "two six-row blocks: x rows 3..8, then x rows 9..12 and two noise rows");
+DI void duo_adj_request(const float* tjb, unsigned tjo, const float* nzb, unsigned nzo, int t, float* stage) {
+    const float* xr = tjb + (size_t)(t * NX + ADJ_X0) * 32;
+    duo_rows_request<6>(xr, tjo * 4u, nullptr, 0u, stage);
+    duo_rows_request<4>(xr + 6 * 32, tjo * 4u, nzb + (size_t)t * (NN * 32), nzo * 4u, stage + 6 * 64);
+}
+template <int PENDING>
+DI void duo_adj_take(const float* stage, int lane, float* xt, float* xi) {
+    asm volatile("s_waitcnt vmcnt(%0)" ::"n"(PENDING) : "memory");
+#pragma unroll
+    for (int i = 0; i < ADJ_NX; ++i) xt[ADJ_X0 + i] = stage[i * 64 + lane];
+#pragma unroll
+    for (int i = 0; i < ADJ_NXI; ++i) xi[i] = stage[(ADJ_NX + i) * 64 + lane];
 }
 
 template <int F16, bool CKPT, bool NZS>
@@ -203,7 +233,7 @@
     return FMA(tot, a.invP, cu);
 }
 
-template <class Team, int M, int F16, bool NZS>
+template <class Team, int M, int F16, bool NZS, bool WIDE>
 DI float duo_cost_grad(const KArgs& a, const Smem& sm, const WaveW& ww, const float* y, float* gout, int b, int tid) {
     b = opaque_s(b); tid = opaque_v(tid);
     const int H = a.H, G = a.G, P = a.P;
@@ -289,8 +319,23 @@
 #pragma unroll
         for (int i = 0; i < NX; ++i) lam[i] = 0.0f;
         __builtin_amdgcn_fence(__ATOMIC_SEQ_CST, "workgroup");
+        static_assert(!WIDE || (NZS && FAST && F16 != 0), "the wide area is a staging area of the matrix-pipe adjoint");
+        constexpr bool wide = WIDE;
+        float sq[nq];
+        if (wide) {
+            duo_adj_request(tjb, tjo, nzb, nzo, H - 1, sm.nzs);
+            asm volatile("s_waitcnt vmcnt(0)" ::: "memory");
+        }
         for (int t = H - 1; t >= 0; --t) {
             duo_rotate_priority();
+            if (wide) {
+                if (pr.hasB) duo_adj_take<4>(sm.nzs, lane, xt, xi);
+                else duo_adj_take<0>(sm.nzs, lane, xt, xi);
+                if (t < H - 1) {
+#pragma unroll
+                    for (int k = 0; k < nq; ++k) { if (j == 0 && pr.own) Sq[(t + 1) * 12 + k] = sq[k]; }
+                }
+            }
             const float* apA = acA + (size_t)t * ACT_STRIDE;
             const float* apB = acB + (size_t)t * ACT_STRIDE;
             float4 hA[4], hB[4];
@@ -306,7 +351,12 @@
             const unsigned so = aso + (unsigned)(t * ACT_STRIDE);
             const float4 ns4 = *reinterpret_cast<const float4*>(acA + so);
             const float nrn = acA[so + 4];
-            {
+            if (wide) {
+#pragma unroll
+                for (int i = 0; i < ADJ_X0; ++i) xt[i] = tjb[tjo + (unsigned)((t * NX + i) * 32)];
+#pragma unroll
+                for (int i = ADJ_NXI; i < NN; ++i) xi[i] = nzb[nzo + (unsigned)((t * NN + i) * 32)];
+            } else {
 #pragma unroll
                 for (int i = 0; i < NX; ++i) xt[i] = tjb[tjo + (unsigned)((t * NX + i) * 32)];
 #pragma unroll
@@ -370,6 +420,11 @@
                 if constexpr (NZS) {
 #pragma unroll
                     for (int k = 0; k < NN; ++k) zB[k] = sm.nzs[k * 64 + lane];
+                    if (wide && t > 0) {
+#pragma unroll
+                        for (int k = 0; k < NN; ++k) asm volatile("" : "+v"(zB[k]));
+                        duo_adj_request(tjb, tjo, nzb, nzo, t - 1, sm.nzs);
+                    }
                 }
                 if (pr.hasB) adj_mlp_pass_mp<NR, true, F16>(sm, ww, ust, h, lane, zB, hB, eB, OB, rB, [&]() {
 #pragma unroll
@@ -420,8 +475,13 @@
 #pragma unroll
             for (int k = 0; k < nq; ++k) {
                 const float s = group_bfly32(valid ? gq[k] : 0.0f);
-                if (j == 0 && pr.own) Sq[t * 12 + k] = s;
-            }
+                if (wide) sq[k] = s;
+                else if (j == 0 && pr.own) Sq[t * 12 + k] = s;
+            }
+        }
+        if (wide) {
+#pragma unroll
+            for (int k = 0; k < nq; ++k) { if (j == 0 && pr.own) Sq[k] = sq[k]; }
         }
         CLK_END(5, t_adj);
     }
diff --git a/sde4mbrl_px4_amd/csrc/sdempc_kernels.h b/sde4mbrl_px4_amd/csrc/sdempc_kernels.h
--- a/sde4mbrl_px4_amd/csrc/sdempc_kernels.h
+++ b/sde4mbrl_px4_amd/csrc/sdempc_kernels.h
@@ -97,6 +97,8 @@
 __host__ __device__ inline int part_stride(int H) { const int a = H * 12, b = (H + 1) * 13; return ((a > b ? a : b) + 1 + 3) & ~3; }
 constexpr int ACT_STRIDE = 1280;
 size_t smem_bytes(int H, int m, int ipb);
+struct DuoStagePlan { int rows; size_t bytes; int per_cu, per_cu_narrow; };
+DuoStagePlan duo_stage_plan(int H, int m, int ipb, int wg_waves, bool ust_lds, bool fast, int f16);
 void note_kernel(const void* host_fn);
 const void* last_launched_kernel();
 int coop_nwg(int P);
diff --git a/sde4mbrl_px4_amd/csrc/sdempc_kernels.hip b/sde4mbrl_px4_amd/csrc/sdempc_kernels.hip
--- a/sde4mbrl_px4_amd/csrc/sdempc_kernels.hip
+++ b/sde4mbrl_px4_amd/csrc/sdempc_kernels.hip
@@ -104,7 +104,7 @@
     float *v[6];
     float *nzs;
 };
-constexpr int NZ_STAGE = 6 * 64;
+constexpr int NZ_ROWS = 6, NZ_ROWS_WIDE = 12;
 constexpr int ZROWS_D = 15, ZROWS_N = 7;
 constexpr int A3T_ROWS = 33;
 struct AdjOff { int xt, azd, azn, a3t; };
@@ -153,8 +153,8 @@
     size_t per_team = (ust_lds ? (size_t)H * UST : 0) + (((H + 1) * NX + 3) & ~3) + 16 + 6 * (size_t)((H * m + 3) & ~3);
     return shared + ipb * per_team + (coop ? (size_t)((H * 12 + 3) & ~3) + (size_t)H * REC + (size_t)4 * H * NZL : 0);
 }
-inline size_t smem_bytes(int H, int m, int ipb, bool coop = false, bool ust_lds = true, int nz_waves = 0) {
-    return (smem_floats(H, m, ipb, coop, ust_lds) + (size_t)nz_waves * NZ_STAGE) * sizeof(float);
+inline size_t smem_bytes(int H, int m, int ipb, bool coop = false, bool ust_lds = true, int nz_waves = 0, int nz_rows = NZ_ROWS) {
+    return (smem_floats(H, m, ipb, coop, ust_lds) + (size_t)nz_waves * nz_rows * 64) * sizeof(float);
 }
 
 constexpr int OFF_SF = blob::SF;
@@ -650,9 +650,9 @@
     else if constexpr (MODE == 1) return lane_rollout<Team>(a, sm, LW, u, b, tid, store_traj, xmean_out);
     else return block_rollout<Team, F16, PK>(a, sm, ww, u, b, tid, store_traj, xmean_out);
 }
-template <class Team, int M, int F16, bool PK, bool PREF, int MODE>
+template <class Team, int M, int F16, bool PK, bool PREF, int MODE, bool WIDE = false>
 DI float team_cost_grad(const KArgs& a, const Smem& sm, const WaveW& ww, const LaneW& LW, CoopCtx& CC, const float* y, float* gout, int b, int tid) {
-    if constexpr (MODE >= 3) return duo_cost_grad<Team, M, F16, MODE == 3>(a, sm, ww, y, gout, b, tid);
+    if constexpr (MODE >= 3) return duo_cost_grad<Team, M, F16, MODE == 3, WIDE>(a, sm, ww, y, gout, b, tid);
     else if constexpr (MODE == 2) return coop_cost_grad<Team, M>(a, sm, LW, CC, y, gout, b, tid);
     else if constexpr (MODE == 1) return lane_cost_grad<Team, M>(a, sm, LW, y, gout, b, tid);
     else return block_cost_grad<Team, M, F16, PK, PREF>(a, sm, ww, y, gout, b, tid);
@@ -715,7 +715,7 @@
 }
 
 template <class Team, bool PK> constexpr int solve_waves_per_simd() { return PK ? 2 : 3; }
-template <class Team, int M, int F16, bool PK, int MODE>
+template <class Team, int M, int F16, bool PK, int MODE, bool WIDE = false>
 DI void solve_instance(const KArgs& a, const Smem& sm, const WaveW& ww, const LaneW& LW, CoopCtx& CC, const int b, const int tid) {
     const int m = a.m, N = a.H * m;
     float *xk = sm.v[0], *yk = sm.v[1], *xn = sm.v[2], *g = sm.v[3], *d1 = sm.v[4], *d2 = sm.v[5];
@@ -736,7 +736,7 @@
     for (int k = 0; k < a.A.max_iter; ++k) {
         c_x = uni_f(c_x); s = uni_f(s); sum_ls = uni_f(sum_ls); sum_s = uni_f(sum_s); c_y = uni_f(c_y); gsq = uni_f(gsq);
         if (!yk_unchanged) {
-            c_y = uni_f(team_cost_grad<Team, M, F16, PK, solve_waves_per_simd<Team, PK>() == 2, MODE>(a, sm, ww, LW, CC, yk, g, b, tid));
+            c_y = uni_f(team_cost_grad<Team, M, F16, PK, solve_waves_per_simd<Team, PK>() == 2, MODE, WIDE>(a, sm, ww, LW, CC, yk, g, b, tid));
             gsq = uni_f(block_dot<Team>(sm, g, g, N, tid));
             ngrad += 1;
         }
@@ -828,15 +828,15 @@
     }
 }
 
-template <class Team, int M, int F16, bool PK = false, int MODE = 0, bool USTG = false>
-__global__ void __launch_bounds__(Team::BNT, (MODE == 2 && PK ? 1 : (MODE == 1 || MODE == 2) ? 2 : solve_waves_per_simd<Team, PK>())) sdempc_solve_kernel(KArgs a) {
+template <class Team, int M, int F16, bool PK, int MODE, bool USTG, bool WIDE>
+DI void solve_kernel_body(const KArgs& a) {
     if constexpr (MODE >= 3) {
         extern __shared__ __attribute__((aligned(16))) float smem[];
         LaneW LW;
         CoopCtx CC;
         const int tid = Team::tid();
         Smem sm = carve(smem, a.H, a.m, Team::team(), false, !USTG);
-        if constexpr (MODE == 3) sm.nzs = smem + smem_floats(a.H, a.m, Team::IPB, false, !USTG) + __builtin_amdgcn_readfirstlane(threadIdx.x >> 6) * NZ_STAGE;
+        if constexpr (MODE == 3) sm.nzs = smem + smem_floats(a.H, a.m, Team::IPB, false, !USTG) + __builtin_amdgcn_readfirstlane(threadIdx.x >> 6) * ((WIDE ? NZ_ROWS_WIDE : NZ_ROWS) * 64);
         WaveW ww;
         if constexpr (Team::IPB > 1) { if (threadIdx.x < Team::IPB) sdempc_pair_bar[threadIdx.x] = 0u; }
         load_weights(a, sm, ww, threadIdx.x, Team::BNT);
@@ -849,7 +849,7 @@
             if constexpr (USTG) sm.ust = a.ustg + (size_t)duo_workspace_slot<Team>() * a.H * UST;
             Team::sync();
             load_common<Team>(a, sm, b, tid);
-            solve_instance<Team, M, F16, PK, MODE>(a, sm, ww, LW, CC, b, tid);
+            solve_instance<Team, M, F16, PK, MODE, WIDE>(a, sm, ww, LW, CC, b, tid);
             if (ticket) {
                 Team::sync();
                 if (tid == 0) reinterpret_cast<unsigned*>(sm.red)[0] = __hip_atomic_fetch_add(ticket, 1u, __ATOMIC_RELAXED, __HIP_MEMORY_SCOPE_AGENT) - a.ticket_base;
@@ -863,7 +863,19 @@
         return;
     }
     SDEMPC_KERNEL_PROLOGUE(USTG);
-    solve_instance<Team, M, F16, PK, MODE>(a, sm, ww, LW, CC, b, tid);
+    solve_instance<Team, M, F16, PK, MODE, WIDE>(a, sm, ww, LW, CC, b, tid);
+}
+template <class Team, int M, int F16, bool PK = false, int MODE = 0, bool USTG = false>
+__global__ void __launch_bounds__(Team::BNT, (MODE == 2 && PK ? 1 : (MODE == 1 || MODE == 2) ? 2 : solve_waves_per_simd<Team, PK>())) sdempc_solve_kernel(KArgs a) {
+    solve_kernel_body<Team, M, F16, PK, MODE, USTG, false>(a);
+}
+struct WideStage {};
+using SolveKern = void (*)(KArgs);
+using SolveKernWide = void (*)(KArgs, WideStage);
+template <class Team, int M, int F16, bool PK, int MODE, bool USTG>
+__global__ void __launch_bounds__(Team::BNT, (solve_waves_per_simd<Team, PK>())) sdempc_solve_kernel(KArgs a, WideStage) {
+    static_assert(MODE == 3 && !PK, "duo layout with staging areas");
+    solve_kernel_body<Team, M, F16, PK, MODE, USTG, true>(a);
 }
 
 template <bool LIMITED = false, class F>
@@ -880,12 +892,18 @@
     return f16 ? f(std::integral_constant<int, 1>{}) : f(std::integral_constant<int, 0>{});
 }
 
+#if SDEMPC_FAST
+#define SDEMPC_DUO_WIDE(X, TEAM, M, USTG) X##_WIDE(TEAM, M, 1, USTG) X##_WIDE(TEAM, M, 2, USTG)
+#else
+#define SDEMPC_DUO_WIDE(X, TEAM, M, USTG)
+#endif
 #define SDEMPC_DUO_M(X, TEAM, M)                                                                                   \
     X(TEAM, M, 0, 3, false) X(TEAM, M, 1, 3, false) X(TEAM, M, 2, 3, false) X(TEAM, M, 0, 3, true) X(TEAM, M, 1, 3, true) X(TEAM, M, 2, 3, true)  \
+    SDEMPC_DUO_WIDE(X, TEAM, M, false) SDEMPC_DUO_WIDE(X, TEAM, M, true)  \
     X(TEAM, M, 0, 4, true) X(TEAM, M, 1, 4, true) X(TEAM, M, 2, 4, true)
 #if SDEMPC_ALL_VARIANTS
 #define SDEMPC_DUO_M8(X, TEAM) SDEMPC_DUO_M(X, TEAM, 8)
-#define SDEMPC_DUO_T8(X, TEAM) X(TEAM, 8, 0, 3, false) X(TEAM, 8, 1, 3, false) X(TEAM, 8, 2, 3, false)
+#define SDEMPC_DUO_T8(X, TEAM) X(TEAM, 8, 0, 3, false) X(TEAM, 8, 1, 3, false) X(TEAM, 8, 2, 3, false) SDEMPC_DUO_WIDE(X, TEAM, 8, false)
 #else
 #define SDEMPC_DUO_M8(X, TEAM)
 #define SDEMPC_DUO_T8(X, TEAM)
@@ -893,12 +911,16 @@
 #define SDEMPC_DUO_TEAM(X, TEAM) SDEMPC_DUO_M(X, TEAM, 4) SDEMPC_DUO_M(X, TEAM, 6) SDEMPC_DUO_M8(X, TEAM)
 #define SDEMPC_DUO_PAIR(X)                                                                                          \
     X(TeamPair, 4, 0, 3, false) X(TeamPair, 4, 1, 3, false) X(TeamPair, 4, 2, 3, false) X(TeamPair, 6, 0, 3, false) X(TeamPair, 6, 1, 3, false) X(TeamPair, 6, 2, 3, false) \
+    SDEMPC_DUO_WIDE(X, TeamPair, 4, false) SDEMPC_DUO_WIDE(X, TeamPair, 6, false) \
     SDEMPC_DUO_T8(X, TeamPair)
 #define SDEMPC_DUO_HEX(X)                                                                                           \
     X(TeamHex, 4, 0, 3, false) X(TeamHex, 4, 1, 3, false) X(TeamHex, 4, 2, 3, false) X(TeamHex, 6, 0, 3, false) X(TeamHex, 6, 1, 3, false) X(TeamHex, 6, 2, 3, false) \
+    SDEMPC_DUO_WIDE(X, TeamHex, 4, false) SDEMPC_DUO_WIDE(X, TeamHex, 6, false) \
     SDEMPC_DUO_T8(X, TeamHex)
 #define SDEMPC_DUO_DECL(TEAM, M, F16, MODE, USTG) extern template __global__ void sdempc_solve_kernel<TEAM, M, F16, false, MODE, USTG>(KArgs);
 #define SDEMPC_DUO_DEF(TEAM, M, F16, MODE, USTG) template __global__ void sdempc_solve_kernel<TEAM, M, F16, false, MODE, USTG>(KArgs);
+#define SDEMPC_DUO_DECL_WIDE(TEAM, M, F16, USTG) extern template __global__ void sdempc_solve_kernel<TEAM, M, F16, false, 3, USTG>(KArgs, WideStage);
+#define SDEMPC_DUO_DEF_WIDE(TEAM, M, F16, USTG) template __global__ void sdempc_solve_kernel<TEAM, M, F16, false, 3, USTG>(KArgs, WideStage);
 
 #if SDEMPC_TU == 1
 SDEMPC_DUO_PAIR(SDEMPC_DUO_DEF)
@@ -971,9 +993,20 @@
     auto per_cu = [&](size_t bytes) { const size_t n = bytes ? cap / bytes : by_regs; return n > by_regs ? by_regs : n; };
     return per_cu(smem_bytes(H, m, 1, false, false)) > per_cu(smem_bytes(H, m, 1));
 }
-template <class Kern>
-static hipError_t launch_persistent(Kern k, const KArgs& a, hipStream_t st, int wg_waves, int bnt, bool ust_lds, int ipb = 1, bool stage = true) {
-    const size_t sb = smem_bytes(a.H, a.m, ipb, false, ust_lds, stage ? wg_waves : 0);
+bool duo_adj_stages(int f16) { return FAST && f16 != 0; }
+DuoStagePlan duo_stage_plan(int H, int m, int ipb, int wg_waves, bool ust_lds, bool adj_stage) {
+    const size_t cap = 156 * 1024, by_regs = 12 / (size_t)wg_waves;
+    auto per_cu = [&](size_t bytes) { const size_t n = cap / bytes; return (int)(n > by_regs ? by_regs : n); };
+    DuoStagePlan p;
+    const size_t narrow = smem_bytes(H, m, ipb, false, ust_lds, wg_waves, NZ_ROWS), wide = smem_bytes(H, m, ipb, false, ust_lds, wg_waves, NZ_ROWS_WIDE);
+    p.per_cu_narrow = per_cu(narrow);
+    p.rows = adj_stage && per_cu(wide) >= 1 && per_cu(wide) == p.per_cu_narrow ? NZ_ROWS_WIDE : NZ_ROWS;
+    p.bytes = p.rows == NZ_ROWS_WIDE ? wide : narrow;
+    p.per_cu = per_cu(p.bytes);
+    return p;
+}
+template <class Kern, class... Tag>
+static hipError_t launch_persistent(Kern k, const KArgs& a, hipStream_t st, int wg_waves, int bnt, size_t sb, int ipb, Tag... tag) {
     hipError_t e = set_smem_attr((const void*)k, sb);
     if (e != hipSuccess) return e;
     size_t per_cu = 12 / (size_t)wg_waves;
@@ -988,10 +1021,20 @@
     ka.tickets = a.work != nullptr && a.ticket_host != nullptr && (size_t)a.B >= 3 * grid * (size_t)ipb;
     if (ka.tickets) ka.ticket_base = *a.ticket_host;
     note_kernel((const void*)k);
-    hipLaunchKernelGGL(k, dim3((unsigned)grid), dim3(bnt), sb, st, ka);
+    hipLaunchKernelGGL(k, dim3((unsigned)grid), dim3(bnt), sb, st, ka, tag...);
     e = hipGetLastError();
     if (e == hipSuccess && ka.tickets) *a.ticket_host = ka.ticket_base + (unsigned)a.B;
     return e;
+}
+template <class TeamD, int M, int F16, bool USTG>
+static hipError_t launch_staged(const KArgs& a, hipStream_t st, int wg_waves, int ipb = 1) {
+    const DuoStagePlan plan = duo_stage_plan(a.H, a.m, ipb, wg_waves, !USTG, duo_adj_stages(F16));
+    if constexpr (FAST && F16 != 0) {
+        const SolveKernWide kw = sdempc_solve_kernel<TeamD, M, F16, false, 3, USTG>;
+        if (plan.rows == NZ_ROWS_WIDE) return launch_persistent(kw, a, st, wg_waves, TeamD::BNT, plan.bytes, ipb, WideStage{});
+    }
+    const SolveKern k = sdempc_solve_kernel<TeamD, M, F16, false, 3, USTG>;
+    return launch_persistent(k, a, st, wg_waves, TeamD::BNT, plan.bytes, ipb);
 }
 template <class TeamD, int M, int F16>
 static hipError_t launch_duo_m(const KArgs& a, hipStream_t st) {
@@ -1004,17 +1047,18 @@
     if (must_g) pick = 1, best = per_cu(false, true);
     else if (can_g && per_cu(false, true) > best) pick = 1, best = per_cu(false, true);
     if (can_g && per_cu(false, false) > best) pick = 2;
-    if (pick == 2) return launch_persistent(sdempc_solve_kernel<TeamD, M, F16, false, 4, true>, a, st, W, TeamD::BNT, false, 1, false);
-    if (pick == 1) return launch_persistent(sdempc_solve_kernel<TeamD, M, F16, false, 3, true>, a, st, W, TeamD::BNT, false);
-    return launch_persistent(sdempc_solve_kernel<TeamD, M, F16, false, 3, false>, a, st, W, TeamD::BNT, true);
+    const SolveKern k4 = sdempc_solve_kernel<TeamD, M, F16, false, 4, true>;
+    if (pick == 2) return launch_persistent(k4, a, st, W, TeamD::BNT, smem_bytes(a.H, a.m, 1, false, false), 1);
+    if (pick == 1) return launch_staged<TeamD, M, F16, true>(a, st, W);
+    return launch_staged<TeamD, M, F16, false>(a, st, W);
 }
 template <int M, int F16>
 static hipError_t launch_duo_small(const KArgs& a, hipStream_t st) {
     const int cus = a.opt.cus > 0 ? a.opt.cus : 256;
     if (a.opt.ustg != 1 && a.opt.hex != 0 && a.B >= 6 * cus && smem_bytes(a.H, a.m, TeamHex::IPB, false, true, 2 * TeamHex::IPB) <= 156 * 1024)
-        return launch_persistent(sdempc_solve_kernel<TeamHex, M, F16, false, 3, false>, a, st, 2 * TeamHex::IPB, TeamHex::BNT, true, TeamHex::IPB);
+        return launch_staged<TeamHex, M, F16, false>(a, st, 2 * TeamHex::IPB, TeamHex::IPB);
     if (a.opt.ustg != 1 && smem_bytes(a.H, a.m, 2, false, true, 4) * 3 <= 156 * 1024)
-        return launch_persistent(sdempc_solve_kernel<TeamPair, M, F16, false, 3, false>, a, st, 4, TeamPair::BNT, true, 2);
+        return launch_staged<TeamPair, M, F16, false>(a, st, 4, 2);
     return launch_duo_m<TeamBlock2, M, F16>(a, st);
 }
 template <int F16>
@@ -1051,7 +1095,7 @@
     if constexpr (Team::IPB == 1) {
         if (takes_duo(a, a.B)) return launch_duo<F16>(a, st);
         if (use_global_ust(a.H, a.m, a.opt) && a.ustg && every_layout_built(a.m))
-            return with_m<true>(a.m, [&](auto M) { return launch_k(sdempc_solve_kernel<Team, M, F16, false, 0, true>, a, st, 1, Team::BNT, false); });
+            return with_m<true>(a.m, [&](auto M) { const SolveKern k = sdempc_solve_kernel<Team, M, F16, false, 0, true>; return launch_k(k, a, st, 1, Team::BNT, false); });
     }
     return with_m(a.m, [&](auto M) { return launch_k(sdempc_solve_kernel<Team, M, F16>, a, st, Team::IPB); });
 }
@@ -1209,6 +1253,10 @@
 void note_kernel(const void* host_fn) { g_last_kernel_fn = host_fn; }
 const void* last_launched_kernel() { return g_last_kernel_fn; }
 size_t smem_bytes(int H, int m, int ipb) { return exact::smem_bytes(H, m, ipb); }
+namespace fastm { bool duo_adj_stages(int f16); }
+DuoStagePlan duo_stage_plan(int H, int m, int ipb, int wg_waves, bool ust_lds, bool fast, int f16) {
+    return exact::duo_stage_plan(H, m, ipb, wg_waves, ust_lds, fast ? fastm::duo_adj_stages(f16) : exact::duo_adj_stages(f16));
+}
 int team_ipb(int G, int H, int m) { return exact::team_ipb(G, H, m); }
 hipError_t launch_rollout(const KArgs& a, int B, hipStream_t st) { return a.fast ? fastm::launch_rollout(a, B, st) : exact::launch_rollout(a, B, st); }
 hipError_t launch_grad(const KArgs& a, int B, hipStream_t st) { return a.fast ? fastm::launch_grad(a, B, st) : exact::launch_grad(a, B, st); }
```

Measured after the change: 4650 (median of 6 runs). About the same (+0.5%).
